# mahdi-slh/DeformContact

Measured on AMD Instinct MI355X. Metric: M edges/sec fwd+bwd, everyday-deform batch=32 per GPU (encoder hot path), higher is better.
Workload: dtype f32 (hops, storage, accumulate); wide dense blocks fp16x2-split operands (3 fp16 MFMA products, fp32 accumulate), narrow ones bf16x3-split (6 products); 1 GPU; everyday-deform synthetic, B=32 sample pairs per GPU: soft 32x(1024 v, 6132 e) + rigid 32x(762 v, 4560 e); TAGConv encoder 2 layers/branch, hidden 256, K=3 (configs[1]); edges_per_gpu_step=342144, global_batch=32, settle_steps=150, hipgraph=True, two_stream_branches=True, merged_branches=False, segmented_adjacency_build=True, parallelism=dp1

## Files before the change

deformcontact_amd/_lib.py:

```python
from __future__ import annotations

import ctypes
import os
from ctypes import POINTER, c_char_p, c_float, c_int, c_int32, c_int64, c_void_p

_HERE = os.path.dirname(os.path.abspath(__file__))
SO_PATH = os.path.join(_HERE, "libdeformcontact_hip.so")

_lib = None

_vp = c_void_p
_SIGNATURES = {
    "dc_version": (c_int, []),
    "dc_last_error": (c_char_p, []),
    "dc_stream_capture_id": (c_int64, [_vp]),
    "dc_csr_workspace_bytes": (c_int64, [c_int64, c_int64]),
    "dc_csr_build": (c_int, [_vp, c_int64, c_int64, c_int, c_int, _vp, _vp, _vp, _vp, _vp, _vp,
                             _vp, c_int64, _vp]),
    "dc_graph_workspace_bytes": (c_int64, [c_int64, c_int64]),
    "dc_graph_build": (c_int, [_vp, c_int64, c_int64, c_int, _vp, _vp, _vp, _vp, _vp, _vp, _vp, _vp,
                               _vp, _vp, c_int64, _vp]),
    "dc_graph_build_parts": (c_int, [POINTER(_vp), POINTER(c_int64), POINTER(c_int64), POINTER(c_int64), c_int,
                                     c_int64, c_int, _vp, _vp, _vp, _vp, _vp, _vp, _vp, _vp, _vp, _vp, c_int64,
                                     _vp]),
    "dc_graph_build_plan": (c_int, [c_int64, c_int64, c_int, POINTER(c_int), POINTER(c_int)]),
    "dc_graph_build_segmented": (c_int, [_vp, c_int64, c_int64, POINTER(c_int64), POINTER(c_int64), c_int,
                                         _vp, _vp, _vp, _vp, _vp, _vp, _vp, _vp, _vp, _vp]),
    "dc_attn_flash_prep": (c_int, [_vp, c_int64, c_int64, _vp, _vp, _vp]),
    "dc_attn_flash_ds": (c_int, [_vp, c_int64, _vp, _vp, c_int64, _vp, _vp, _vp, _vp, _vp, _vp, c_int64, c_int64,
                                 c_int64, c_int64, _vp, _vp, c_int64, _vp, _vp, _vp, _vp]),
    "dc_tag_linear_fwd_h2p_corr": (c_int, [_vp, c_int64, _vp, _vp, _vp, _vp, c_int64, c_int64, c_int64, c_int64, _vp, _vp,
                                           _vp]),
    "dc_tag_linear_bwd_dw_h2_corr": (c_int, [_vp, c_int64, _vp, _vp, POINTER(_vp), POINTER(c_int64), c_int, POINTER(_vp),
                                             c_int, c_int64, c_int, _vp, c_int64, c_int64, c_int64, c_int64, _vp, _vp,
                                             _vp]),
    "dc_attn_flash_fwd": (c_int, [_vp, c_int64, _vp, _vp, _vp, _vp, _vp, c_int64, c_int64, c_int64, c_int64, _vp,
                                  c_int64, _vp, _vp]),
    "dc_hop_chain_max_nodes": (c_int64, []),
    "dc_hop_chain_lds_request": (c_int64, []),
    "dc_hop_chain_f32": (c_int, [_vp, _vp, _vp, _vp, c_int64, POINTER(c_int64), c_int, _vp, c_int64, c_int64, c_int64,
                                 c_int, c_int, c_int, _vp, c_int, _vp]),
    "dc_spmm_f32_bias_act": (c_int, [_vp, _vp, _vp, _vp, c_int64, _vp, c_int, _vp, c_int64, c_int64, c_int64, _vp]),
    "dc_colsum_workspace_bytes": (c_int64, [c_int64, c_int64, c_int]),
    "dc_mask_colsum_f32": (c_int, [_vp, c_int64, _vp, c_int64, _vp, c_int64, c_int64, c_int64, _vp, c_int64, _vp, c_int,
                                   _vp]),
    "dc_gat_alpha_fwd": (c_int, [_vp, c_int64, _vp, _vp, _vp, _vp, c_int64, c_int64, _vp]),
    "dc_gat_alpha_bwd": (c_int, [_vp, c_int64, _vp, _vp, _vp, _vp, _vp, c_int64, c_int64, c_int64, _vp, c_int64, _vp, _vp,
                                 c_int, _vp]),
    "dc_spmm_f32_pack": (c_int, [_vp, _vp, _vp, _vp, c_int64, _vp, c_int64, c_int64, c_int64, c_int64, c_int64, _vp]),
    "dc_spmm_f32_window": (c_int, [_vp, _vp, _vp, _vp, c_int64, _vp, c_int64, _vp, c_int64, c_int64,
                                   c_int64, c_int64, _vp]),
    "dc_spmm_f32_rowmax_window": (c_int, [_vp, _vp, _vp, _vp, c_int64, _vp, c_int64, _vp, c_int64, c_int64,
                                          c_int64, _vp, c_int, c_int64, _vp]),
    "dc_tag_grouped_weight_prep": (c_int, [POINTER(_vp), c_int, c_int, c_int64, c_int64, POINTER(_vp),
                                           POINTER(_vp), POINTER(_vp), POINTER(_vp), _vp]),
    "dc_tag_grouped_fwd_h2p": (c_int, [_vp, c_int64, c_int, POINTER(c_int64), POINTER(c_int64), c_int64,
                                       POINTER(_vp), POINTER(_vp), c_int, _vp, c_int64, c_int64, c_int64, _vp,
                                       POINTER(_vp), _vp]),
    "dc_tag_grouped_mask_grad": (c_int, [POINTER(_vp), POINTER(c_int64), c_int, POINTER(c_int64),
                                         POINTER(c_int64), c_int64, _vp, c_int64, _vp, c_int64, c_int64, _vp,
                                         _vp, _vp]),
    "dc_tag_grouped_bwd_dw_workspace_bytes": (c_int64, [POINTER(c_int64), c_int, c_int64, c_int64, c_int]),
    "dc_tag_grouped_bwd_dw_h2": (c_int, [_vp, c_int64, POINTER(_vp), POINTER(c_int64), c_int, c_int,
                                         POINTER(c_int64), POINTER(c_int64), c_int64, POINTER(_vp),
                                         POINTER(_vp), c_int, _vp, c_int64, c_int64, c_int64, _vp, _vp, _vp]),
    "dc_generic_dense_launches": (c_int64, [c_int]),
    "dc_kernel_trace": (None, [c_int]),
    "dc_kernel_trace_dump": (c_int64, [c_char_p, c_int64]),
    "dc_hash_i64": (c_int, [_vp, c_int64, _vp, _vp]),
    "dc_morton_codes": (c_int, [_vp, c_int64, c_int64, POINTER(c_float), POINTER(c_float), _vp, _vp]),
    "dc_morton_order_workspace_bytes": (c_int64, [c_int64]),
    "dc_morton_order": (c_int, [_vp, c_int64, c_int64, _vp, _vp, _vp, c_int64, _vp]),
    "dc_relabel_edges": (c_int, [_vp, c_int64, _vp, c_int64, _vp, _vp]),
    "dc_gather_rows": (c_int, [_vp, c_int64, _vp, _vp, c_int64, c_int64, c_int64, _vp]),
    "dc_invert_perm": (c_int, [_vp, _vp, _vp, c_int64, _vp]),
    "dc_spmm_f32": (c_int, [_vp, _vp, _vp, _vp, c_int64, _vp, c_int64, _vp, c_int64, c_int64,
                            c_int64, _vp]),
    "dc_spmm_bf16": (c_int, [_vp, _vp, _vp, _vp, c_int64, _vp, c_int64, _vp, c_int64, c_int64,
                             c_int64, c_int, _vp]),
    "dc_tag_linear_fwd_bf16": (c_int, [_vp, c_int64, _vp, _vp, c_int, _vp, c_int64, c_int, c_int64, c_int64,
                                       c_int64, _vp]),
    "dc_tag_mask_grad_bf16": (c_int, [_vp, c_int64, c_int, _vp, c_int64, c_int, _vp, c_int64, c_int64, c_int64, _vp]),
    "dc_tag_linear_bwd_dw_bf16_workspace_bytes": (c_int64, [c_int64, c_int64, c_int64, c_int]),
    "dc_tag_linear_bwd_dw_bf16": (c_int, [_vp, c_int64, _vp, c_int64, c_int, POINTER(_vp), _vp, c_int, _vp, c_int64,
                                          c_int64, c_int64, c_int64, _vp]),
    "dc_to_bf16": (c_int, [POINTER(_vp), c_int, c_int64, c_int64, c_int64, _vp, c_int64, _vp]),
    "dc_contact_loss_workspace_bytes": (c_int64, [c_int64]),
    "dc_contact_loss": (c_int, [_vp, _vp, _vp, _vp, _vp, c_int64, _vp, c_int64, c_int64, c_int64, _vp, _vp,
                                _vp, _vp, c_int64, _vp]),
    "dc_tag_linear_fwd": (c_int, [POINTER(_vp), POINTER(c_int64), POINTER(_vp), c_int, _vp, c_int,
                                  _vp, c_int64, c_int64, c_int64, c_int64, _vp]),
    "dc_tag_linear_bwd_dx": (c_int, [_vp, c_int64, _vp, c_int64, POINTER(_vp), c_int,
                                     POINTER(_vp), POINTER(c_int64), c_int64, c_int64, c_int64,
                                     _vp]),
    "dc_tag_linear_fwd_split": (c_int, [POINTER(_vp), POINTER(c_int64), POINTER(_vp), c_int, _vp,
                                        c_int, _vp, c_int64, c_int64, c_int64, c_int64, c_int, _vp]),
    "dc_tag_linear_bwd_dx_split_workspace_bytes": (c_int64, [c_int64, c_int64, c_int]),
    "dc_tag_linear_bwd_dx_split": (c_int, [_vp, c_int64, _vp, c_int64, POINTER(_vp), c_int,
                                           POINTER(_vp), POINTER(c_int64), _vp, c_int64, c_int64,
                                           c_int64, c_int64, c_int, _vp]),
    "dc_tag_linear_bwd_dw_workspace_bytes": (c_int64, [c_int64, c_int64, c_int64, c_int]),
    "dc_tag_linear_bwd_dw": (c_int, [_vp, c_int64, _vp, c_int64, POINTER(_vp), POINTER(c_int64),
                                     c_int, POINTER(_vp), c_int, c_int64, _vp, c_int, _vp, c_int64,
                                     c_int64, c_int64, c_int64, _vp]),
    "dc_tag_linear_bwd_dw_split": (c_int, [_vp, c_int64, _vp, c_int64, POINTER(_vp),
                                           POINTER(c_int64), c_int, POINTER(_vp), c_int, c_int64,
                                           _vp, c_int, _vp, c_int64, c_int64, c_int64, c_int64,
                                           c_int, _vp]),
    "dc_tag_linear_fwd_h2": (c_int, [POINTER(_vp), POINTER(c_int64), POINTER(_vp), c_int, _vp,
                                     c_int, _vp, c_int64, c_int64, c_int64, c_int64, _vp, _vp, _vp]),
    "dc_tag_linear_bwd_dx_h2": (c_int, [_vp, c_int64, _vp, c_int64, POINTER(_vp), c_int,
                                        POINTER(_vp), POINTER(c_int64), _vp, c_int64, c_int64,
                                        c_int64, c_int64, _vp, _vp, _vp]),
    "dc_tag_linear_bwd_dw_h2": (c_int, [_vp, c_int64, _vp, c_int64, POINTER(_vp),
                                        POINTER(c_int64), c_int, POINTER(_vp), c_int, c_int64,
                                        _vp, c_int, _vp, c_int64, c_int64, c_int64, c_int64,
                                        _vp, _vp, _vp]),
    "dc_tag_mask_grad": (c_int, [_vp, c_int64, _vp, c_int64, _vp, c_int64, c_int64, c_int64, _vp, _vp, _vp]),
    "dc_tag_transpose_weights": (c_int, [POINTER(_vp), c_int, c_int64, c_int64, _vp, _vp]),
    "dc_tag_linear_fwd_h2p_workspace_bytes": (c_int64, [c_int64, c_int64, c_int64]),
    "dc_tag_linear_fwd_h2p": (c_int, [_vp, c_int64, _vp, _vp, c_int, _vp, c_int64, c_int64, c_int64, c_int64,
                                      _vp, _vp, _vp, c_int64, _vp]),
    "dc_tag_linear_fwd_h2p_exp": (c_int, [_vp, c_int64, _vp, _vp, c_int64, c_int64, c_int64, c_int64, _vp, _vp, _vp,
                                          c_int64, _vp]),
    "dc_tag_weight_prep": (c_int, [POINTER(_vp), c_int, c_int64, c_int64, _vp, _vp, _vp, _vp, _vp]),
    "dc_tag_weight_prep_zero": (c_int, [POINTER(_vp), c_int, c_int64, c_int64, _vp, _vp, _vp, _vp, _vp, c_int64, _vp]),
    "dc_rowabsmax_f32": (c_int, [_vp, c_int64, c_int64, c_int64, _vp, _vp]),
    "dc_tag_weight_rowmax": (c_int, [POINTER(_vp), c_int, c_int64, c_int64, _vp, _vp]),
    "dc_spmm_f32_rowmax": (c_int, [_vp, _vp, _vp, _vp, c_int64, _vp, c_int64, _vp, c_int64, c_int64,
                                   c_int64, _vp, c_int, _vp]),
    "dc_tag_pack_input": (c_int, [_vp, c_int64, _vp, c_int64, c_int64, c_int64, c_int64, c_int64, _vp]),
    "dc_tag_pack_weights": (c_int, [POINTER(_vp), c_int, _vp, c_int64, c_int64, c_int64, _vp]),
    "dc_tag_linear_fwd_narrow_ok": (c_int, [c_int64, c_int, c_int64, c_int64]),
    "dc_tag_linear_fwd_narrow": (c_int, [_vp, c_int64, POINTER(_vp), c_int, c_int64, _vp, c_int, _vp, c_int64, c_int64,
                                         c_int64, c_int64, _vp]),
    "dc_attn_softmax_rows": (c_int, [_vp, c_int64, c_int64, c_int64, c_int64, _vp, _vp]),
    "dc_attn_exp_rows": (c_int, [_vp, c_int64, c_int64, c_int64, c_int64, _vp, _vp]),
    "dc_attn_ds_rows": (c_int, [_vp, _vp, c_int64, c_int64, c_int64, _vp, _vp, _vp]),
    "dc_adam_flat": (c_int, [_vp, _vp, _vp, _vp, c_int64, _vp, c_float, c_float, c_float, c_float,
                             c_int, _vp]),
    "dc_compose_perm": (c_int, [_vp, _vp, _vp, _vp, c_int64, _vp]),
    "dc_gat_edge_softmax_fwd": (c_int, [_vp, _vp, _vp, _vp, c_float, _vp, c_int64, _vp]),
    "dc_gat_edge_softmax_bwd": (c_int, [_vp, _vp, _vp, _vp, c_float, _vp, _vp, _vp, _vp, c_int64,
                                        _vp]),
    "dc_sddmm_f32": (c_int, [_vp, _vp, _vp, c_int64, _vp, c_int64, _vp, c_int64, c_int64, _vp]),
    "dc_segment_sum_f32": (c_int, [_vp, _vp, _vp, _vp, c_int64, _vp]),
    "dc_gather_f32": (c_int, [_vp, _vp, _vp, _vp, c_int64, _vp]),
}


class DeformContactLibraryError(RuntimeError):
    pass


def lib():
    global _lib
    if _lib is None:
        if not os.path.exists(SO_PATH):
            raise DeformContactLibraryError(
                f"{SO_PATH} not found. Build it with `python -m deformcontact_amd.build` "
                "(hipcc --offload-arch=gfx950). deformcontact_amd has no CPU/PyTorch fallback.")
        try:
            handle = ctypes.CDLL(SO_PATH)
        except OSError as e:
            raise DeformContactLibraryError(f"cannot load {SO_PATH}: {e}") from e
        for name, (res, args) in _SIGNATURES.items():
            try:
                fn = getattr(handle, name)
            except AttributeError as e:
                raise DeformContactLibraryError(
                    f"{SO_PATH} does not export {name}; rebuild the library") from e
            fn.restype, fn.argtypes = res, args
        _lib = handle
    return _lib


def check(rc: int, what: str) -> None:
    if rc != 0:
        msg = lib().dc_last_error()
        raise DeformContactLibraryError(
            f"{what} failed (rc={rc}): {msg.decode() if msg else '?'}")


def kernel_trace(on: bool) -> None:
    lib().dc_kernel_trace(1 if on else 0)


def kernel_trace_counts() -> dict:
    n = int(lib().dc_kernel_trace_dump(None, 0))
    buf = ctypes.create_string_buffer(n + 1)
    lib().dc_kernel_trace_dump(buf, n + 1)
    out = {}
    for line in buf.value.decode().splitlines():
        name, _, cnt = line.rpartition(" ")
        out[name] = int(cnt)
    return out


def exported_names():
    return list(_SIGNATURES)
```

deformcontact_amd/csrc/dc_dense.h:

```cpp
#pragma once
#include "dc_common.h"

namespace dc {

constexpr int BK = 16;
constexpr int LDK = BK + 4;
constexpr int BN = 128;
constexpr int kMaxSeg = DC_MAX_SEG;

using f32x16 = __attribute__((ext_vector_type(16))) float;

struct Mat {
    const float *p;
    int64_t ld;
};

template <int MB>
struct Frag {
    float a[MB][4];
    float b[2][4];
};

template <int MB, bool A_KC, bool B_KC>
__device__ __forceinline__ void load_frag(Frag<MB> &f, const float *As, const float *Bs, int c,
                                          int wm, int wn) {
    constexpr int BM = 64 * MB;
    const int lane = threadIdx.x & 63, r = lane & 31, h = lane >> 5;
    const int kb = 8 * c + 4 * h;
#pragma unroll
    for (int mb = 0; mb < MB; ++mb) {
        const int row = wm * 32 * MB + mb * 32 + r;
        if (A_KC) {
            const float4 t = *reinterpret_cast<const float4 *>(As + row * LDK + kb);
            f.a[mb][0] = t.x, f.a[mb][1] = t.y, f.a[mb][2] = t.z, f.a[mb][3] = t.w;
        } else {
#pragma unroll
            for (int t = 0; t < 4; ++t) f.a[mb][t] = As[(kb + t) * BM + row];
        }
    }
#pragma unroll
    for (int nb = 0; nb < 2; ++nb) {
        if (B_KC) {
            const float4 t =
                *reinterpret_cast<const float4 *>(Bs + (wn * 64 + nb * 32 + r) * LDK + kb);
            f.b[nb][0] = t.x, f.b[nb][1] = t.y, f.b[nb][2] = t.z, f.b[nb][3] = t.w;
        } else {
#pragma unroll
            for (int t = 0; t < 4; ++t) f.b[nb][t] = Bs[(kb + t) * BN + wn * 64 + nb * 32 + r];
        }
    }
}

template <int MB>
__device__ __forceinline__ void mma_frag(const Frag<MB> &f, f32x16 (&acc)[MB][2]) {
#pragma unroll
    for (int t = 0; t < 4; ++t)
#pragma unroll
        for (int mb = 0; mb < MB; ++mb) {
            acc[mb][0] = __builtin_amdgcn_mfma_f32_32x32x2f32(f.a[mb][t], f.b[0][t], acc[mb][0], 0, 0, 0);
            acc[mb][1] = __builtin_amdgcn_mfma_f32_32x32x2f32(f.a[mb][t], f.b[1][t], acc[mb][1], 0, 0, 0);
        }
}

template <int MB>
__device__ __forceinline__ void zero_acc(f32x16 (&acc)[MB][2]) {
#pragma unroll
    for (int mb = 0; mb < MB; ++mb)
#pragma unroll
        for (int i = 0; i < 16; ++i) acc[mb][0][i] = 0.f, acc[mb][1][i] = 0.f;
}

template <int MB> struct Tile {
    static constexpr int BM = 64 * MB;
    static constexpr int A_KC = BM * LDK, B_KC = BN * LDK, A_RC = BK * BM, B_RC = BK * BN;
};

template <int MB, typename F>
__device__ __forceinline__ void for_each_acc(const f32x16 (&acc)[MB][2], int wm, int wn, F &&f) {
    const int lane = threadIdx.x & 63, c = lane & 31, h = lane >> 5;
#pragma unroll
    for (int mb = 0; mb < MB; ++mb)
#pragma unroll
        for (int nb = 0; nb < 2; ++nb)
#pragma unroll
            for (int reg = 0; reg < 16; ++reg) {
                const int row = wm * 32 * MB + mb * 32 + (reg & 3) + 8 * (reg >> 2) + 4 * h;
                const int col = wn * 64 + nb * 32 + c;
                f(row, col, acc[mb][nb][reg]);
            }
}

struct H2Scales {
    const float *a_rowmax;
    const float *b_rowmax;
    int b_presplit;
};

__device__ __forceinline__ unsigned h2_exp(float m) {
    unsigned e = (__float_as_uint(m) >> 23) & 0xffu;
    e = e < 15u ? 15u : e;
    return e > 254u ? 254u : e;
}
__device__ __forceinline__ float h2_scale(float m) { return __uint_as_float((268u - h2_exp(m)) << 23); }
__device__ __forceinline__ float h2_unscale(float m) { return __uint_as_float((h2_exp(m) - 14u) << 23); }

__device__ __forceinline__ float h2_block_max(const float *v, int64_t beg, int64_t end, float *red) {
    float m = 0.f;
    for (int64_t i = beg + threadIdx.x; i < end; i += 256) m = fmaxf(m, v[i]);
#pragma unroll
    for (int o = 32; o >= 1; o >>= 1) m = fmaxf(m, __shfl_xor(m, o));
    if ((threadIdx.x & 63) == 0) red[threadIdx.x >> 6] = m;
    __syncthreads();
    m = fmaxf(fmaxf(red[0], red[1]), fmaxf(red[2], red[3]));
    __syncthreads();
    return m;
}

constexpr int kMaxGroups = DC_MAX_GROUPS;
constexpr int kGroupAlign = DC_GROUP_ALIGN;
struct FwdGroups {
    int n;
    int64_t row_beg[kMaxGroups];
    int64_t row_end[kMaxGroups];
    const float *w[kMaxGroups];
    const float *bias[kMaxGroups];
    const float *b_rowmax[kMaxGroups];
};
__device__ __forceinline__ int group_of_row(const int64_t (&row_beg)[kMaxGroups], int n, int64_t row) {
    int g = 0;
#pragma unroll
    for (int q = 1; q < kMaxGroups; ++q)
        if (q < n && row >= row_beg[q]) g = q;
    return g;
}

struct FwdParams {
    Mat x[kMaxSeg];
    Mat w[kMaxSeg];
    const float *bias;
    float *out;
    int64_t ldo, N, Fi, Fo;
    int nseg, relu;
    H2Scales h2;
    int ksplit;
    float *kpartial;
    const float *exp_lse;
    int64_t exp_ncols;
    FwdGroups grp;
    const float *x2, *x2_coef;
};

struct DxParams {
    Mat g, mask;
    int has_mask;
    Mat w[kMaxSeg];
    float *gx[kMaxSeg];
    int64_t ldgx[kMaxSeg];
    int64_t N, Fi, Fo;
    int nseg;
    H2Scales h2;
};

struct DwGroups {
    int n;
    int chunk_beg[kMaxGroups + 1];
    int64_t row_beg[kMaxGroups], row_end[kMaxGroups], chunk_rows[kMaxGroups];
};

struct DwParams {
    Mat g, mask;
    int has_mask;
    Mat x[kMaxSeg];
    float *partial;
    float *bias_partial;
    int64_t N, Fi, Fo, chunk_rows;
    int nseg, nchunks;
    H2Scales h2;
    DwGroups grp;
    const float *g2, *g2_coef;
};


struct DwBf16Params {
    const uint16_t *g, *x;
    int64_t ldg, ldx;
    float *partial;
    float *bias_partial;
    int64_t N, Fi, Fo, chunk_rows;
    int nseg, nchunks;
};
bool dw_bf16_launch(const DwBf16Params &p, hipStream_t hs);

bool fwd_fast_launch(const FwdParams &p, int mb, hipStream_t hs);
bool dx_fast_launch(const DxParams &p, int mb, hipStream_t hs);
bool dw_fast_launch(const DwParams &p, int mb, hipStream_t hs);
bool fwd_split_launch(const FwdParams &p, int mb, int products, hipStream_t hs);
bool dx_split_launch(DxParams p, float *wt, int mb, int products, hipStream_t hs);
bool dw_split_launch(const DwParams &p, int mb, int products, hipStream_t hs);
bool dw_h2w_launch(const DwParams &p, hipStream_t hs);
bool fwd_h2_launch(const FwdParams &p, int mb, hipStream_t hs);
bool fwd_h2w_launch(const FwdParams &p, hipStream_t hs);
bool fwd_h2d_launch(const FwdParams &p, hipStream_t hs);
void transpose_weights_launch(const float *const *ws, int nseg, int64_t Fo, int64_t Fi, float *wt,
                              hipStream_t hs);

}
```

deformcontact_amd/csrc/dc_dense.hip:

```cpp
#include <stdlib.h>

#include "dc_dense.h"

#include <atomic>
static std::atomic<long long> g_generic_dense_launches{0};

namespace dc {

template <bool VEC>
__device__ __forceinline__ float4 ld4(const float *row_ptr, int64_t k, int64_t kmax) {
    if (VEC) {
        const int64_t kc = (k + 4 <= kmax) ? k : 0;
        return *reinterpret_cast<const float4 *>(row_ptr + kc);
    } else {
        const int64_t last = kmax - 1;
        return make_float4(row_ptr[k + 0 <= last ? k + 0 : last], row_ptr[k + 1 <= last ? k + 1 : last],
                           row_ptr[k + 2 <= last ? k + 2 : last], row_ptr[k + 3 <= last ? k + 3 : last]);
    }
}

__device__ __forceinline__ float4 zero_invalid(float4 v, bool row_ok, int64_t k, int64_t kmax) {
    return make_float4((row_ok && k + 0 < kmax) ? v.x : 0.f, (row_ok && k + 1 < kmax) ? v.y : 0.f,
                       (row_ok && k + 2 < kmax) ? v.z : 0.f, (row_ok && k + 3 < kmax) ? v.w : 0.f);
}
// ... 325 lines not shown
        *dst = p.accumulate ? *dst + t : t;
    }
}

__device__ __forceinline__ void dw_reduce_body1(const ReduceParams &p) {
    const int64_t per_out = p.Fo * p.cols, total = per_out * p.ngw;
    const int64_t seg_elems = p.Fo * p.Fi, slab = seg_elems * p.nseg;
    const int64_t i = (int64_t)blockIdx.x * blockDim.x + threadIdx.x;
    const float *src;
    float *dst;
    int64_t stride;
    if (i < total) {
        const int j = (int)(i / per_out);
        const int64_t rem = i % per_out, o = rem / p.cols, c = rem % p.cols;
        src = p.partial + (int64_t)(j / p.bps) * seg_elems + o * p.Fi + (int64_t)(j % p.bps) * p.cols + c;
        dst = p.gw[j] + rem;
        stride = slab;
    } else if (p.gbias && i < total + p.Fo) {
        src = p.bias_partial + (i - total);
        dst = p.gbias + (i - total);
        stride = p.Fo;
    } else {
        return;
    }
    float s = 0.f;
    int c = 0;
    for (; c + 8 <= p.nchunks; c += 8) {
        float v[8];
#pragma unroll
        for (int u = 0; u < 8; ++u) v[u] = src[(int64_t)(c + u) * stride];
#pragma unroll
        for (int u = 0; u < 8; ++u) s += v[u];
    }
    for (; c < p.nchunks; ++c) s += src[(int64_t)c * stride];
    *dst = p.accumulate ? *dst + s : s;
}

__global__ void __launch_bounds__(256)
k_dw_reduce(ReduceParams p) { dw_reduce_body1(p); }
__global__ void __launch_bounds__(256)
k_dw_reduce4(ReduceParams p) { dw_reduce_body(p); }
constexpr int kReduce4From = 64;
static inline void launch_reduce(const ReduceParams &r, int64_t total, hipStream_t hs) {
    if (r.nchunks >= kReduce4From)
        DC_LAUNCH(k_dw_reduce4, dim3((unsigned)((total + kReduceOutputs - 1) / kReduceOutputs)), dim3(256), 0, hs, r);
    else
        DC_LAUNCH(k_dw_reduce, dim3((unsigned)((total + 255) / 256)), dim3(256), 0, hs, r);
}

struct ReduceGroups {
    ReduceParams g[kMaxGroups];
};
__global__ void __launch_bounds__(256)
k_dw_reduce_grouped(ReduceGroups rg) { dw_reduce_body1(rg.g[blockIdx.y]); }

static inline Mat make_mat(const float *p, int64_t ld, bool *vec) {
    if (((uintptr_t)p & 15) != 0 || (ld % 4) != 0) *vec = false;
    return Mat{p, ld};
}

static inline int env_int(const char *name, int dflt) {
    const char *v = getenv(name);
    return v ? atoi(v) : dflt;
}

static inline int pick_mb(int64_t rows, int64_t col_tiles) {
    return (((rows + 127) / 128) * col_tiles >= 512) ? 2 : 1;
}

static inline int split_mb(int64_t rows, int64_t col_tiles) {
    const int64_t nb2 = ((rows + 127) / 128) * col_tiles, nb1 = ((rows + 63) / 64) * col_tiles;
    const double t2 = (double)((nb2 + 255) / 256);
    const double t1 = (double)((nb1 + 255) / 256) * 0.5 * 1.12;
    return t1 < t2 ? 1 : 2;
}

static inline int dw_mb(int64_t Fo) {
    return Fo >= 128 ? 2 : 1;
}

static void dw_plan(int64_t N, int64_t Fi, int64_t Fo, int nseg, int64_t *chunk_rows,
                    int *nchunks) {
    const int64_t BM = 64 * dw_mb(Fo);
    const int64_t tiles = ((Fo + BM - 1) / BM) * ((Fi + BN - 1) / BN) * nseg;
    constexpr int target = 512, maxchunks = 128;
    int64_t want = target / (tiles > 0 ? tiles : 1);
    if (want < 1) want = 1;
    if (want > maxchunks) want = maxchunks;
    if (want == 1 && N >= 8192) {
        const int64_t t2 = ((Fo + 127) / 128) * ((Fi + 255) / 256) * nseg;
        double best = 0.0;
        for (int64_t c = 1; c <= 8 && N / c >= 2048; ++c) {
            const int64_t w = (t2 * c + 255) / 256;
            const double eff = (double)(t2 * c) / (double)(w * 256);
            if (eff > best + 0.02) best = eff, want = c;
        }
    }
    int64_t rows = (N + want - 1) / want;
    if (rows < 256) rows = 256;
    rows = (rows + 2 * BK - 1) / (2 * BK) * (2 * BK);
    *chunk_rows = rows;
    *nchunks = (int)((N + rows - 1) / rows);
    if (*nchunks < 1) *nchunks = 1;
}

}

using namespace dc;

static int fwd_impl(const float *const *xs, const int64_t *ldxs, const float *const *ws, int nseg,
                    const float *bias, int relu, float *out, int64_t ldo, int64_t N, int64_t Fi,
                    int64_t Fo, dc_stream_t stream, int products, H2Scales h2 = H2Scales{},
                    float *ksplit_ws = nullptr, int64_t ksplit_ws_bytes = 0, const float *exp_lse = nullptr,
                    int64_t exp_ncols = 0) {
    DC_REQUIRE(nseg >= 1 && nseg <= kMaxSeg, "dc_tag_linear_fwd: nseg must be 1..%d", kMaxSeg);
    DC_REQUIRE(N >= 0 && Fi >= 1 && Fo >= 1, "dc_tag_linear_fwd: bad sizes");
    if (N == 0) return DC_OK;
    DC_REQUIRE(xs && ldxs && ws && out && ldo >= Fo, "dc_tag_linear_fwd: null pointer / ldo < Fo");
    FwdParams p{};
    bool vec = (Fi % 4 == 0);
    for (int s = 0; s < nseg; ++s) {
        DC_REQUIRE(xs[s] && ws[s] && ldxs[s] >= Fi, "dc_tag_linear_fwd: bad segment %d", s);
        p.x[s] = make_mat(xs[s], ldxs[s], &vec);
        p.w[s] = make_mat(ws[s], Fi, &vec);
    }
    p.bias = bias, p.out = out, p.ldo = ldo, p.N = N, p.Fi = Fi, p.Fo = Fo;
    p.nseg = nseg, p.relu = relu;
    p.h2 = h2;
    p.exp_lse = exp_lse, p.exp_ncols = exp_ncols;
    DC_REQUIRE(!exp_lse || h2.b_presplit, "dc_tag_linear_fwd: the exp epilogue exists on the pre-split h2 kernels only");
    const int64_t ntn = (Fo + BN - 1) / BN;
    const int mb = pick_mb(N, ntn);
    const int64_t grid = ((N + 64 * mb - 1) / (64 * mb)) * ntn;
    DC_REQUIRE(grid < (int64_t)INT32_MAX, "dc_tag_linear_fwd: grid too large");
    const dim3 gd((unsigned)grid), bd(256);
    hipStream_t hs = (hipStream_t)stream;
    if (products == 2 && vec) {
        int smb = split_mb(N, ntn);
        const int64_t nst = Fi / BK;
        if (ksplit_ws && !bias && !relu && ldo == Fo && nseg == 1) {
            smb = 2;
            int64_t tiles = ((N + 127) / 128) * ntn;
            if (tiles < 128) smb = 1, tiles = ((N + 63) / 64) * ntn;
            int64_t ks = tiles < 256 ? (512 + tiles - 1) / tiles : 1;
            if (ks > nst / 8) ks = nst / 8;
            if (ks > 32) ks = 32;
            while (ks > 1 && ks * N * Fo * (int64_t)sizeof(float) > ksplit_ws_bytes) --ks;
            if (ks > 1) p.ksplit = (int)ks, p.kpartial = ksplit_ws;
        }
        if (fwd_h2_launch(p, smb, hs)) {
            if (p.ksplit > 1) {
                ReduceParams r{};
                r.partial = p.kpartial, r.gw[0] = out, r.Fi = Fo, r.Fo = N, r.cols = Fo;
                r.nseg = 1, r.nchunks = p.ksplit, r.ngw = 1, r.bps = 1, r.accumulate = 0;
                const int64_t total = N * Fo;
                launch_reduce(r, total, hs);
            }
            return check_launch("dc_tag_linear_fwd_h2");
        }
        p.ksplit = 0, p.kpartial = nullptr;
    }
    DC_REQUIRE(!h2.b_presplit, "dc_tag_linear_fwd_h2p: shape not eligible for the pre-split kernel");
    if (products && vec && fwd_split_launch(p, split_mb(N, ntn), products, hs))
        return check_launch("dc_tag_linear_fwd_split");
    DC_REQUIRE(products != 2, "dc_tag_linear_fwd_h2: needs Fi %% 16 == 0, 16-byte aligned operands, "
                              "equal leading dimensions (Fi=%lld)", (long long)Fi);
    if (vec && fwd_fast_launch(p, mb, hs)) return check_launch("dc_tag_linear_fwd");
    static const int trace = env_int("DC_DENSE_TRACE", 0);
    ++g_generic_dense_launches;
    if (trace)
        fprintf(stderr, "[dc] generic fwd dense kernel: N=%lld Fi=%lld Fo=%lld nseg=%d vec=%d ldx=%lld ldo=%lld products=%d\n",
                (long long)N, (long long)Fi, (long long)Fo, nseg, (int)vec, (long long)ldxs[0], (long long)ldo, products);
    if (mb == 2 && vec)
        DC_LAUNCH((k_tag_linear_fwd<2, true>), gd, bd, 0, hs, p);
    else if (mb == 2)
        DC_LAUNCH((k_tag_linear_fwd<2, false>), gd, bd, 0, hs, p);
    else if (vec)
        DC_LAUNCH((k_tag_linear_fwd<1, true>), gd, bd, 0, hs, p);
    else
        DC_LAUNCH((k_tag_linear_fwd<1, false>), gd, bd, 0, hs, p);
    return check_launch("dc_tag_linear_fwd");
}

static int dx_impl(const float *g, int64_t ldg, const float *out_for_mask, int64_t ldo,
                   const float *const *ws, int nseg, float *const *gxs, const int64_t *ldgxs,
                   int64_t N, int64_t Fi, int64_t Fo, dc_stream_t stream, float *split_ws,
                   int products, H2Scales h2 = H2Scales{}) {
    DC_REQUIRE(nseg >= 1 && nseg <= kMaxSeg, "dc_tag_linear_bwd_dx: nseg must be 1..%d", kMaxSeg);
    DC_REQUIRE(N >= 0 && Fi >= 1 && Fo >= 1, "dc_tag_linear_bwd_dx: bad sizes");
    if (N == 0) return DC_OK;
    DC_REQUIRE(g && ws && gxs && ldgxs && ldg >= Fo, "dc_tag_linear_bwd_dx: null pointer / ldg < Fo");
    DC_REQUIRE(!out_for_mask || ldo >= Fo, "dc_tag_linear_bwd_dx: ldo < Fo");
    DxParams p{};
    bool vec = (Fi % 4 == 0) && (Fo % 4 == 0);
    p.g = make_mat(g, ldg, &vec);
    p.has_mask = out_for_mask != nullptr;
    if (out_for_mask) p.mask = make_mat(out_for_mask, ldo, &vec);
    for (int s = 0; s < nseg; ++s) {
        DC_REQUIRE(ws[s] && gxs[s] && ldgxs[s] >= Fi, "dc_tag_linear_bwd_dx: bad segment %d", s);
        p.w[s] = make_mat(ws[s], Fi, &vec);
        p.gx[s] = gxs[s];
        p.ldgx[s] = ldgxs[s];
    }
    p.N = N, p.Fi = Fi, p.Fo = Fo, p.nseg = nseg;
    p.h2 = h2;
    const int64_t ntn = ((Fi + BN - 1) / BN) * nseg;
    const int mb = pick_mb(N, ntn);
    const int64_t grid = ((N + 64 * mb - 1) / (64 * mb)) * ntn;
    DC_REQUIRE(grid < (int64_t)INT32_MAX, "dc_tag_linear_bwd_dx: grid too large");
    if (!p.has_mask) p.mask = p.g;
    const dim3 gd((unsigned)grid), bd(256);
    hipStream_t hs = (hipStream_t)stream;
    if (split_ws && vec && dx_split_launch(p, split_ws, split_mb(N, ntn), products, hs))
        return check_launch("dc_tag_linear_bwd_dx_split");
    DC_REQUIRE(products != 2, "dc_tag_linear_bwd_dx_h2: needs Fo %% 16 == 0, Fi %% 4 == 0 and 16-byte "
                              "aligned operands (Fi=%lld Fo=%lld)", (long long)Fi, (long long)Fo);
    if (vec && dx_fast_launch(p, mb, hs)) return check_launch("dc_tag_linear_bwd_dx");
    ++g_generic_dense_launches;
#define DC_DX(MB_, V_, M_) DC_LAUNCH((k_tag_linear_bwd_dx<MB_, V_, M_>), gd, bd, 0, hs, p)
    if (mb == 2) {
        if (vec && p.has_mask) DC_DX(2, true, true);
        else if (vec) DC_DX(2, true, false);
        else if (p.has_mask) DC_DX(2, false, true);
        else DC_DX(2, false, false);
    } else {
        if (vec && p.has_mask) DC_DX(1, true, true);
        else if (vec) DC_DX(1, true, false);
        else if (p.has_mask) DC_DX(1, false, true);
        else DC_DX(1, false, false);
    }
#undef DC_DX
    return check_launch("dc_tag_linear_bwd_dx");
}

extern "C" int dc_tag_linear_fwd(const float *const *xs, const int64_t *ldxs,
                                 const float *const *ws, int nseg, const float *bias, int relu,
                                 float *out, int64_t ldo, int64_t N, int64_t Fi, int64_t Fo,
                                 dc_stream_t stream) {
    return fwd_impl(xs, ldxs, ws, nseg, bias, relu, out, ldo, N, Fi, Fo, stream, 0);
}

extern "C" int dc_tag_linear_fwd_split(const float *const *xs, const int64_t *ldxs,
                                       const float *const *ws, int nseg, const float *bias,
                                       int relu, float *out, int64_t ldo, int64_t N, int64_t Fi,
                                       int64_t Fo, int products, dc_stream_t stream) {
    DC_REQUIRE(products == 6 || products == 3 || products == 1,
               "dc_tag_linear_fwd_split: products must be 6, 3 or 1");
    return fwd_impl(xs, ldxs, ws, nseg, bias, relu, out, ldo, N, Fi, Fo, stream, products);
}

extern "C" int dc_tag_linear_bwd_dx(const float *g, int64_t ldg, const float *out_for_mask,
                                    int64_t ldo, const float *const *ws, int nseg,
                                    float *const *gxs, const int64_t *ldgxs, int64_t N, int64_t Fi,
                                    int64_t Fo, dc_stream_t stream) {
    return dx_impl(g, ldg, out_for_mask, ldo, ws, nseg, gxs, ldgxs, N, Fi, Fo, stream, nullptr, 0);
}

extern "C" int dc_tag_linear_bwd_dw(const float *g, int64_t ldg, const float *out_for_mask,
                                    int64_t ldo, const float *const *xs, const int64_t *ldxs,
                                    int nseg, float *const *gws, int ngw, int64_t gw_cols,
                                    float *gbias, int accumulate, void *partials,
                                    int64_t partials_bytes, int64_t N, int64_t Fi, int64_t Fo,
                                    dc_stream_t stream);
extern "C" int dc_tag_linear_bwd_dw_split(const float *g, int64_t ldg, const float *out_for_mask,
                                          int64_t ldo, const float *const *xs, const int64_t *ldxs,
                                          int nseg, float *const *gws, int ngw, int64_t gw_cols,
                                          float *gbias, int accumulate, void *partials,
                                          int64_t partials_bytes, int64_t N, int64_t Fi, int64_t Fo,
                                          int products, dc_stream_t stream);

extern "C" int64_t dc_tag_linear_bwd_dx_split_workspace_bytes(int64_t Fi, int64_t Fo, int nseg) {
    if (Fi < 1 || Fo < 1 || nseg < 1 || nseg > kMaxSeg) return DC_EINVAL;
    return (int64_t)sizeof(float) * nseg * Fi * Fo + 16;
}

extern "C" int dc_tag_linear_bwd_dx_split(const float *g, int64_t ldg, const float *out_for_mask,
                                          int64_t ldo, const float *const *ws, int nseg,
                                          float *const *gxs, const int64_t *ldgxs, void *workspace,
                                          int64_t workspace_bytes, int64_t N, int64_t Fi,
                                          int64_t Fo, int products, dc_stream_t stream) {
    DC_REQUIRE(products == 6 || products == 3 || products == 1,
               "dc_tag_linear_bwd_dx_split: products must be 6, 3 or 1");
    DC_REQUIRE(workspace && ((uintptr_t)workspace & 15) == 0 &&
                   workspace_bytes >= dc_tag_linear_bwd_dx_split_workspace_bytes(Fi, Fo, nseg),
               "dc_tag_linear_bwd_dx_split: workspace missing, misaligned or too small");
    return dx_impl(g, ldg, out_for_mask, ldo, ws, nseg, gxs, ldgxs, N, Fi, Fo, stream,
                   (float *)workspace, products);
}

extern "C" int64_t dc_tag_linear_bwd_dw_workspace_bytes(int64_t N, int64_t Fi, int64_t Fo,
                                                        int nseg) {
    if (N < 0 || Fi < 1 || Fo < 1 || nseg < 1 || nseg > kMaxSeg) return DC_EINVAL;
    int64_t rows;
    int nchunks;
    dw_plan(N, Fi, Fo, nseg, &rows, &nchunks);
    return (int64_t)sizeof(float) * (nchunks + 1) * (nseg * Fo * Fi + Fo) + 16;
}

static int dw_impl(const float *g, int64_t ldg, const float *out_for_mask, int64_t ldo,
                   const float *const *xs, const int64_t *ldxs, int nseg, float *const *gws, int ngw,
                   int64_t gw_cols, float *gbias, int accumulate, void *partials,
                   int64_t partials_bytes, int64_t N, int64_t Fi, int64_t Fo, dc_stream_t stream,
                   int products, H2Scales h2 = H2Scales{}, const float *g2 = nullptr,
                   const float *g2_coef = nullptr) {
    DC_REQUIRE(nseg >= 1 && nseg <= kMaxSeg, "dc_tag_linear_bwd_dw: nseg must be 1..%d", kMaxSeg);
    DC_REQUIRE(N >= 0 && Fi >= 1 && Fo >= 1, "dc_tag_linear_bwd_dw: bad sizes");
    DC_REQUIRE(g && xs && ldxs && gws && partials && ldg >= Fo,
               "dc_tag_linear_bwd_dw: null pointer / ldg < Fo");
    DC_REQUIRE(!out_for_mask || ldo >= Fo, "dc_tag_linear_bwd_dw: ldo < Fo");
    DC_REQUIRE(partials_bytes >= dc_tag_linear_bwd_dw_workspace_bytes(N, Fi, Fo, nseg),
               "dc_tag_linear_bwd_dw: workspace too small");
    DC_REQUIRE(((uintptr_t)partials & 15) == 0, "dc_tag_linear_bwd_dw: workspace not 16-byte aligned");
    DwParams p{};
    bool vec = (Fi % 4 == 0) && (Fo % 4 == 0);
    p.g = make_mat(g, ldg, &vec);
    p.has_mask = out_for_mask != nullptr;
    if (out_for_mask) p.mask = make_mat(out_for_mask, ldo, &vec);
    ReduceParams r{};
    for (int s = 0; s < nseg; ++s) {
        DC_REQUIRE(xs[s] && ldxs[s] >= Fi, "dc_tag_linear_bwd_dw: bad segment %d", s);
        p.x[s] = make_mat(xs[s], ldxs[s], &vec);
    }
    DC_REQUIRE(ngw >= nseg && ngw <= 2 * kMaxSeg && ngw % nseg == 0 && gw_cols >= 1 &&
                   (ngw / nseg) * gw_cols <= Fi,
               "dc_tag_linear_bwd_dw: %d output blocks of %lld columns do not tile %d segments of %lld",
               ngw, (long long)gw_cols, nseg, (long long)Fi);
    for (int j = 0; j < ngw; ++j) {
        DC_REQUIRE(gws[j], "dc_tag_linear_bwd_dw: null output block %d", j);
        r.gw[j] = gws[j];
    }
    dw_plan(N, Fi, Fo, nseg, &p.chunk_rows, &p.nchunks);
    p.N = N, p.Fi = Fi, p.Fo = Fo, p.nseg = nseg;
    p.h2 = h2;
    p.partial = (float *)partials;
    const int64_t tail = vec ? N % BK : 0;
    const bool ragged = tail != 0 && N > tail;
    const int nslots = p.nchunks + (ragged ? 1 : 0);
    p.bias_partial = gbias ? p.partial + (int64_t)nslots * nseg * Fo * Fi : nullptr;
    const int mb = dw_mb(Fo);
    const int64_t tiles = ((Fo + 64 * mb - 1) / (64 * mb)) * ((Fi + BN - 1) / BN);
    const int64_t grid = tiles * nseg * p.nchunks;
    if (!p.has_mask) p.mask = p.g;
    const dim3 gd((unsigned)grid), bd(256);
    hipStream_t hs = (hipStream_t)stream;
    if (g2) {
        DC_REQUIRE(g2_coef && products == 2 && vec && !ragged && (((uintptr_t)g2) & 15) == 0,
                   "dc_tag_linear_bwd_dw_h2_corr: needs the coefficient vector, aligned operands and N %% 16 == 0");
        p.g2 = g2, p.g2_coef = g2_coef;
        DC_REQUIRE(dw_h2w_launch(p, hs), "dc_tag_linear_bwd_dw_h2_corr: shape not eligible for the 128 x 256 tile kernel "
                   "(needs Fo %% 128 == 0, Fi == 256, N %% 32 == 0; N=%lld Fi=%lld Fo=%lld)", (long long)N,
                   (long long)Fi, (long long)Fo);
        r.partial = p.partial, r.bias_partial = p.bias_partial, r.gbias = gbias;
        r.Fi = Fi, r.Fo = Fo, r.nseg = nseg, r.nchunks = nslots;
        r.cols = gw_cols, r.ngw = ngw, r.bps = ngw / nseg, r.accumulate = accumulate;
        const int64_t total_c = (int64_t)ngw * Fo * gw_cols + (gbias ? Fo : 0);
        launch_reduce(r, total_c, hs);
        return check_launch("dc_tag_linear_bwd_dw_h2_corr");
    }
    if (ragged) {
        DwParams t = p;
        const int64_t n0 = N - tail;
        t.g.p += n0 * t.g.ld;
        t.mask.p += n0 * t.mask.ld;
        for (int s = 0; s < nseg; ++s) t.x[s].p += n0 * t.x[s].ld;
        t.N = tail, t.chunk_rows = BK, t.nchunks = 1;
        t.partial = p.partial + (int64_t)p.nchunks * nseg * Fo * Fi;
        t.bias_partial = p.bias_partial ? p.bias_partial + (int64_t)p.nchunks * Fo : nullptr;
        t.h2 = H2Scales{};
        const dim3 gt((unsigned)(tiles * nseg));
        if (mb == 2) {
            if (p.has_mask) DC_LAUNCH((k_tag_linear_bwd_dw<2, true, true>), gt, bd, 0, hs, t);
            else DC_LAUNCH((k_tag_linear_bwd_dw<2, true, false>), gt, bd, 0, hs, t);
        } else {
            if (p.has_mask) DC_LAUNCH((k_tag_linear_bwd_dw<1, true, true>), gt, bd, 0, hs, t);
            else DC_LAUNCH((k_tag_linear_bwd_dw<1, true, false>), gt, bd, 0, hs, t);
        }
        p.N = n0;
    }
    bool fast_done = products && vec && dw_split_launch(p, mb, products, hs);
    DC_REQUIRE(fast_done || products != 2, "dc_tag_linear_bwd_dw_h2: needs N %% 16 == 0, Fi %% 4 == 0, "
               "Fo %% 4 == 0 and 16-byte aligned operands (N=%lld)", (long long)N);
    fast_done = fast_done || (vec && dw_fast_launch(p, mb, hs));
#define DC_DW(MB_, V_, M_) DC_LAUNCH((k_tag_linear_bwd_dw<MB_, V_, M_>), gd, bd, 0, hs, p)
    if (!fast_done) ++g_generic_dense_launches;
    if (fast_done) {
    } else
    if (mb == 2) {
        if (vec && p.has_mask) DC_DW(2, true, true);
        else if (vec) DC_DW(2, true, false);
        else if (p.has_mask) DC_DW(2, false, true);
        else DC_DW(2, false, false);
    } else {
        if (vec && p.has_mask) DC_DW(1, true, true);
        else if (vec) DC_DW(1, true, false);
        else if (p.has_mask) DC_DW(1, false, true);
        else DC_DW(1, false, false);
    }
#undef DC_DW
    r.partial = p.partial, r.bias_partial = p.bias_partial, r.gbias = gbias;
    r.Fi = Fi, r.Fo = Fo, r.nseg = nseg, r.nchunks = nslots;
    r.cols = gw_cols, r.ngw = ngw, r.bps = ngw / nseg, r.accumulate = accumulate;
    const int64_t total = (int64_t)ngw * Fo * gw_cols + (gbias ? Fo : 0);
    launch_reduce(r, total, (hipStream_t)stream);
    return check_launch("dc_tag_linear_bwd_dw");
}

extern "C" int dc_tag_linear_bwd_dw(const float *g, int64_t ldg, const float *out_for_mask,
                                    int64_t ldo, const float *const *xs, const int64_t *ldxs,
                                    int nseg, float *const *gws, int ngw, int64_t gw_cols,
                                    float *gbias, int accumulate, void *partials,
                                    int64_t partials_bytes, int64_t N, int64_t Fi, int64_t Fo,
                                    dc_stream_t stream) {
    return dw_impl(g, ldg, out_for_mask, ldo, xs, ldxs, nseg, gws, ngw, gw_cols, gbias, accumulate,
                   partials, partials_bytes, N, Fi, Fo, stream, 0);
}

extern "C" int dc_tag_linear_bwd_dw_split(const float *g, int64_t ldg, const float *out_for_mask,
                                          int64_t ldo, const float *const *xs, const int64_t *ldxs,
                                          int nseg, float *const *gws, int ngw, int64_t gw_cols,
                                          float *gbias, int accumulate, void *partials,
                                          int64_t partials_bytes, int64_t N, int64_t Fi, int64_t Fo,
                                          int products, dc_stream_t stream) {
    DC_REQUIRE(products == 6 || products == 3 || products == 1,
               "dc_tag_linear_bwd_dw_split: products must be 6, 3 or 1");
    return dw_impl(g, ldg, out_for_mask, ldo, xs, ldxs, nseg, gws, ngw, gw_cols, gbias, accumulate,
                   partials, partials_bytes, N, Fi, Fo, stream, products);
}


extern "C" int dc_tag_linear_fwd_h2(const float *const *xs, const int64_t *ldxs,
                                    const float *const *ws, int nseg, const float *bias, int relu,
                                    float *out, int64_t ldo, int64_t N, int64_t Fi, int64_t Fo,
                                    const float *x_rowmax, const float *w_rowmax,
                                    dc_stream_t stream) {
    DC_REQUIRE(x_rowmax && w_rowmax, "dc_tag_linear_fwd_h2: x_rowmax / w_rowmax missing");
    H2Scales h{};
    h.a_rowmax = x_rowmax, h.b_rowmax = w_rowmax;
    return fwd_impl(xs, ldxs, ws, nseg, bias, relu, out, ldo, N, Fi, Fo, stream, 2, h);
}

extern "C" int64_t dc_tag_linear_fwd_h2p_workspace_bytes(int64_t N, int64_t K, int64_t Fo) {
    if (N < 0 || K < 1 || Fo < 1) return DC_EINVAL;
    const int64_t tiles = ((N + 63) / 64) * ((Fo + BN - 1) / BN);
    if (tiles >= 256 || K / BK < 16) return 0;
    return 32 * N * Fo * (int64_t)sizeof(float);
}

extern "C" int dc_tag_linear_fwd_h2p(const float *x, int64_t ldx, const void *w_image,
                                     const float *bias, int relu, float *out, int64_t ldo, int64_t N,
                                     int64_t K, int64_t Fo, const float *x_rowmax,
                                     const float *w_rowmax, void *workspace,
                                     int64_t workspace_bytes, dc_stream_t stream) {
    DC_REQUIRE(x && w_image && x_rowmax && w_rowmax, "dc_tag_linear_fwd_h2p: null pointer");
    DC_REQUIRE(K >= 16 && K % 16 == 0 && ldx >= K && ldx % 4 == 0 && (((uintptr_t)x) & 15) == 0 &&
                   (((uintptr_t)w_image) & 15) == 0,
               "dc_tag_linear_fwd_h2p: K %% 16 == 0 and 16-byte aligned operands required (K=%lld)",
               (long long)K);
    H2Scales h{};
    h.a_rowmax = x_rowmax, h.b_rowmax = w_rowmax, h.b_presplit = 1;
    const float *xs[1] = {x};
    const float *ws[1] = {(const float *)w_image};
    const int64_t ld[1] = {ldx};
    DC_REQUIRE(!workspace || (((uintptr_t)workspace) & 15) == 0, "dc_tag_linear_fwd_h2p: workspace misaligned");
    return fwd_impl(xs, ld, ws, 1, bias, relu, out, ldo, N, K, Fo, stream, 2, h, (float *)workspace,
                    workspace ? workspace_bytes : 0);
}

extern "C" int dc_tag_linear_fwd_h2p_corr(const float *x, int64_t ldx, const float *x2, const float *x2_coef,
                                          const void *w_image, float *out, int64_t ldo, int64_t N, int64_t K,
                                          int64_t Fo, const float *x_rowmax, const float *w_rowmax,
                                          dc_stream_t stream) {
    DC_REQUIRE(N >= 0 && K >= 32 && K % 32 == 0 && Fo >= 1, "dc_tag_linear_fwd_h2p_corr: K must be a multiple of 32");
    if (N == 0) return DC_OK;
    DC_REQUIRE(x && x2 && x2_coef && w_image && out && x_rowmax && w_rowmax && ldx >= K && ldo >= Fo &&
                   (((uintptr_t)x2) & 15) == 0, "dc_tag_linear_fwd_h2p_corr: null / short / misaligned operand");
    FwdParams p{};
    bool vec = true;
    p.x[0] = make_mat(x, ldx, &vec);
    p.w[0] = make_mat((const float *)w_image, K, &vec);
    p.out = out, p.ldo = ldo, p.N = N, p.Fi = K, p.Fo = Fo, p.nseg = 1;
    p.h2.a_rowmax = x_rowmax, p.h2.b_rowmax = w_rowmax, p.h2.b_presplit = 1;
    p.x2 = x2, p.x2_coef = x2_coef;
    DC_REQUIRE(vec && fwd_h2w_launch(p, (hipStream_t)stream),
               "dc_tag_linear_fwd_h2p_corr: shape not eligible for the 128 x 256 tile kernel (N=%lld K=%lld Fo=%lld: "
               "needs 16-byte aligned rows)", (long long)N, (long long)K, (long long)Fo);
    return check_launch("dc_tag_linear_fwd_h2p_corr");
}

extern "C" int dc_tag_linear_fwd_h2p_exp(const float *x, int64_t ldx, const void *w_image, float *out,
                                         int64_t ldo, int64_t N, int64_t K, int64_t Fo, const float *x_rowmax,
                                         const float *w_rowmax, const float *row_lse, int64_t ncols_valid,
                                         dc_stream_t stream) {
    DC_REQUIRE(x && w_image && x_rowmax && w_rowmax && row_lse, "dc_tag_linear_fwd_h2p_exp: null pointer");
    DC_REQUIRE(K >= 16 && K % 16 == 0 && ldx >= K && ldx % 4 == 0 && (((uintptr_t)x) & 15) == 0 &&
                   (((uintptr_t)w_image) & 15) == 0 && ncols_valid >= 0 && ncols_valid <= Fo,
               "dc_tag_linear_fwd_h2p_exp: K %% 16 == 0, 16-byte aligned operands, 0 <= ncols_valid <= Fo required");
    H2Scales h{};
    h.a_rowmax = x_rowmax, h.b_rowmax = w_rowmax, h.b_presplit = 1;
    const float *xs[1] = {x};
    const float *ws[1] = {(const float *)w_image};
    const int64_t ld[1] = {ldx};
    return fwd_impl(xs, ld, ws, 1, nullptr, 0, out, ldo, N, K, Fo, stream, 2, h, nullptr, 0, row_lse, ncols_valid);
}

extern "C" int dc_tag_linear_bwd_dx_h2(const float *g, int64_t ldg, const float *out_for_mask,
                                       int64_t ldo, const float *const *ws, int nseg,
                                       float *const *gxs, const int64_t *ldgxs, void *workspace,
                                       int64_t workspace_bytes, int64_t N, int64_t Fi, int64_t Fo,
                                       const float *g_rowmax, const float *w_rowmax,
                                       dc_stream_t stream) {
    DC_REQUIRE(w_rowmax && g_rowmax, "dc_tag_linear_bwd_dx_h2: g_rowmax / w_rowmax missing");
    DC_REQUIRE(workspace && ((uintptr_t)workspace & 15) == 0 &&
                   workspace_bytes >= dc_tag_linear_bwd_dx_split_workspace_bytes(Fi, Fo, nseg),
               "dc_tag_linear_bwd_dx_h2: workspace missing, misaligned or too small");
    H2Scales h{};
    h.a_rowmax = g_rowmax, h.b_rowmax = w_rowmax;
    return dx_impl(g, ldg, out_for_mask, ldo, ws, nseg, gxs, ldgxs, N, Fi, Fo, stream,
                   (float *)workspace, 2, h);
}

extern "C" int dc_tag_linear_bwd_dw_h2(const float *g, int64_t ldg, const float *out_for_mask,
                                       int64_t ldo, const float *const *xs, const int64_t *ldxs,
                                       int nseg, float *const *gws, int ngw, int64_t gw_cols,
                                       float *gbias, int accumulate, void *partials,
                                       int64_t partials_bytes, int64_t N, int64_t Fi, int64_t Fo,
                                       const float *g_rowmax, const float *x_rowmax,
                                       dc_stream_t stream) {
    DC_REQUIRE(g_rowmax && x_rowmax, "dc_tag_linear_bwd_dw_h2: g_rowmax / x_rowmax missing");
    H2Scales h{};
    h.a_rowmax = g_rowmax, h.b_rowmax = x_rowmax;
    return dw_impl(g, ldg, out_for_mask, ldo, xs, ldxs, nseg, gws, ngw, gw_cols, gbias, accumulate,
                   partials, partials_bytes, N, Fi, Fo, stream, 2, h);
}

extern "C" int dc_tag_linear_bwd_dw_h2_corr(const float *g, int64_t ldg, const float *g2, const float *g2_coef,
                                            const float *const *xs, const int64_t *ldxs, int nseg,
                                            float *const *gws, int ngw, int64_t gw_cols, int accumulate,
                                            void *partials, int64_t partials_bytes, int64_t N, int64_t Fi,
                                            int64_t Fo, const float *g_rowmax, const float *x_rowmax,
                                            dc_stream_t stream) {
    DC_REQUIRE(g2 && g2_coef && g_rowmax && x_rowmax, "dc_tag_linear_bwd_dw_h2_corr: null g2 / coefficients / row maxima");
    H2Scales h2{};
    h2.a_rowmax = g_rowmax, h2.b_rowmax = x_rowmax;
    return dw_impl(g, ldg, nullptr, 0, xs, ldxs, nseg, gws, ngw, gw_cols, nullptr, accumulate, partials,
                   partials_bytes, N, Fi, Fo, stream, 2, h2, g2, g2_coef);
}

namespace dc {
__global__ void __launch_bounds__(256)
k_rowabsmax(const float *__restrict__ x, int64_t ld, int64_t N, int F, float *__restrict__ rowmax,
            bool vec4) {
    const int64_t row = (int64_t)blockIdx.x * 4 + (threadIdx.x >> 6);
    if (row >= N) return;
    const int lane = threadIdx.x & 63;
    const float *xr = x + row * ld;
    float m = 0.f;
    if (vec4) {
        for (int c = lane * 4; c < F; c += 256) {
            const float4 v = *reinterpret_cast<const float4 *>(xr + c);
            m = fmaxf(m, fmaxf(fmaxf(fabsf(v.x), fabsf(v.y)), fmaxf(fabsf(v.z), fabsf(v.w))));
        }
    } else {
        for (int c = lane; c < F; c += 64) m = fmaxf(m, fabsf(xr[c]));
    }
#pragma unroll
    for (int o = 32; o >= 1; o >>= 1) m = fmaxf(m, __shfl_xor(m, o));
    if (lane == 0) rowmax[row] = m;
}

struct WRowmaxParams {
    const float *w[kMaxSeg];
    int nseg;
    int64_t Fo, Fi;
    float *out;
};
__global__ void __launch_bounds__(256) k_w_rowmax(WRowmaxParams p) {
    const int64_t o = (int64_t)blockIdx.x * 4 + (threadIdx.x >> 6);
    if (o >= p.Fo) return;
    const int lane = threadIdx.x & 63;
    float m = 0.f;
    for (int s = 0; s < p.nseg; ++s) {
        const float *wr = p.w[s] + o * p.Fi;
        for (int64_t c = lane; c < p.Fi; c += 64) m = fmaxf(m, fabsf(wr[c]));
    }
#pragma unroll
    for (int q = 32; q >= 1; q >>= 1) m = fmaxf(m, __shfl_xor(m, q));
    if (lane == 0) p.out[o] = m;
}
}

namespace dc {
__global__ void __launch_bounds__(256)
k_mask_grad(const float *__restrict__ g, int64_t ldg, const float *__restrict__ mask, int64_t ldm,
            float *__restrict__ gm, int64_t ldgm, int64_t N, int F, float *__restrict__ rowmax_a,
            float *__restrict__ rowmax_b, bool vec4) {
    const int64_t row = (int64_t)blockIdx.x * 4 + (threadIdx.x >> 6);
    if (row >= N) return;
    const int lane = threadIdx.x & 63;
    const float *gr = g + row * ldg, *mr = mask ? mask + row * ldm : nullptr;
    float *o = gm + row * ldgm;
    float m = 0.f;
    if (vec4) {
        for (int c = lane * 4; c < F; c += 256) {
            float4 v = *reinterpret_cast<const float4 *>(gr + c);
            if (mr) {
                const float4 k = *reinterpret_cast<const float4 *>(mr + c);
                v = make_float4(k.x > 0.f ? v.x : 0.f, k.y > 0.f ? v.y : 0.f, k.z > 0.f ? v.z : 0.f,
                                k.w > 0.f ? v.w : 0.f);
            }
            *reinterpret_cast<float4 *>(o + c) = v;
            m = fmaxf(m, fmaxf(fmaxf(fabsf(v.x), fabsf(v.y)), fmaxf(fabsf(v.z), fabsf(v.w))));
        }
    } else {
        for (int c = lane; c < F; c += 64) {
            float v = gr[c];
            if (mr && !(mr[c] > 0.f)) v = 0.f;
            o[c] = v;
            m = fmaxf(m, fabsf(v));
        }
    }
#pragma unroll
    for (int q = 32; q >= 1; q >>= 1) m = fmaxf(m, __shfl_xor(m, q));
    if (lane == 0) {
        rowmax_a[row] = m;
        if (rowmax_b) rowmax_b[row] = m;
    }
}
}

extern "C" int dc_tag_mask_grad(const float *g, int64_t ldg, const float *out_for_mask, int64_t ldo,
                                float *gm, int64_t ldgm, int64_t N, int64_t F, float *rowmax_a,
                                float *rowmax_b, dc_stream_t stream) {
    DC_REQUIRE(N >= 0 && F >= 1 && F < (1 << 24) && ldg >= F && ldgm >= F && (!out_for_mask || ldo >= F),
               "dc_tag_mask_grad: bad sizes");
    if (N == 0) return DC_OK;
    DC_REQUIRE(g && gm && rowmax_a, "dc_tag_mask_grad: null pointer");
    const bool vec4 = (F % 4 == 0) && (ldg % 4 == 0) && (ldgm % 4 == 0) && (((uintptr_t)g) & 15) == 0 &&
                      (((uintptr_t)gm) & 15) == 0 &&
                      (!out_for_mask || ((ldo % 4 == 0) && (((uintptr_t)out_for_mask) & 15) == 0));
    DC_LAUNCH(k_mask_grad, dim3((unsigned)((N + 3) / 4)), dim3(256), 0, (hipStream_t)stream, g,
                       ldg, out_for_mask, ldo, gm, ldgm, N, (int)F, rowmax_a, rowmax_b, vec4);
    return check_launch("dc_tag_mask_grad");
}

namespace dc {
struct WPrepParams {
    const float *w[kMaxSeg];
    int nseg;
    int64_t Fo, Fi;
    float *w_rowmax, *wt_rowmax;
    _Float16 *wimg, *wtimg;
    float *zero;
    int64_t zero_n;
    int tall;
};
__device__ __forceinline__ void wprep_put(_Float16 *img_row, int64_t k, float v, float scale) {
    const float x = v * scale;
    const _Float16 h = (_Float16)x;
    _Float16 *rec = img_row + (k >> 4) * 32 + (k & 15);
    rec[0] = h;
    rec[16] = (_Float16)(x - (float)h);
}
__device__ __forceinline__ void weight_prep_body(const WPrepParams &p) {
    const int lane = threadIdx.x & 63;
    for (int64_t i = (int64_t)blockIdx.x * blockDim.x + threadIdx.x; i < p.zero_n; i += (int64_t)gridDim.x * blockDim.x)
        p.zero[i] = 0.f;
    if (p.tall)
        for (int64_t i = (int64_t)blockIdx.x * blockDim.x + threadIdx.x; i < p.Fi; i += (int64_t)gridDim.x * blockDim.x)
            p.wt_rowmax[i] = 0.f;
    const int64_t rb = (p.Fo + 3) / 4;
    float m = 0.f;
    const bool small = p.Fi <= 256 && p.Fo <= 256;
    if ((int64_t)blockIdx.x < rb) {
        const int64_t o = (int64_t)blockIdx.x * 4 + (threadIdx.x >> 6);
        if (o >= p.Fo) return;
        float v[kMaxSeg][4];
        if (small) {
#pragma unroll
            for (int s = 0; s < kMaxSeg; ++s)
#pragma unroll
                for (int j = 0; j < 4; ++j) {
                    const int64_t c = lane + 64 * j;
                    v[s][j] = (s < p.nseg && c < p.Fi) ? p.w[s][o * p.Fi + c] : 0.f;
                    m = fmaxf(m, fabsf(v[s][j]));
                }
        } else {
            for (int s = 0; s < p.nseg; ++s) {
                const float *wr = p.w[s] + o * p.Fi;
                for (int64_t c = lane; c < p.Fi; c += 64) m = fmaxf(m, fabsf(wr[c]));
            }
        }
#pragma unroll
        for (int q = 32; q >= 1; q >>= 1) m = fmaxf(m, __shfl_xor(m, q));
        if (lane == 0) p.w_rowmax[o] = m;
        if (p.wimg) {
            const float sc = h2_scale(m);
            _Float16 *row = p.wimg + o * (2 * p.nseg * p.Fi);
            if (small) {
#pragma unroll
                for (int s = 0; s < kMaxSeg; ++s)
#pragma unroll
                    for (int j = 0; j < 4; ++j) {
                        const int64_t c = lane + 64 * j;
                        if (s < p.nseg && c < p.Fi) wprep_put(row, s * p.Fi + c, v[s][j], sc);
                    }
            } else {
                for (int s = 0; s < p.nseg; ++s) {
                    const float *wr = p.w[s] + o * p.Fi;
                    for (int64_t c = lane; c < p.Fi; c += 64) wprep_put(row, s * p.Fi + c, wr[c], sc);
                }
            }
        }
    } else {
        const int64_t f = ((int64_t)blockIdx.x - rb) * 4 + (threadIdx.x >> 6);
        if (f >= p.Fi) return;
        float v[kMaxSeg][4];
        if (small) {
#pragma unroll
            for (int s = 0; s < kMaxSeg; ++s)
#pragma unroll
                for (int j = 0; j < 4; ++j) {
                    const int64_t o = lane + 64 * j;
                    v[s][j] = (s < p.nseg && o < p.Fo) ? p.w[s][o * p.Fi + f] : 0.f;
                    m = fmaxf(m, fabsf(v[s][j]));
                }
        } else {
            for (int s = 0; s < p.nseg; ++s) {
                const float *wc = p.w[s] + f;
                for (int64_t o = lane; o < p.Fo; o += 64) m = fmaxf(m, fabsf(wc[o * p.Fi]));
// ... 438 lines not shown
```

deformcontact_amd/csrc/dc_dense_narrow.hip:

```cpp
#include "dc_dense.h"

#ifndef DC_NARROW_ABL
#define DC_NARROW_ABL 0
#endif

namespace dc {

using nb_bf16x4 = __attribute__((ext_vector_type(4))) __bf16;
using nb_bf16x8 = __attribute__((ext_vector_type(8))) __bf16;
using nb_f32x4 = __attribute__((ext_vector_type(4))) float;

struct NarrowParams {
    const float *x;
    int64_t ld;
    const float *w[kMaxSeg];
    int nseg, fi;
    const float *bias;
    float *out;
    int64_t ldo, N;
    int relu, ntiles;
};

constexpr int kNarrowFo = 256;

__device__ __forceinline__ void nb_lds_barrier() {
    asm volatile("s_waitcnt lgkmcnt(0)\n\ts_barrier" ::: "memory");
}

__device__ __forceinline__ void nb_split1(float x, __bf16 &hi, __bf16 &mid, __bf16 &lo) {
    hi = (__bf16)x;
    const float r = x - (float)hi;
    mid = (__bf16)r;
    const float r2 = r - (float)mid;
    lo = (__bf16)r2;
}

template <int KS, int MB>
__global__ void __launch_bounds__(256)
k_fwd_narrow(NarrowParams p) {
    constexpr int TR = 32 * MB;
    constexpr int SROWA = KS * 96 + 16;
    constexpr int PPR = 4 * KS;
    constexpr int TP = TR * PPR, NV = (TP + 255) / 256;
    constexpr int KP = 16 * KS;
    constexpr int kOffStage = ((TR * SROWA + 1023) / 1024) * 1024;
    constexpr int kLdsTiles = kOffStage + TR * 1024, kLdsW = kNarrowFo * (KP + 4) * 4;
    __shared__ __attribute__((aligned(1024))) char lds[kLdsTiles > kLdsW ? kLdsTiles : kLdsW];
    char *const sA = lds;
    float *const so = reinterpret_cast<float *>(lds + kOffStage);
    const int wid = __builtin_amdgcn_readfirstlane((int)(threadIdx.x >> 6)), lane = threadIdx.x & 63;
    const int c = lane & 31, h = lane >> 5;

    nb_f32x4 xv[NV];
    auto load_tile = [&](int t) {
        const int64_t row0 = (int64_t)t * TR;
#pragma unroll
        for (int j = 0; j < NV; ++j) {
            const int q = (int)threadIdx.x + 256 * j;
            if (TP % 256 != 0 && q >= TP) continue;
            const int r = q / PPR, c4 = q - r * PPR;
            int64_t row = row0 + r;
            row = row < p.N ? row : p.N - 1;
            if (DC_NARROW_ABL & 8) xv[j] = nb_f32x4{(float)row, 1.f, 2.f, 3.f};
            else xv[j] = *reinterpret_cast<const nb_f32x4 *>(p.x + row * p.ld + 4 * c4);
        }
    };
    int t = blockIdx.x;
    if (t < p.ntiles) load_tile(t);

    constexpr int WROW = KP + 4;
    {
        float *wi = reinterpret_cast<float *>(lds);
        const int width = p.nseg * p.fi, per4 = kNarrowFo * p.fi / 4;
        constexpr int MAXQ = 8;
        nb_f32x4 wv[kMaxSeg][MAXQ];
#pragma unroll
        for (int s = 0; s < kMaxSeg; ++s)
#pragma unroll
            for (int j = 0; j < MAXQ; ++j) {
                const int q = (int)threadIdx.x + 256 * j;
                if (!(DC_NARROW_ABL & 2) && s < p.nseg && q < per4) wv[s][j] = *reinterpret_cast<const nb_f32x4 *>(p.w[s] + 4 * q);
            }
#pragma unroll
        for (int s = 0; s < kMaxSeg; ++s)
#pragma unroll
            for (int j = 0; j < MAXQ; ++j) {
                const int q = (int)threadIdx.x + 256 * j;
                if (!(DC_NARROW_ABL & 2) && s < p.nseg && q < per4) {
                    int o = (4 * q) / p.fi, f = 4 * q - o * p.fi;
#pragma unroll
                    for (int i = 0; i < 4; ++i) {
                        wi[o * WROW + s * p.fi + f] = wv[s][j][i];
                        if (++f == p.fi) f = 0, ++o;
                    }
                }
            }
        const int padw = KP - width;
        for (int e = threadIdx.x; e < kNarrowFo * padw; e += 256) {
            const int o = e / padw, f = e - o * padw;
            wi[o * WROW + width + f] = 0.f;
        }
    }
    __syncthreads();
    nb_bf16x8 fb[2][KS][3];
#pragma unroll
    for (int nb = 0; nb < 2; ++nb) {
        const float *wr = reinterpret_cast<const float *>(lds) + (64 * wid + 32 * nb + c) * WROW + 8 * h;
#pragma unroll
        for (int ks = 0; ks < KS; ++ks) {
            const nb_f32x4 v0 = *reinterpret_cast<const nb_f32x4 *>(wr + 16 * ks);
            const nb_f32x4 v1 = *reinterpret_cast<const nb_f32x4 *>(wr + 16 * ks + 4);
#pragma unroll
            for (int j = 0; j < 8; ++j) {
                __bf16 hi, mid, lo;
                nb_split1(j < 4 ? v0[j] : v1[j - 4], hi, mid, lo);
                fb[nb][ks][0][j] = hi, fb[nb][ks][1][j] = mid, fb[nb][ks][2][j] = lo;
            }
        }
    }
    __syncthreads();
    float bcol[2];
#pragma unroll
    for (int nb = 0; nb < 2; ++nb) bcol[nb] = p.bias ? p.bias[64 * wid + 32 * nb + c] : 0.f;
    const bool relu = p.relu != 0;

    auto store_tile = [&]() {
#pragma unroll
        for (int j = 0; j < NV; ++j) {
            const int q = (int)threadIdx.x + 256 * j;
            if (TP % 256 != 0 && q >= TP) continue;
            const int r = q / PPR, c4 = q - r * PPR;
            nb_bf16x4 hi, mid, lo;
#pragma unroll
            for (int i = 0; i < 4; ++i) {
                __bf16 a, b, d;
                nb_split1(xv[j][i], a, b, d);
                hi[i] = a, mid[i] = b, lo[i] = d;
            }
            char *dst = sA + r * SROWA + (c4 >> 2) * 96 + ((c4 >> 1) & 1) * 16 + (c4 & 1) * 8;
            *reinterpret_cast<nb_bf16x4 *>(dst) = hi;
            *reinterpret_cast<nb_bf16x4 *>(dst + 32) = mid;
            *reinterpret_cast<nb_bf16x4 *>(dst + 64) = lo;
        }
    };

    auto store_rows = [&](int64_t row0) {
#pragma unroll 4
        for (int r = wid; r < TR; r += 4) {
            const int64_t row = row0 + r;
            const nb_f32x4 v = *reinterpret_cast<const nb_f32x4 *>(so + r * 256 + 4 * lane);
            if (row < p.N && (!(DC_NARROW_ABL & 4) || v[0] == 12345.678f)) *reinterpret_cast<nb_f32x4 *>(p.out + row * p.ldo + 4 * lane) = v;
        }
    };
    int64_t prev_row0 = -1;
    for (; t < p.ntiles; t += gridDim.x) {
        const int64_t row0 = (int64_t)t * TR;
        if (!(DC_NARROW_ABL & 8)) store_tile();
        if (prev_row0 >= 0) store_rows(prev_row0);
        if (t + (int)gridDim.x < p.ntiles) load_tile(t + gridDim.x);
        nb_lds_barrier();
        f32x16 acc[MB][2];
#pragma unroll
        for (int mb = 0; mb < MB; ++mb)
#pragma unroll
            for (int nb = 0; nb < 2; ++nb)
#pragma unroll
                for (int i = 0; i < 16; ++i) acc[mb][nb][i] = 0.f;
        constexpr int HI = 0, MID = 1, LO = 2;
        constexpr int pa6[6] = {LO, HI, MID, MID, HI, HI}, pb6[6] = {HI, LO, MID, HI, MID, HI};
#pragma unroll
        for (int ks = 0; ks < KS; ++ks) {
            nb_bf16x8 fa[MB][3];
#pragma unroll
            for (int mb = 0; mb < MB; ++mb)
#pragma unroll
                for (int pl = 0; pl < 3; ++pl)
                    fa[mb][pl] = *reinterpret_cast<const nb_bf16x8 *>(sA + (mb * 32 + c) * SROWA + ks * 96 + pl * 32 + h * 16);
#pragma unroll
            for (int tt = 0; tt < 6; ++tt)
#pragma unroll
                for (int mb = 0; mb < MB; ++mb)
#pragma unroll
                    for (int nb = 0; nb < 2; ++nb)
                        if (!(DC_NARROW_ABL & 1))
                            acc[mb][nb] = __builtin_amdgcn_mfma_f32_32x32x16_bf16(fa[mb][pa6[tt]], fb[nb][ks][pb6[tt]], acc[mb][nb], 0, 0, 0);
                        else
                            acc[mb][nb][tt] += (float)fa[mb][pa6[tt]][0] * (float)fb[nb][ks][pb6[tt]][0];
        }
#pragma unroll
        for (int mb = 0; mb < MB; ++mb)
#pragma unroll
            for (int nb = 0; nb < 2; ++nb)
#pragma unroll
                for (int r = 0; r < 16; ++r) {
                    float v = acc[mb][nb][r] + bcol[nb];
                    if (relu) v = fmaxf(v, 0.f);
                    if (!(DC_NARROW_ABL & 16) || r == 0)
                        so[(mb * 32 + (r & 3) + 8 * (r >> 2) + 4 * h) * 256 + 64 * wid + 32 * nb + c] = v;
                }
        nb_lds_barrier();
        prev_row0 = row0;
    }
    if (prev_row0 >= 0) store_rows(prev_row0);
}

template <int KS>
static void narrow_launch(const NarrowParams &p0, hipStream_t hs) {
    NarrowParams p = p0;
    p.ntiles = (int)((p.N + 31) / 32);
    const unsigned grid = (unsigned)(p.ntiles < 256 ? p.ntiles : 256);
    DC_LAUNCH((k_fwd_narrow<KS, 1>), dim3(grid), dim3(256), 0, hs, p);
}

}

using namespace dc;

extern "C" int dc_tag_linear_fwd_narrow_ok(int64_t fi, int nseg, int64_t wpad, int64_t Fo) {
    return (Fo == kNarrowFo && nseg >= 1 && nseg <= kMaxSeg && fi >= 1 && fi <= 32 && nseg * fi <= wpad &&
            (wpad == 96 || wpad == 112 || wpad == 128)) ? 1 : 0;
}

extern "C" int dc_tag_linear_fwd_narrow(const float *slab, int64_t ld, const float *const *ws, int nseg, int64_t fi,
                                        const float *bias, int relu, float *out, int64_t ldo, int64_t N, int64_t wpad,
                                        int64_t Fo, dc_stream_t stream) {
    DC_REQUIRE(dc_tag_linear_fwd_narrow_ok(fi, nseg, wpad, Fo),
               "dc_tag_linear_fwd_narrow: needs Fo = 256, a padded reduction of 96 / 112 / 128 >= nseg * fi (got Fo=%lld wpad=%lld "
               "nseg=%d fi=%lld)", (long long)Fo, (long long)wpad, nseg, (long long)fi);
    DC_REQUIRE(N >= 0, "dc_tag_linear_fwd_narrow: negative N");
    if (N == 0) return DC_OK;
    DC_REQUIRE(slab && ws && out && ld >= wpad && ldo >= Fo, "dc_tag_linear_fwd_narrow: null pointer / short leading dimension");
    DC_REQUIRE(ld % 4 == 0 && ldo % 4 == 0 && ((uintptr_t)slab & 15) == 0 && ((uintptr_t)out & 15) == 0,
               "dc_tag_linear_fwd_narrow: rows of the slab and of the output must be 16-byte aligned");
    DC_REQUIRE(N < ((int64_t)1 << 31) - 64, "dc_tag_linear_fwd_narrow: too many rows");
    NarrowParams p{};
    p.x = slab, p.ld = ld, p.nseg = nseg, p.fi = (int)fi, p.bias = bias, p.out = out, p.ldo = ldo, p.N = N, p.relu = relu;
    for (int s = 0; s < nseg; ++s) {
        DC_REQUIRE(ws[s], "dc_tag_linear_fwd_narrow: null weight segment %d", s);
        p.w[s] = ws[s];
    }
    hipStream_t hs = (hipStream_t)stream;
    switch (wpad) {
    case 96: narrow_launch<6>(p, hs); break;
    case 112: narrow_launch<7>(p, hs); break;
    default: narrow_launch<8>(p, hs); break;
    }
    return check_launch("dc_tag_linear_fwd_narrow");
}
```

deformcontact_amd/csrc/dc_dense_split.hip:

```cpp
#include "dc_dense.h"

#ifndef DC_DWS_ABL
#define DC_DWS_ABL 0
#endif

namespace dc {

using bf16x4 = __attribute__((ext_vector_type(4))) __bf16;
using bf16x8 = __attribute__((ext_vector_type(8))) __bf16;

constexpr int kPlane = 32;

template <int NP> struct Planes {
    static_assert(NP == 6 || NP == 3 || NP == 1 || NP == 2, "products per tile: 6, 3, 1 or 2 (= fp16x2)");
    static constexpr bool F16 = NP == 2;
    static constexpr int P = NP == 6 ? 3 : ((NP == 3 || NP == 2) ? 2 : 1);
    static constexpr int NPROD = NP == 2 ? 3 : NP;
    static constexpr int SROW = P * kPlane + 16;
};

using f16x4 = __attribute__((ext_vector_type(4))) _Float16;
using f16x8 = __attribute__((ext_vector_type(8))) _Float16;

__device__ __forceinline__ void split4_h2(const float4 &v, f16x4 &h, f16x4 &l) {
    const float x[4] = {v.x, v.y, v.z, v.w};
#pragma unroll
    for (int i = 0; i < 4; ++i) {
        const _Float16 a = (_Float16)x[i];
        h[i] = a;
        l[i] = (_Float16)(x[i] - (float)a);
    }
}

__device__ __forceinline__ void split1(float x, __bf16 &hi, __bf16 &mid, __bf16 &lo) {
    hi = (__bf16)x;
    const float r = x - (float)hi;
    mid = (__bf16)r;
    const float r2 = r - (float)mid;
    lo = (__bf16)r2;
}

__device__ __forceinline__ void split4(const float4 &v, bf16x4 &hi, bf16x4 &mid, bf16x4 &lo) {
    __bf16 h, m, l;
    split1(v.x, h, m, l); hi[0] = h, mid[0] = m, lo[0] = l;
    split1(v.y, h, m, l); hi[1] = h, mid[1] = m, lo[1] = l;
    split1(v.z, h, m, l); hi[2] = h, mid[2] = m, lo[2] = l;
    split1(v.w, h, m, l); hi[3] = h, mid[3] = m, lo[3] = l;
}

template <int ROWS, bool MASK, int NP>
struct SplitOp {
    static constexpr int SROW = Planes<NP>::SROW, P = Planes<NP>::P;
    static constexpr int NV = ROWS / 64;
    const float *p[NV];
    const float *pm[MASK ? NV : 1];
    float4 v[NV];
    float4 m[MASK ? NV : 1];
    int off[NV];
    float sc[NV];

    __device__ __forceinline__ void init(const float *base, const float *mbase, int64_t ld,
                                         int64_t row0, int64_t nrows, int64_t mld = 0) {
        const int k4 = threadIdx.x & 3, r = threadIdx.x >> 2;
#pragma unroll
        for (int j = 0; j < NV; ++j) {
            int64_t row = row0 + r + 64 * j;
            row = row < nrows ? row : nrows - 1;
            p[j] = base + row * ld + 4 * k4;
            if (MASK) pm[j] = mbase + row * (mld ? mld : ld) + 4 * k4;
            off[j] = (r + 64 * j) * SROW + 8 * k4;
        }
    }
    __device__ __forceinline__ void rebase(int64_t delta) {
#pragma unroll
        for (int j = 0; j < NV; ++j) p[j] += delta;
    }
    __device__ __forceinline__ void load() {
#pragma unroll
        for (int j = 0; j < NV; ++j) {
            v[j] = *reinterpret_cast<const float4 *>(p[j]);
            p[j] += BK;
            if (MASK) {
                m[j] = *reinterpret_cast<const float4 *>(pm[j]);
                pm[j] += BK;
            }
        }
    }
    __device__ __forceinline__ void store(char *lds) const {
#pragma unroll
        for (int j = 0; j < NV; ++j) {
            float4 x = v[j];
            if (MASK)
                x = make_float4(m[j].x > 0.f ? x.x : 0.f, m[j].y > 0.f ? x.y : 0.f,
                                m[j].z > 0.f ? x.z : 0.f, m[j].w > 0.f ? x.w : 0.f);
            if (Planes<NP>::F16) {
                x = make_float4(x.x * sc[j], x.y * sc[j], x.z * sc[j], x.w * sc[j]);
                f16x4 h, l;
                split4_h2(x, h, l);
                *reinterpret_cast<f16x4 *>(lds + off[j]) = h;
                *reinterpret_cast<f16x4 *>(lds + off[j] + kPlane) = l;
                continue;
            }
            bf16x4 hi, mid, lo;
            split4(x, hi, mid, lo);
            *reinterpret_cast<bf16x4 *>(lds + off[j]) = hi;
            if (P > 1) *reinterpret_cast<bf16x4 *>(lds + off[j] + kPlane) = mid;
            if (P > 2) *reinterpret_cast<bf16x4 *>(lds + off[j] + 2 * kPlane) = lo;
        }
    }
    __device__ __forceinline__ void set_scale(float s) {
#pragma unroll
        for (int j = 0; j < NV; ++j) sc[j] = s;
    }
};

template <int MB, int NP>
struct SplitFrag {
    bf16x8 a[MB][Planes<NP>::P];
    bf16x8 b[2][Planes<NP>::P];
};

template <int MB, int NP>
__device__ __forceinline__ void load_split_frag(SplitFrag<MB, NP> &f, const char *As,
                                                const char *Bs, int wm, int wn) {
    constexpr int SROW = Planes<NP>::SROW, P = Planes<NP>::P;
    const int lane = threadIdx.x & 63, r = lane & 31, h = lane >> 5;
#pragma unroll
    for (int mb = 0; mb < MB; ++mb)
#pragma unroll
        for (int pl = 0; pl < P; ++pl)
            f.a[mb][pl] = *reinterpret_cast<const bf16x8 *>(
                As + (wm * 32 * MB + mb * 32 + r) * SROW + pl * kPlane + 16 * h);
#pragma unroll
    for (int nb = 0; nb < 2; ++nb)
#pragma unroll
        for (int pl = 0; pl < P; ++pl)
            f.b[nb][pl] = *reinterpret_cast<const bf16x8 *>(
                Bs + (wn * 64 + nb * 32 + r) * SROW + pl * kPlane + 16 * h);
}

template <int MB, int NP>
__device__ __forceinline__ void mma_split(const SplitFrag<MB, NP> &f, f32x16 (&acc)[MB][2]) {
    constexpr int HI = 0, MID = 1, LO = 2;
    constexpr int pa6[6] = {LO, HI, MID, MID, HI, HI}, pb6[6] = {HI, LO, MID, HI, MID, HI};
    constexpr int pa3[3] = {MID, HI, HI}, pb3[3] = {HI, MID, HI};
    constexpr int NPROD = Planes<NP>::NPROD;
#pragma unroll
    for (int t = 0; t < NPROD; ++t) {
        const int ia = NPROD == 6 ? pa6[t] : (NPROD == 3 ? pa3[t] : HI);
        const int ib = NPROD == 6 ? pb6[t] : (NPROD == 3 ? pb3[t] : HI);
#pragma unroll
        for (int mb = 0; mb < MB; ++mb)
#pragma unroll
            for (int nb = 0; nb < 2; ++nb) {
                if (Planes<NP>::F16)
                    acc[mb][nb] = __builtin_amdgcn_mfma_f32_32x32x16_f16(
                        __builtin_bit_cast(f16x8, f.a[mb][ia]), __builtin_bit_cast(f16x8, f.b[nb][ib]),
                        acc[mb][nb], 0, 0, 0);
                else
                    acc[mb][nb] = __builtin_amdgcn_mfma_f32_32x32x16_bf16(f.a[mb][ia], f.b[nb][ib],
                                                                          acc[mb][nb], 0, 0, 0);
            }
    }
}

template <int MB, int NP, typename OA, typename OB, typename Next>
__device__ __forceinline__ void split_loop(char *lds, int nst, OA &A, OB &B, Next &&next_stage,
                                           f32x16 (&acc)[MB][2], int wm, int wn) {
    constexpr int SROW = Planes<NP>::SROW;
    constexpr int BM = 64 * MB, kOffB = BM * SROW, kStage = (BM + BN) * SROW;
    if (nst <= 0) return;
    A.load();
    B.load();
    next_stage();
    A.store(lds);
    B.store(lds + kOffB);
    if (nst > 1) {
        A.load();
        B.load();
        next_stage();
    }
    __syncthreads();
    for (int it = 0; it < nst; ++it) {
        char *cur = lds + (it & 1) * kStage, *nxt = lds + ((it + 1) & 1) * kStage;
        SplitFrag<MB, NP> f;
        load_split_frag<MB, NP>(f, cur, cur + kOffB, wm, wn);
        if (it + 1 < nst) {
            A.store(nxt);
            B.store(nxt + kOffB);
        }
        if (it + 2 < nst) {
            A.load();
            B.load();
            next_stage();
        }
        mma_split<MB, NP>(f, acc);
        __syncthreads();
    }
}

template <int MB, int NP>
__global__ void __launch_bounds__(256)
k_fwd_split(FwdParams p) {
    constexpr int BM = 64 * MB, SROW = Planes<NP>::SROW;
    __shared__ __attribute__((aligned(16))) char lds[2 * (BM + BN) * SROW];
    const unsigned ntn = (unsigned)((p.Fo + BN - 1) / BN);
    const unsigned lb = xcd_remap(blockIdx.x, gridDim.x);
    const int64_t row0 = (int64_t)(lb / ntn) * BM, col0 = (int64_t)(lb % ntn) * BN;
    const int wid = threadIdx.x >> 6, wm = wid >> 1, wn = wid & 1;

    f32x16 acc[MB][2];
    zero_acc<MB>(acc);
    SplitOp<BM, false, NP> A;
    SplitOp<BN, false, NP> B;
    A.init(p.x[0].p, nullptr, p.x[0].ld, row0, p.N);
    B.init(p.w[0].p, nullptr, p.Fi, col0, p.Fo);
    constexpr bool F16 = Planes<NP>::F16;
    __shared__ float s_inv[F16 ? BM : 1];
    if (F16) {
        const int r = threadIdx.x >> 2;
#pragma unroll
        for (int j = 0; j < BM / 64; ++j) {
            int64_t row = row0 + r + 64 * j;
            row = row < p.N ? row : p.N - 1;
            const float m = p.h2.a_rowmax[row];
            A.sc[j] = h2_scale(m);
            if ((threadIdx.x & 3) == 0) s_inv[r + 64 * j] = h2_unscale(m);
        }
#pragma unroll
        for (int j = 0; j < BN / 64; ++j) {
            int64_t col = col0 + r + 64 * j;
            col = col < p.Fo ? col : p.Fo - 1;
            B.sc[j] = h2_scale(p.h2.b_rowmax[col]);
        }
    }
    const int kst = (int)(p.Fi / BK), nst = kst * p.nseg;
    int kk = 0, seg = 0;
    auto next_stage = [&]() {
        if (++kk == kst && seg + 1 < p.nseg) {
            kk = 0;
            A.rebase((p.x[seg + 1].p - p.x[seg].p) - p.Fi);
            B.rebase((p.w[seg + 1].p - p.w[seg].p) - p.Fi);
            ++seg;
        }
    };
    split_loop<MB, NP>(lds, nst, A, B, next_stage, acc, wm, wn);

    float bcol[2], icol[2] = {1.f, 1.f};
#pragma unroll
    for (int nb = 0; nb < 2; ++nb) {
        const int64_t col = col0 + wn * 64 + nb * 32 + (threadIdx.x & 31);
        bcol[nb] = (p.bias && col < p.Fo) ? p.bias[col] : 0.f;
        if (F16) icol[nb] = h2_unscale(p.h2.b_rowmax[col < p.Fo ? col : p.Fo - 1]);
    }
    const bool relu = p.relu != 0;
    for_each_acc<MB>(acc, wm, wn, [&](int r, int c, float v) {
        const int64_t row = row0 + r, col = col0 + c;
        if (row < p.N && col < p.Fo) {
            if (F16) v = (v * s_inv[r]) * icol[(c >> 5) & 1];
            v += bcol[(c >> 5) & 1];
            if (relu) v = fmaxf(v, 0.f);
            p.out[row * p.ldo + col] = v;
        }
    });
}

template <int MB, bool MASK, int NP>
__global__ void __launch_bounds__(256)
k_dx_split(DxParams p) {
    constexpr int BM = 64 * MB, SROW = Planes<NP>::SROW;
    __shared__ __attribute__((aligned(16))) char lds[2 * (BM + BN) * SROW];
    const unsigned ntn = (unsigned)((p.Fi + BN - 1) / BN), per_row = ntn * p.nseg;
    const unsigned lb = xcd_remap(blockIdx.x, gridDim.x);
    const int64_t row0 = (int64_t)(lb / per_row) * BM;
    const int s = (int)((lb % per_row) / ntn);
    const int64_t col0 = (int64_t)(lb % ntn) * BN;
    const int wid = threadIdx.x >> 6, wm = wid >> 1, wn = wid & 1;

    f32x16 acc[MB][2];
    zero_acc<MB>(acc);
    SplitOp<BM, MASK, NP> A;
    SplitOp<BN, false, NP> B;
    A.init(p.g.p, p.mask.p, p.g.ld, row0, p.N, p.mask.ld);
    B.init(p.w[s].p, nullptr, p.Fo, col0, p.Fi);
    constexpr bool F16 = Planes<NP>::F16;
    __shared__ float s_inv[F16 ? BM : 1];
    float invb = 1.f;
    if (F16) {
        const int r = threadIdx.x >> 2;
#pragma unroll
        for (int j = 0; j < BM / 64; ++j) {
            int64_t row = row0 + r + 64 * j;
            row = row < p.N ? row : p.N - 1;
            const float m = p.h2.a_rowmax[row];
            A.sc[j] = h2_scale(m);
            if ((threadIdx.x & 3) == 0) s_inv[r + 64 * j] = h2_unscale(m);
        }
        const float bm = h2_block_max(p.h2.b_rowmax, 0, p.Fo, reinterpret_cast<float *>(lds));
        B.set_scale(h2_scale(bm));
        invb = h2_unscale(bm);
    }
    split_loop<MB, NP>(lds, (int)(p.Fo / BK), A, B, []() {}, acc, wm, wn);
    float *out = p.gx[s];
    const int64_t ldo = p.ldgx[s];
    for_each_acc<MB>(acc, wm, wn, [&](int r, int c, float v) {
        const int64_t row = row0 + r, col = col0 + c;
        if (F16) v = (v * s_inv[r]) * invb;
        if (row < p.N && col < p.Fi) out[row * ldo + col] = v;
    });
}

template <int COLS, int NP> struct TrImage {
    static constexpr int ROWB = COLS * 2 + 64;
    static constexpr int PLANE = BK * ROWB;
    static constexpr int BYTES = Planes<NP>::P * PLANE;
};

template <int COLS, bool MASK, int NP>
struct SplitOpRC {
    static constexpr int P = Planes<NP>::P;
    static constexpr int NV = COLS / 64;
    static constexpr int PER = COLS / 4, KPER = 256 / PER;
    using Img = TrImage<COLS, NP>;
    const float *p[NV];
    const float *pm[MASK ? NV : 1];
    float4 v[NV];
    float4 m[MASK ? NV : 1];
    int off[NV];
    int64_t step, mstep;
    float sc;

    __device__ __forceinline__ void init(const float *base, const float *mbase, int64_t ld,
                                         int64_t k0, int64_t col0, int64_t ncols, int64_t mld = 0) {
        const int c4 = threadIdx.x % PER, kr = threadIdx.x / PER;
        int64_t col = col0 + 4 * c4;
        col = col + 4 <= ncols ? col : ncols - 4;
        mld = mld ? mld : ld;
#pragma unroll
        for (int j = 0; j < NV; ++j) {
            const int64_t k = k0 + kr + KPER * j;
            p[j] = base + k * ld + col;
            if (MASK) pm[j] = mbase + k * mld + col;
            off[j] = (kr + KPER * j) * Img::ROWB + 8 * c4;
        }
        step = BK * ld;
        mstep = BK * mld;
    }
    __device__ __forceinline__ void load() {
#pragma unroll
        for (int j = 0; j < NV; ++j) {
            if ((DC_DWS_ABL & 8) && MASK) v[j] = make_float4(1.f, 2.f, 3.f, (float)j);
            else if ((DC_DWS_ABL & 16) && !MASK) v[j] = make_float4(1.f, 2.f, 3.f, (float)j);
            else v[j] = *reinterpret_cast<const float4 *>(p[j]);
            p[j] += step;
            if (MASK) {
                if (DC_DWS_ABL & 2) m[j] = make_float4(1.f, -1.f, 1.f, 1.f);
                else m[j] = *reinterpret_cast<const float4 *>(pm[j]);
                pm[j] += mstep;
            }
        }
    }
    __device__ __forceinline__ float4 value(int j) const {
        if (!MASK) return v[j];
        return make_float4(m[j].x > 0.f ? v[j].x : 0.f, m[j].y > 0.f ? v[j].y : 0.f,
                           m[j].z > 0.f ? v[j].z : 0.f, m[j].w > 0.f ? v[j].w : 0.f);
    }
    __device__ __forceinline__ void store(char *lds) const {
#pragma unroll
        for (int j = 0; j < NV; ++j) {
            if (Planes<NP>::F16) {
                float4 x = value(j);
                x = make_float4(x.x * sc, x.y * sc, x.z * sc, x.w * sc);
                f16x4 h, l;
                split4_h2(x, h, l);
                *reinterpret_cast<f16x4 *>(lds + off[j]) = h;
                *reinterpret_cast<f16x4 *>(lds + off[j] + Img::PLANE) = l;
                continue;
            }
            bf16x4 hi, mid, lo;
            split4(value(j), hi, mid, lo);
            *reinterpret_cast<bf16x4 *>(lds + off[j]) = hi;
            if (P > 1) *reinterpret_cast<bf16x4 *>(lds + off[j] + Img::PLANE) = mid;
            if (P > 2) *reinterpret_cast<bf16x4 *>(lds + off[j] + 2 * Img::PLANE) = lo;
        }
    }
};

using s16x4 = __attribute__((ext_vector_type(4))) short;
typedef __attribute__((address_space(3))) s16x4 lds_s16x4;

template <int ROWB>
__device__ __forceinline__ bf16x8 tr_operand(const char *plane, int m0) {
    const int lane = threadIdx.x & 63, g = lane >> 4, q = (lane >> 2) & 3, pp = lane & 3;
    const int h = g >> 1;
    const char *a = plane + (8 * h + q) * ROWB + (m0 + 16 * (g & 1) + 4 * pp) * 2;
    const s16x4 lo4 = __builtin_amdgcn_ds_read_tr16_b64_v4i16((lds_s16x4 *)(uintptr_t)(a));
    const s16x4 hi4 = __builtin_amdgcn_ds_read_tr16_b64_v4i16(
        (lds_s16x4 *)(uintptr_t)(a + 4 * ROWB));
    union { s16x4 s[2]; bf16x8 b; } u;
    u.s[0] = lo4, u.s[1] = hi4;
    return u.b;
}

template <int MB, bool MASK, int NP>
__global__ void __launch_bounds__(256)
k_dw_split(DwParams p) {
    constexpr int BM = 64 * MB, P = Planes<NP>::P;
    using IA = TrImage<BM, NP>;
    using IB = TrImage<BN, NP>;
    constexpr int kStage = IA::BYTES + IB::BYTES, kOffB = IA::BYTES;
    __shared__ __attribute__((aligned(16))) char lds[2 * kStage];
    const unsigned ntm = (unsigned)((p.Fo + BM - 1) / BM), ntn = (unsigned)((p.Fi + BN - 1) / BN);
    const unsigned tiles = ntm * ntn, per_chunk = tiles * p.nseg;
    const unsigned lb = xcd_remap(blockIdx.x, gridDim.x);
    const unsigned chunk = lb / per_chunk, rem = lb % per_chunk;
    const int s = (int)(rem / tiles);
    const int64_t o0 = (int64_t)((rem % tiles) / ntn) * BM, f0 = (int64_t)((rem % tiles) % ntn) * BN;
    const int64_t n_beg = (int64_t)chunk * p.chunk_rows;
    const int64_t n_end = (n_beg + p.chunk_rows < p.N) ? n_beg + p.chunk_rows : p.N;
    const int wid = threadIdx.x >> 6, wm = wid >> 1, wn = wid & 1;
    const bool do_bias = p.bias_partial && s == 0 && f0 == 0;

    f32x16 acc[MB][2];
    zero_acc<MB>(acc);
    float4 bsum4 = make_float4(0.f, 0.f, 0.f, 0.f);
    using OA = SplitOpRC<BM, MASK, NP>;
    OA A;
    SplitOpRC<BN, false, NP> B;
    A.init(p.g.p, p.mask.p, p.g.ld, n_beg, o0, p.Fo, p.mask.ld);
    B.init(p.x[s].p, nullptr, p.x[s].ld, n_beg, f0, p.Fi);
    float inva = 1.f, invb = 1.f;
    if (Planes<NP>::F16) {
        const float am = h2_block_max(p.h2.a_rowmax, n_beg, n_end, reinterpret_cast<float *>(lds));
        const float bm = h2_block_max(p.h2.b_rowmax, n_beg, n_end, reinterpret_cast<float *>(lds));
        A.sc = h2_scale(am), B.sc = h2_scale(bm);
        inva = h2_unscale(am), invb = h2_unscale(bm);
    }
    auto bias_acc = [&]() {
        if (do_bias) {
#pragma unroll
            for (int j = 0; j < OA::NV; ++j) {
                const float4 x = A.value(j);
                bsum4.x += x.x, bsum4.y += x.y, bsum4.z += x.z, bsum4.w += x.w;
            }
        }
    };
    const int nst = (int)((n_end - n_beg) / BK);
    if (nst > 0) {
        A.load();
        B.load();
        A.store(lds);
        B.store(lds + kOffB);
        bias_acc();
        if (nst > 1) {
            A.load();
            B.load();
        }
    }
    __syncthreads();
    for (int it = 0; it < nst; ++it) {
        const char *cur = lds + (it & 1) * kStage;
        char *nxt = lds + ((it + 1) & 1) * kStage;
        SplitFrag<MB, NP> f;
#pragma unroll
        for (int pl = 0; pl < P; ++pl) {
#pragma unroll
            for (int mb = 0; mb < MB; ++mb)
                f.a[mb][pl] = tr_operand<IA::ROWB>(cur + pl * IA::PLANE, wm * 32 * MB + mb * 32);
#pragma unroll
            for (int nb = 0; nb < 2; ++nb)
                f.b[nb][pl] = tr_operand<IB::ROWB>(cur + kOffB + pl * IB::PLANE, wn * 64 + nb * 32);
        }
        if (it + 1 < nst) {
            A.store(nxt);
            B.store(nxt + kOffB);
            bias_acc();
        }
        if (it + 2 < nst) {
            A.load();
            B.load();
        }
        if (!(DC_DWS_ABL & 1)) mma_split<MB, NP>(f, acc);
        else acc[0][0][it & 15] += (float)f.a[0][0][0] * (float)f.b[0][0][0];
        __syncthreads();
    }
    float *out = p.partial + ((int64_t)chunk * p.nseg + s) * p.Fo * p.Fi;
    for_each_acc<MB>(acc, wm, wn, [&](int r, int c, float v) {
        const int64_t o = o0 + r, ff = f0 + c;
        if (Planes<NP>::F16) v = (v * inva) * invb;
        if (o < p.Fo && ff < p.Fi && (!(DC_DWS_ABL & 4) || v == 12345.678f)) out[o * p.Fi + ff] = v;
    });
    if (do_bias) {
        __syncthreads();
        float4 *red = reinterpret_cast<float4 *>(lds);
        red[threadIdx.x] = bsum4;
        __syncthreads();
        if (threadIdx.x < OA::PER) {
            float4 t = make_float4(0.f, 0.f, 0.f, 0.f);
            for (int g = 0; g < 256 / OA::PER; ++g) {
                const float4 v = red[g * OA::PER + threadIdx.x];
                t.x += v.x, t.y += v.y, t.z += v.z, t.w += v.w;
            }
            float *bp = p.bias_partial + (int64_t)chunk * p.Fo;
            const int64_t o = o0 + 4 * threadIdx.x;
            if (o + 4 <= p.Fo) bp[o + 0] = t.x, bp[o + 1] = t.y, bp[o + 2] = t.z, bp[o + 3] = t.w;
        }
    }
}

constexpr int kDwK = 32;
template <int COLS> struct TrImage32 {
    static constexpr int ROWB = COLS * 2 + 64;
    static constexpr int PLANE = kDwK * ROWB;
    static constexpr int BYTES = 2 * PLANE;
};

template <bool CORR = false>
__global__ void __launch_bounds__(512)
k_dw_h2w(DwParams p) {
    using IA = TrImage32<128>;
    using IB = TrImage32<256>;
    constexpr int kStage = IA::BYTES + IB::BYTES, kOffB = IA::BYTES;
    __shared__ __attribute__((aligned(16))) char lds[2 * kStage];
    const unsigned nto = (unsigned)(p.Fo / 128);
    const unsigned per_chunk = nto * (unsigned)p.nseg;
    const unsigned lb = xcd_remap(blockIdx.x, gridDim.x);
    const unsigned chunk = lb / per_chunk, rem = lb % per_chunk;
    const int s = (int)(rem / nto);
    const int64_t o0 = (int64_t)(rem % nto) * 128;
    int64_t n_beg = (int64_t)chunk * p.chunk_rows;
    int64_t n_end = (n_beg + p.chunk_rows < p.N) ? n_beg + p.chunk_rows : p.N;
    if (p.grp.n >= 1) {
        int g = 0;
#pragma unroll
        for (int q = 1; q < kMaxGroups; ++q)
            if (q < p.grp.n && (int)chunk >= p.grp.chunk_beg[q]) g = q;
        n_beg = p.grp.row_beg[g] + (int64_t)((int)chunk - p.grp.chunk_beg[g]) * p.grp.chunk_rows[g];
        n_end = n_beg + p.grp.chunk_rows[g] < p.grp.row_end[g] ? n_beg + p.grp.chunk_rows[g] : p.grp.row_end[g];
        if (n_end < n_beg) n_end = n_beg;
    }
    const int wid = threadIdx.x >> 6, wm = wid >> 2, wn = wid & 3;
    const bool do_bias = p.bias_partial && s == 0;

    float am = 0.f, bm = 0.f;
    for (int64_t i = n_beg + threadIdx.x; i < n_end; i += 512) {
        am = fmaxf(am, p.h2.a_rowmax[i]);
        bm = fmaxf(bm, p.h2.b_rowmax[i]);
    }
#pragma unroll
    for (int o = 32; o >= 1; o >>= 1) {
        am = fmaxf(am, __shfl_xor(am, o));
        bm = fmaxf(bm, __shfl_xor(bm, o));
    }
    {
        float *red = reinterpret_cast<float *>(lds);
        if ((threadIdx.x & 63) == 0) red[wid] = am, red[8 + wid] = bm;
        __syncthreads();
        am = bm = 0.f;
#pragma unroll
        for (int i = 0; i < 8; ++i) am = fmaxf(am, red[i]), bm = fmaxf(bm, red[8 + i]);
        __syncthreads();
    }
    const float sca = h2_scale(am), scb = h2_scale(bm), inva = h2_unscale(am), invb = h2_unscale(bm);

    const int c4g = threadIdx.x & 31, krg = threadIdx.x >> 5;
    const int c4x = threadIdx.x & 63, krx = threadIdx.x >> 6;
    const int64_t ldg = p.g.ld, ldx = p.x[s].ld;
    unsigned offg[2], offx[4];
    int ldsg[2], ldsx[4];
#pragma unroll
    for (int j = 0; j < 2; ++j) {
        offg[j] = (unsigned)((krg + 16 * j) * ldg + 4 * c4g);
        ldsg[j] = (krg + 16 * j) * IA::ROWB + 8 * c4g;
    }
#pragma unroll
    for (int j = 0; j < 4; ++j) {
        offx[j] = (unsigned)((krx + 8 * j) * ldx + 4 * c4x);
        ldsx[j] = kOffB + (krx + 8 * j) * IB::ROWB + 8 * c4x;
    }
    const float *baseg = p.g.p + n_beg * ldg + o0;
    const float *basex = p.x[s].p + n_beg * ldx;
    using f32x4 = __attribute__((ext_vector_type(4))) float;
    f32x4 vg0[2], vg1[2], vx0[4], vx1[4];
    f32x4 vc0[2], vc1[2];
    float cc0[2], cc1[2];
    f32x4 bsum = {0.f, 0.f, 0.f, 0.f};
    const float *baseg2 = CORR ? p.g2 + n_beg * ldg + o0 : nullptr;
    const float *basec = CORR ? p.g2_coef + n_beg + krg : nullptr;

    auto gload_c = [&](f32x4 (&vg)[2], f32x4 (&vx)[4], f32x4 (&vc)[2], float (&cc)[2]) {
#pragma unroll
        for (int j = 0; j < 2; ++j) vg[j] = *reinterpret_cast<const f32x4 *>(baseg + offg[j]);
        if (CORR) {
#pragma unroll
            for (int j = 0; j < 2; ++j) {
                vc[j] = *reinterpret_cast<const f32x4 *>(baseg2 + offg[j]);
                cc[j] = basec[16 * j];
            }
            baseg2 += kDwK * ldg;
            basec += kDwK;
        }
#pragma unroll
        for (int j = 0; j < 4; ++j) vx[j] = *reinterpret_cast<const f32x4 *>(basex + offx[j]);
        baseg += kDwK * ldg;
        basex += kDwK * ldx;
    };
    auto gload = [&](f32x4 (&vg)[2], f32x4 (&vx)[4]) {
        if (&vg == &vg0) gload_c(vg, vx, vc0, cc0); else gload_c(vg, vx, vc1, cc1);
    };
    auto split_store = [&](char *dst, int plane, f32x4 v, float sc) {
        v = v * sc;
        f16x4 h, l;
#pragma unroll
        for (int i = 0; i < 4; ++i) {
            const _Float16 a = (_Float16)v[i];
            h[i] = a;
            l[i] = (_Float16)(v[i] - (float)a);
        }
        *reinterpret_cast<f16x4 *>(dst) = h;
        *reinterpret_cast<f16x4 *>(dst + plane) = l;
    };
    auto lstore = [&](const f32x4 (&vg)[2], const f32x4 (&vx)[4], int b) {
        char *buf = lds + b * kStage;
        const bool set0 = &vg == &vg0;
#pragma unroll
        for (int j = 0; j < 2; ++j) {
            f32x4 gv = vg[j];
            if (CORR) gv = set0 ? gv - vc0[j] * cc0[j] : gv - vc1[j] * cc1[j];
            split_store(buf + ldsg[j], IA::PLANE, gv, sca);
            if (do_bias) bsum += vg[j];
        }
#pragma unroll
        for (int j = 0; j < 4; ++j) split_store(buf + ldsx[j], IB::PLANE, vx[j], scb);
    };
    f32x16 acc[2][2];
    zero_acc<2>(acc);
    auto compute = [&](int b) {
        const char *buf = lds + b * kStage;
#pragma unroll
        for (int ks = 0; ks < 2; ++ks) {
            SplitFrag<2, 2> f;
#pragma unroll
            for (int pl = 0; pl < 2; ++pl) {
#pragma unroll
                for (int mb = 0; mb < 2; ++mb)
                    f.a[mb][pl] = tr_operand<IA::ROWB>(buf + pl * IA::PLANE + ks * 16 * IA::ROWB, wm * 64 + mb * 32);
#pragma unroll
                for (int nb = 0; nb < 2; ++nb)
                    f.b[nb][pl] = tr_operand<IB::ROWB>(buf + kOffB + pl * IB::PLANE + ks * 16 * IB::ROWB,
                                                       wn * 64 + nb * 32);
            }
            mma_split<2, 2>(f, acc);
        }
    };

    const int nst = (int)((n_end - n_beg) / kDwK);
    if (nst > 0) {
        gload(vg0, vx0);
        if (nst > 1) gload(vg1, vx1);
        lstore(vg0, vx0, 0);
    }
    __syncthreads();
    int it = 0;
#define DC_DW_STAGE(CUR, VG_L, VX_L, VG_S, VX_S)                                                      \
    gload(VG_L, VX_L);                                                                \
    __builtin_amdgcn_sched_barrier(0);                    \
    compute(CUR);                                                                                     \
    lstore(VG_S, VX_S, CUR ^ 1);                                                      \
    __syncthreads();
    for (; it + 3 < nst; it += 2) {
        DC_DW_STAGE(0, vg0, vx0, vg1, vx1)
        DC_DW_STAGE(1, vg1, vx1, vg0, vx0)
    }
#undef DC_DW_STAGE
#define DC_DW_TAIL(K, CUR, VG_L, VX_L, VG_S, VX_S)                                                    \
    if (it + K < nst) {                                                                               \
        if (it + K + 2 < nst) gload(VG_L, VX_L);                                                      \
        compute(CUR);                                                                                 \
        if (it + K + 1 < nst) lstore(VG_S, VX_S, CUR ^ 1);                                            \
        __syncthreads();                                                                              \
    }
    for (; it < nst; it += 2) {
        DC_DW_TAIL(0, 0, vg0, vx0, vg1, vx1)
        DC_DW_TAIL(1, 1, vg1, vx1, vg0, vx0)
    }
#undef DC_DW_TAIL

    float *out = p.partial + ((int64_t)chunk * p.nseg + s) * p.Fo * p.Fi;
    for_each_acc<2>(acc, wm, wn, [&](int r, int c, float v) {
        out[(o0 + r) * p.Fi + c] = (v * inva) * invb;
    });
    if (do_bias) {
        f32x4 *red = reinterpret_cast<f32x4 *>(lds);
        red[threadIdx.x] = bsum;
        __syncthreads();
        if (threadIdx.x < 32) {
            f32x4 t = {0.f, 0.f, 0.f, 0.f};
            for (int g = 0; g < 16; ++g) t += red[g * 32 + threadIdx.x];
            float *bp = p.bias_partial + (int64_t)chunk * p.Fo + o0 + 4 * threadIdx.x;
            bp[0] = t[0], bp[1] = t[1], bp[2] = t[2], bp[3] = t[3];
        }
    }
}

bool dw_h2w_launch(const DwParams &p, hipStream_t hs) {
    static const int wide = getenv("DC_DW_WIDE") ? atoi(getenv("DC_DW_WIDE")) : 1;
    if ((!wide && p.grp.n < 1) || p.has_mask || p.Fo % 128 != 0 || p.Fo < 128 || p.Fi != 256 || p.N % kDwK != 0 ||
        p.chunk_rows % kDwK != 0)
        return false;
    if (p.g.ld * kDwK >= ((int64_t)1 << 30)) return false;
    for (int s = 0; s < p.nseg; ++s)
        if (p.x[s].ld * kDwK >= ((int64_t)1 << 30)) return false;
    const int64_t grid = (p.Fo / 128) * p.nseg * p.nchunks;
    if (grid >= (int64_t)INT32_MAX) return false;
    const dim3 gd((unsigned)grid), bd(512);
    if (p.g2) DC_LAUNCH((k_dw_h2w<true>), gd, bd, 0, hs, p);
    else DC_LAUNCH((k_dw_h2w<false>), gd, bd, 0, hs, p);
    return true;
}

struct TransposeParams {
    const float *w[kMaxSeg];
    float *wt;
    int64_t Fi, Fo;
    int nseg;
};

__global__ void __launch_bounds__(256)
k_transpose_w(TransposeParams p) {
    __shared__ float tile[32][33];
    const int64_t tf = (p.Fi + 31) / 32, to = (p.Fo + 31) / 32;
    const int64_t b = blockIdx.x;
    const int s = (int)(b / (tf * to));
    const int64_t o0 = ((b % (tf * to)) / tf) * 32, f0 = (b % tf) * 32;
    const int tx = threadIdx.x & 31, ty = threadIdx.x >> 5;
    for (int i = ty; i < 32; i += 8) {
        const int64_t o = o0 + i, f = f0 + tx;
        tile[i][tx] = (o < p.Fo && f < p.Fi) ? p.w[s][o * p.Fi + f] : 0.f;
    }
    __syncthreads();
    float *dst = p.wt + (int64_t)s * p.Fi * p.Fo;
    for (int i = ty; i < 32; i += 8) {
        const int64_t f = f0 + i, o = o0 + tx;
        if (f < p.Fi && o < p.Fo) dst[f * p.Fo + o] = tile[tx][i];
    }
}

void transpose_weights_launch(const float *const *ws, int nseg, int64_t Fo, int64_t Fi, float *wt,
                              hipStream_t hs) {
    TransposeParams t{};
    for (int s = 0; s < nseg; ++s) t.w[s] = ws[s];
    t.wt = wt, t.Fi = Fi, t.Fo = Fo, t.nseg = nseg;
    const int64_t tiles = ((Fi + 31) / 32) * ((Fo + 31) / 32) * nseg;
    DC_LAUNCH(k_transpose_w, dim3((unsigned)tiles), dim3(256), 0, hs, t);
}

static inline bool al16(const void *q) { return ((uintptr_t)q & 15) == 0; }

bool fwd_split_launch(const FwdParams &p, int mb, int np, hipStream_t hs) {
    if (np != 6 && np != 3 && np != 1 && np != 2) return false;
    if (np == 2 && (!p.h2.a_rowmax || !p.h2.b_rowmax)) return false;
    if (p.Fi % BK != 0 || p.Fi < BK) return false;
    for (int s = 0; s < p.nseg; ++s)
        if (!al16(p.x[s].p) || !al16(p.w[s].p) || p.x[s].ld % 4 != 0 || p.x[s].ld != p.x[0].ld)
            return false;
    const int64_t grid = ((p.N + 64 * mb - 1) / (64 * mb)) * ((p.Fo + BN - 1) / BN);
    const dim3 gd((unsigned)grid), bd(256);
#define DC_L(MB_, NP_) DC_LAUNCH((k_fwd_split<MB_, NP_>), gd, bd, 0, hs, p)
    if (mb == 2) { if (np == 6) DC_L(2, 6); else if (np == 3) DC_L(2, 3); else if (np == 2) DC_L(2, 2); else DC_L(2, 1); }
    else { if (np == 6) DC_L(1, 6); else if (np == 3) DC_L(1, 3); else if (np == 2) DC_L(1, 2); else DC_L(1, 1); }
#undef DC_L
    return true;
}

bool dx_split_eligible(const DxParams &p) {
    if (p.Fo % BK != 0 || p.Fo < BK || p.Fi % 4 != 0 || !al16(p.g.p) || p.g.ld % 4 != 0) return false;
    if (p.has_mask && (!al16(p.mask.p) || p.mask.ld % 4 != 0)) return false;
    return true;
}

bool dx_split_launch(DxParams p, float *wt, int mb, int np, hipStream_t hs) {
    if (!dx_split_eligible(p) || !al16(wt) || (np != 6 && np != 3 && np != 1 && np != 2)) return false;
    if (np == 2 && (!p.h2.b_rowmax || !p.h2.a_rowmax)) return false;
    TransposeParams t{};
    for (int s = 0; s < p.nseg; ++s) t.w[s] = p.w[s].p;
    t.wt = wt, t.Fi = p.Fi, t.Fo = p.Fo, t.nseg = p.nseg;
    const int64_t tiles = ((p.Fi + 31) / 32) * ((p.Fo + 31) / 32) * p.nseg;
    DC_LAUNCH(k_transpose_w, dim3((unsigned)tiles), dim3(256), 0, hs, t);
    for (int s = 0; s < p.nseg; ++s) p.w[s] = Mat{wt + (int64_t)s * p.Fi * p.Fo, p.Fo};
    const int64_t grid = ((p.N + 64 * mb - 1) / (64 * mb)) * ((p.Fi + BN - 1) / BN) * p.nseg;
    const dim3 gd((unsigned)grid), bd(256);
#define DC_L(MB_, M_)                                                                 \
    do {                                                                              \
        if (np == 6) DC_LAUNCH((k_dx_split<MB_, M_, 6>), gd, bd, 0, hs, p);       \
        else if (np == 3) DC_LAUNCH((k_dx_split<MB_, M_, 3>), gd, bd, 0, hs, p);  \
        else if (np == 2) DC_LAUNCH((k_dx_split<MB_, M_, 2>), gd, bd, 0, hs, p);  \
        else DC_LAUNCH((k_dx_split<MB_, M_, 1>), gd, bd, 0, hs, p);               \
    } while (0)
    if (mb == 2) { if (p.has_mask) DC_L(2, true); else DC_L(2, false); }
    else { if (p.has_mask) DC_L(1, true); else DC_L(1, false); }
#undef DC_L
    return true;
}

bool dw_split_launch(const DwParams &p, int mb, int np, hipStream_t hs) {
    if (np != 6 && np != 3 && np != 1 && np != 2) return false;
    if (np == 2 && (!p.h2.a_rowmax || !p.h2.b_rowmax)) return false;
    if (p.N % BK != 0 || p.chunk_rows % BK != 0 || p.Fi % 4 != 0 || p.Fo % 4 != 0 || p.Fi < 4 ||
        p.Fo < 4 || !al16(p.g.p) || p.g.ld % 4 != 0)
        return false;
    if (p.has_mask && (!al16(p.mask.p) || p.mask.ld % 4 != 0)) return false;
    for (int s = 0; s < p.nseg; ++s)
        if (!al16(p.x[s].p) || p.x[s].ld % 4 != 0) return false;
    if (np == 2 && dw_h2w_launch(p, hs)) return true;
    const int64_t tiles = ((p.Fo + 64 * mb - 1) / (64 * mb)) * ((p.Fi + BN - 1) / BN);
    const dim3 gd((unsigned)(tiles * p.nseg * p.nchunks)), bd(256);
#define DC_L(MB_, M_)                                                                 \
    do {                                                                              \
        if (np == 6) DC_LAUNCH((k_dw_split<MB_, M_, 6>), gd, bd, 0, hs, p);       \
        else if (np == 3) DC_LAUNCH((k_dw_split<MB_, M_, 3>), gd, bd, 0, hs, p);  \
        else if (np == 2) DC_LAUNCH((k_dw_split<MB_, M_, 2>), gd, bd, 0, hs, p);  \
        else DC_LAUNCH((k_dw_split<MB_, M_, 1>), gd, bd, 0, hs, p);               \
    } while (0)
    if (mb == 2) { if (p.has_mask) DC_L(2, true); else DC_L(2, false); }
    else { if (p.has_mask) DC_L(1, true); else DC_L(1, false); }
#undef DC_L
    return true;
}

}
```

deformcontact_amd/ops.py:

```python
from __future__ import annotations

import ctypes
import os
from typing import List, Optional

import torch

from . import _lib
from .deferred import resolve
from .graph import GraphIndex, SortedAdjacency, _require_cuda, current_stream_ptr


def _rowmajor(t: torch.Tensor, what: str) -> int:
    if t.dim() != 2 or t.dtype != torch.float32:
        raise ValueError(f"{what}: expected a 2-D float32 tensor, got {tuple(t.shape)} {t.dtype}")
    if t.size(1) > 1 and t.stride(1) != 1:
        raise ValueError(f"{what}: innermost dimension must be contiguous")
    return t.stride(0) if t.size(0) > 1 else max(t.stride(0), t.size(1))


def hop(adj: SortedAdjacency, x: torch.Tensor, out: Optional[torch.Tensor] = None,
        addend: Optional[torch.Tensor] = None, weighted: bool = True,
        rowmax: Optional[torch.Tensor] = None, rowmax_mode: int = 0) -> torch.Tensor:
    _require_cuda(x, "x")
    n, f = x.shape
    if adj.ptr.numel() != n + 1:
        raise ValueError(f"hop: x has {n} rows but the graph has {adj.ptr.numel() - 1} nodes")
    if out is None:
        out = torch.empty((n, f), dtype=torch.float32, device=x.device)
    ldx, ldy = _rowmajor(x, "x"), _rowmajor(out, "out")
    if out.shape != x.shape:
        raise ValueError("hop: out shape mismatch")
    lda = 0
    if addend is not None:
        if addend.shape != x.shape:
            raise ValueError("hop: addend shape mismatch")
        lda = _rowmajor(addend, "addend")
    w = adj.w if weighted else None
    if rowmax is not None and (rowmax.dtype != torch.float32 or rowmax.numel() != n or not rowmax.is_contiguous()):
        raise ValueError("hop: rowmax must be a contiguous float32 [N] tensor")
    if adj.row_offset:
        if rowmax is not None:
            rc = _lib.lib().dc_spmm_f32_rowmax_window(
                adj.ptr.data_ptr(), adj.other.data_ptr(), w.data_ptr() if w is not None else None,
                x.data_ptr(), ldx, addend.data_ptr() if addend is not None else None, lda,
                out.data_ptr(), ldy, n, f, rowmax.data_ptr(), int(rowmax_mode), int(adj.row_offset),
                current_stream_ptr(x.device))
            _lib.check(rc, "dc_spmm_f32_rowmax_window")
            return out
        rc = _lib.lib().dc_spmm_f32_window(
            adj.ptr.data_ptr(), adj.other.data_ptr(), w.data_ptr() if w is not None else None,
            x.data_ptr(), ldx, addend.data_ptr() if addend is not None else None, lda,
            out.data_ptr(), ldy, n, f, int(adj.row_offset), current_stream_ptr(x.device))
        _lib.check(rc, "dc_spmm_f32_window")
        return out
    if rowmax is not None:
        rc = _lib.lib().dc_spmm_f32_rowmax(
            adj.ptr.data_ptr(), adj.other.data_ptr(), w.data_ptr() if w is not None else None,
            x.data_ptr(), ldx, addend.data_ptr() if addend is not None else None, lda,
            out.data_ptr(), ldy, n, f, rowmax.data_ptr(), int(rowmax_mode),
            current_stream_ptr(x.device))
        _lib.check(rc, "dc_spmm_f32_rowmax")
        return out
    rc = _lib.lib().dc_spmm_f32(
        adj.ptr.data_ptr(), adj.other.data_ptr(), w.data_ptr() if w is not None else None,
        x.data_ptr(), ldx, addend.data_ptr() if addend is not None else None, lda,
        out.data_ptr(), ldy, n, f, current_stream_ptr(x.device))
    _lib.check(rc, "dc_spmm_f32")
    return out


def weight_rowmax(ws) -> torch.Tensor:
    fo, fi = ws[0].shape
    out = torch.empty(fo, dtype=torch.float32, device=ws[0].device)
    rc = _lib.lib().dc_tag_weight_rowmax(_ptr_array(ws), len(ws), fo, fi, out.data_ptr(),
                                         current_stream_ptr(out.device))
    _lib.check(rc, "dc_tag_weight_rowmax")
    return out


def rowabsmax(x: torch.Tensor) -> torch.Tensor:
    _require_cuda(x, "x")
    n, f = x.shape
    out = torch.empty(n, dtype=torch.float32, device=x.device)
    rc = _lib.lib().dc_rowabsmax_f32(x.data_ptr(), _rowmajor(x, "x"), n, f, out.data_ptr(),
                                     current_stream_ptr(x.device))
    _lib.check(rc, "dc_rowabsmax_f32")
    return out


def _rowmajor_any(t: torch.Tensor, what: str, dtypes) -> int:
    if t.dim() != 2 or t.dtype not in dtypes:
        raise ValueError(f"{what}: expected a 2-D tensor of {dtypes}, got {tuple(t.shape)} {t.dtype}")
    if t.size(1) > 1 and t.stride(1) != 1:
        raise ValueError(f"{what}: innermost dimension must be contiguous")
    return t.stride(0) if t.size(0) > 1 else max(t.stride(0), t.size(1))


def hop_bf16(adj: SortedAdjacency, x: torch.Tensor, out: Optional[torch.Tensor] = None,
             addend: Optional[torch.Tensor] = None, weighted: bool = True,
             out_dtype: torch.dtype = torch.bfloat16) -> torch.Tensor:
    _require_cuda(x, "x")
    if out_dtype not in (torch.bfloat16, torch.float32):
        raise ValueError("hop_bf16: out_dtype must be bfloat16 or float32")
    ldx = _rowmajor_any(x, "x", (torch.bfloat16,))
    n, f = x.shape
    if adj.ptr.numel() != n + 1:
        raise ValueError(f"hop_bf16: x has {n} rows but the graph has {adj.ptr.numel() - 1} nodes")
    if out is None:
        out = torch.empty((n, f), dtype=out_dtype, device=x.device)
    if out.shape != x.shape:
        raise ValueError("hop_bf16: out shape mismatch")
    ldy = _rowmajor_any(out, "out", (out_dtype,))
    lda = 0
    if addend is not None:
        if addend.shape != x.shape:
            raise ValueError("hop_bf16: addend shape mismatch")
        lda = _rowmajor_any(addend, "addend", (out_dtype,))
    w = adj.w if weighted else None
    rc = _lib.lib().dc_spmm_bf16(
        adj.ptr.data_ptr(), adj.other.data_ptr(), w.data_ptr() if w is not None else None,
        x.data_ptr(), ldx, addend.data_ptr() if addend is not None else None, lda,
        out.data_ptr(), ldy, n, f, 1 if out_dtype == torch.float32 else 0,
        current_stream_ptr(x.device))
    _lib.check(rc, "dc_spmm_bf16")
    return out


class _HopFn(torch.autograd.Function):

    @staticmethod
    def forward(ctx, g: GraphIndex, x: torch.Tensor, weighted: bool):
        ctx.g, ctx.weighted = g, weighted
        return hop(g.fwd, x.contiguous(), weighted=weighted)

    @staticmethod
    def backward(ctx, gy):
        return None, hop(ctx.g.bwd, gy.contiguous(), weighted=ctx.weighted), None


def propagate(g: GraphIndex, x: torch.Tensor, weighted: bool = True) -> torch.Tensor:
    return _HopFn.apply(g, resolve(x), weighted)


def _ptr_array(tensors):
    return (ctypes.c_void_p * len(tensors))(*[t.data_ptr() for t in tensors])


def _i64_array(vals):
    return (ctypes.c_int64 * len(vals))(*vals)


MAX_SEG = 4

DIRECT_PARAM_GRAD = True


DENSE_SPLIT_BF16 = os.environ.get("DC_DENSE_SPLIT", "1") != "0"

DENSE_PRODUCTS = 6


NARROW_FWD = os.environ.get("DC_NARROW_FWD", "1") != "0"

DENSE_F16X2 = os.environ.get("DC_DENSE_F16X2", "1") != "0"


HOP_CHAIN = os.environ.get("DC_HOP_CHAIN", "1") != "0"
_CHAIN_MAX_NODES = None


def hop_chain_eligible(g, adj: SortedAdjacency, slab: torch.Tensor, f: int, k: int) -> bool:
    global _CHAIN_MAX_NODES
    seg = getattr(g, "_layout", None)
    if not HOP_CHAIN or seg is None or k < 1 or f % 32 != 0 or adj.row_offset:
        return False
    if _CHAIN_MAX_NODES is None:
        _CHAIN_MAX_NODES = int(_lib.lib().dc_hop_chain_max_nodes())
    return (0 < g._seg_max_nodes <= _CHAIN_MAX_NODES and slab.dtype == torch.float32 and slab.dim() == 2
            and slab.stride(1) == 1 and slab.stride(0) % 4 == 0 and slab.data_ptr() % 16 == 0
            and adj.ptr.numel() == slab.size(0) + 1)


HOP_CHAIN_GCN = True


def hop_chain(g, adj: SortedAdjacency, slab: torch.Tensor, f: int, k: int, weighted: bool = True,
              rowmax: Optional[torch.Tensor] = None, rowmax_mode: int = 0, src_block: int = 0, direction: int = 1) -> None:
    nptr, nseg = g._layout
    w = adj.w if weighted else None
    deg = g.fwd.ptr if (HOP_CHAIN_GCN and w is not None and g.normalize and not g.self_loops) else None
    rc = _lib.lib().dc_hop_chain_f32(
        adj.ptr.data_ptr(), adj.other.data_ptr(), w.data_ptr() if w is not None else None,
        deg.data_ptr() if deg is not None else None, adj.other.numel(),
        nptr, nseg, slab.data_ptr(), slab.stride(0), slab.size(0), f, k, int(src_block), int(direction),
        rowmax.data_ptr() if rowmax is not None else None, int(rowmax_mode), current_stream_ptr(slab.device))
    _lib.check(rc, "dc_hop_chain_f32")


DEBUG_TAP = None
DEBUG_CHAIN = None
DEBUG_CHAIN_PRE = None


def chained_hops(g: GraphIndex, slab: torch.Tensor, f: int, k: int, backward: bool,
                 rowmax: Optional[torch.Tensor] = None, transposed: bool = False,
                 rowmax_has_block0: bool = False, rowmax_zeroed: bool = False) -> None:
    if k == 0:
        return
    adj = g.bwd if (backward or transposed) else g.fwd
    blocks = [slab[:, j * f:(j + 1) * f] for j in range(k + 1)]
    if backward:
        for j in range(k, 0, -1):
            hop(adj, blocks[j], out=blocks[j - 1], addend=blocks[j - 1], weighted=g.normalize)
    elif hop_chain_eligible(g, adj, slab, f, k):
        if DEBUG_CHAIN_PRE is not None:
            DEBUG_CHAIN_PRE(g, adj, slab, f, k, transposed)
        hop_chain(g, adj, slab, f, k, weighted=g.normalize, rowmax=rowmax,
                  rowmax_mode=2 if rowmax_has_block0 else (3 if rowmax_zeroed else 1))
        if DEBUG_CHAIN is not None:
            DEBUG_CHAIN(g, adj, slab, f, k, transposed)
    else:
        for j in range(k):
            hop(adj, blocks[j], out=blocks[j + 1], weighted=g.normalize, rowmax=rowmax,
                rowmax_mode=1 if (j == 0 and not rowmax_has_block0) else 2)


HOP_CACHE = os.environ.get("DC_HOP_CACHE", "1") != "0"
_HOP_CACHE_ENTRIES = 2


def _hop_cache_key(x: torch.Tensor, k: int, wpad: int, want_rowmax: bool):
    return (x.data_ptr(), tuple(x.shape), tuple(x.stride()), int(k), int(wpad), bool(want_rowmax))


def _hop_cache_get(g, key, x, dev):
    cache = getattr(g, "_hop_cache", None)
    if not cache or key not in cache:
        return None
    from .graph import capture_id
    cid = capture_id(dev)
    slab, rowmax, ecid, _ref, version = cache[key]
    if version == x._version and (ecid == cid or (cid != 0 and g._static_ok)):
        return slab, rowmax
    return None


def _hop_cache_put(g, key, x, slab, rowmax, dev):
    from .graph import capture_id
    cache = g.__dict__.setdefault("_hop_cache", {})
    if key not in cache:
        while len(cache) >= _HOP_CACHE_ENTRIES:
            cache.pop(next(iter(cache)))
    cache[key] = (slab, rowmax, capture_id(dev), x, x._version)


FUSED_PACK = os.environ.get("DC_FUSED_PACK", "1") != "0"


def _build_input_slab(g: GraphIndex, x: torch.Tensor, k: int, want_rowmax: bool, into=None):
    n, fi = x.shape
    concat, width, wpad = tag_slab_geometry(fi, k)
    dev = x.device
    slab = into[0] if into is not None else _alloc_slab(n, wpad, dev)
    xin = x if (x.dim() == 2 and x.stride(1) == 1) else x.contiguous()
    adj = g.fwd if (g is not None and k >= 1) else None
    if (FUSED_PACK and adj is not None and not want_rowmax and fi <= 32 and not adj.row_offset and g.normalize
            and adj.ptr.numel() == n + 1):
        _lib.check(_lib.lib().dc_spmm_f32_pack(adj.ptr.data_ptr(), adj.other.data_ptr(), adj.w.data_ptr(),
                                               xin.data_ptr(), xin.stride(0), slab.data_ptr(), slab.stride(0), n, fi,
                                               width, wpad, current_stream_ptr(dev)), "dc_spmm_f32_pack")
        for j in range(1, k):
            hop(adj, slab[:, j * fi:(j + 1) * fi], out=slab[:, (j + 1) * fi:(j + 2) * fi], weighted=True)
        return slab, None
    _lib.check(_lib.lib().dc_tag_pack_input(xin.data_ptr(), xin.stride(0), slab.data_ptr(), slab.stride(0), n,
                                            fi, width, wpad, current_stream_ptr(dev)),
               "dc_tag_pack_input")
    rowmax = None
    if want_rowmax:
        rowmax = into[1] if into is not None else torch.empty(n, dtype=torch.float32, device=dev)
    chained_hops(g, slab, fi, k, backward=False, rowmax=rowmax)
    return slab, rowmax




def _tag_uses_h2(fi: int, k: int, fo: Optional[int] = None) -> bool:
    concat, _, wpad = tag_slab_geometry(fi, k)
    ok = (DENSE_F16X2 and DENSE_SPLIT_BF16 and DENSE_PRODUCTS == 6 and not concat and fi % 16 == 0 and wpad % 4 == 0)
    if k >= 1:
        return ok
    return ok and fo is not None and fi >= 128 and fi % 32 == 0 and fo % 16 == 0 and fo >= 64


def precompute_input_hops(g: GraphIndex, x: torch.Tensor, k: int = 3) -> None:
    _require_cuda(x, "x")
    if not HOP_CACHE or k < 1 or x.dtype != torch.float32 or x.dim() != 2:
        return
    fi = x.size(1)
    want = _tag_uses_h2(fi, k)
    key = _hop_cache_key(x, k, tag_slab_geometry(fi, k)[2], want)
    if _hop_cache_get(g, key, x, x.device) is None:
        slab, rowmax = _build_input_slab(g, x, k, want)
        _hop_cache_put(g, key, x, slab, rowmax, x.device)


def _grad_sink(p):
    ref = getattr(p, "_dc_grad_sink", None)
    bucket = ref() if ref is not None else None
    if bucket is None or not p.requires_grad:
        return None
    g = p.grad
    if (g is None or g.dtype != torch.float32 or not g.is_contiguous() or g.device != p.device
            or g.shape != p.shape or not bucket.owns(p, g)):
        return None
    return bucket


def tag_slab_geometry(fi: int, k: int):
    concat = (fi * (k + 1) <= 128) or (fi % 16 != 0)
    width = (k + 1) * fi
    wpad = (width + 15) // 16 * 16 if concat else width
    return concat, width, wpad


_SLAB_TAG = "_dc_hop_slab"

SLAB_PAD = 64


def _alloc_slab(n: int, wpad: int, dev, tag=None) -> torch.Tensor:
    pad = SLAB_PAD if (SLAB_PAD > 0 and (wpad * 4) % 1024 == 0) else 0
    base = torch.empty((n, wpad + pad), dtype=torch.float32, device=dev)
    if tag is not None:
        setattr(base, _SLAB_TAG, tag)
    return base[:, :wpad] if pad else base


_SLAB_CLAIMED = "_dc_hop_slab_claimed"


def _as_slab_block0(x: torch.Tensor, n: int, fi: int, wpad: int):
    base = x._base
    if (base is not None and getattr(base, _SLAB_TAG, None) == (n, fi, wpad)
            and not getattr(base, _SLAB_CLAIMED, False)
            and base.dim() == 2 and base.size(0) == n and base.size(1) >= wpad
            and base.is_contiguous() and x.stride() == (base.size(1), 1) and x.shape == (n, fi)
            and x.data_ptr() == base.data_ptr() and base.dtype == torch.float32):
        setattr(base, _SLAB_CLAIMED, True)
        return base[:, :wpad] if base.size(1) > wpad else base
    return None


def _h2_weight_prep(L, ws, k: int, fo: int, fi: int, want_t: bool, dev, st, zero: Optional[torch.Tensor] = None):
    width = (k + 1) * fi
    wmax = torch.empty(fo, dtype=torch.float32, device=dev)
    wimg = torch.empty((fo, width), dtype=torch.float32, device=dev)
    wt = wt_rowmax = None
    if want_t:
        wt = torch.empty((fi, (k + 1) * fo), dtype=torch.float32, device=dev)
        wt_rowmax = torch.empty(fi, dtype=torch.float32, device=dev)
    _lib.check(L.dc_tag_weight_prep_zero(_ptr_array(ws), k + 1, fo, fi, wmax.data_ptr(), wimg.data_ptr(),
                                         wt.data_ptr() if wt is not None else None,
                                         wt_rowmax.data_ptr() if wt is not None else None,
                                         zero.data_ptr() if zero is not None else None,
                                         zero.numel() if zero is not None else 0, st), "dc_tag_weight_prep")
    return wmax, wimg, wt, wt_rowmax


DW_LAST_STREAMS: set = set()
DW_POSITION = {"unlisted": "mid", "listed": "last"}


def _dw_position(dev) -> str:
    return DW_POSITION["listed" if current_stream_ptr(dev) in DW_LAST_STREAMS else "unlisted"]


class _TagConvFn(torch.autograd.Function):

    @staticmethod
    def forward(ctx, g: GraphIndex, x: torch.Tensor, bias: Optional[torch.Tensor], relu: bool,
                next_geom, *weights):
        n, fi = x.shape
        k = len(weights) - 1
        fo = weights[0].size(0)
        if k + 1 > MAX_SEG:
            raise NotImplementedError(f"TAGConv K={k} > {MAX_SEG - 1} is not supported by the fused dense block")
        dev = x.device
        concat, width, wpad = tag_slab_geometry(fi, k)
        slab = _as_slab_block0(x, n, fi, wpad)
        if (slab is None and k == 0 and wpad == fi and x.is_contiguous() and x.data_ptr() % 16 == 0):
            slab = x
        L = _lib.lib()
        st = current_stream_ptr(dev)
        six = next_geom is SIX_PRODUCTS
        if six:
            next_geom = None
        h2 = _tag_uses_h2(fi, k, None if six else fo)
        rowmax = None
        prepped = None
        if slab is None:
            key = None
            if HOP_CACHE and g is not None and k >= 1 and not ctx.needs_input_grad[1]:
                key = _hop_cache_key(x, k, wpad, h2)
                hit = _hop_cache_get(g, key, x, dev)
                if hit is not None:
                    slab, rowmax = hit
            if slab is None:
                slab, rowmax = _build_input_slab(g, x, k, h2)
                if key is not None:
                    _hop_cache_put(g, key, x, slab, rowmax, dev)
        else:
            rowmax = torch.empty(n, dtype=torch.float32, device=dev) if h2 else None
            zeroed = False
            if h2 and g is not None and hop_chain_eligible(g, g.fwd, slab, fi, k):
                prepped = _h2_weight_prep(L, [w.contiguous() for w in weights], k, fo, fi,
                                          ctx.needs_input_grad[1] and fo % 16 == 0, dev, st, zero=rowmax)
                zeroed = True
            chained_hops(g, slab, fi, k, backward=False, rowmax=rowmax, rowmax_zeroed=zeroed)
        if h2 and k == 0:
            rowmax = torch.empty(n, dtype=torch.float32, device=dev)
            _lib.check(L.dc_rowabsmax_f32(slab.data_ptr(), slab.stride(0), n, fi, rowmax.data_ptr(), st), "dc_rowabsmax_f32")
        blocks = [slab[:, j * fi:(j + 1) * fi] for j in range(k + 1)]
        narrow = (concat and NARROW_FWD and DENSE_SPLIT_BF16 and DENSE_PRODUCTS == 6
                  and bool(L.dc_tag_linear_fwd_narrow_ok(fi, k + 1, wpad, fo)))
        if concat and narrow:
            ws = [w.contiguous() for w in weights]
            xs, ldxs, fi_eff = [slab], [slab.stride(0)], wpad
        elif concat:
            wc = [w.contiguous() for w in weights]
            wcat = torch.empty((fo, wpad), dtype=torch.float32, device=dev)
            _lib.check(L.dc_tag_pack_weights(_ptr_array(wc), k + 1, wcat.data_ptr(), fo, fi, wpad,
                                             st), "dc_tag_pack_weights")
            ws = [wcat]
            xs, ldxs, fi_eff = [slab], [slab.stride(0)], wpad
        else:
            ws = [w.contiguous() for w in weights]
            xs, ldxs, fi_eff = blocks, [slab.stride(0)] * (k + 1), fi
        if isinstance(next_geom, OutInto):
            out = next_geom.view
            if out.shape != (n, fo) or out.stride(1) != 1 or out.dtype != torch.float32 or out.device != dev:
                raise ValueError("tag_conv: out_into view has the wrong shape / layout")
        elif next_geom is not None:
            next_width, next_wpad = next_geom
            nxt = _alloc_slab(n, next_wpad, dev, tag=(n, fo, next_wpad))
            if next_wpad > next_width:
                nxt[:, next_width:].zero_()
            out = nxt[:, :fo]
        else:
            out = torch.empty((n, fo), dtype=torch.float32, device=dev)
        ldo = out.stride(0)
        b = bias.contiguous() if bias is not None else None
        args = (_ptr_array(xs), _i64_array(ldxs), _ptr_array(ws), len(xs),
                b.data_ptr() if b is not None else None, int(relu), out.data_ptr(), ldo, n, fi_eff, fo)
        wmax = wt = wt_rowmax = None
        if h2:
            if prepped is None:
                prepped = _h2_weight_prep(L, ws, k, fo, fi, ctx.needs_input_grad[1] and fo % 16 == 0, dev, st)
            wmax, wimg, wt, wt_rowmax = prepped
            rc = L.dc_tag_linear_fwd_h2p(slab.data_ptr(), slab.stride(0), wimg.data_ptr(),
                                         b.data_ptr() if b is not None else None, int(relu),
                                         out.data_ptr(), ldo, n, width, fo,
                                         rowmax.data_ptr(), wmax.data_ptr(), None, 0, st)
        elif narrow:
            rc = L.dc_tag_linear_fwd_narrow(slab.data_ptr(), slab.stride(0), _ptr_array(ws), k + 1, fi,
                                            b.data_ptr() if b is not None else None, int(relu), out.data_ptr(), ldo, n,
                                            wpad, fo, st)
        elif DENSE_SPLIT_BF16:
            rc = L.dc_tag_linear_fwd_split(*args, DENSE_PRODUCTS, st)
        else:
            rc = L.dc_tag_linear_fwd(*args, st)
        _lib.check(rc, "dc_tag_linear_fwd")
        ctx.g, ctx.k, ctx.fi, ctx.fo, ctx.has_bias, ctx.relu, ctx.concat = \
            g, k, fi, fo, bias is not None, relu, concat
        ctx.narrow = narrow
        ctx.params, ctx.bias_param = weights, bias
        ctx.h2 = h2
        ctx.save_for_backward(slab, out if relu else None, rowmax, wt, wt_rowmax, *ws)
        return out

    @staticmethod
    def backward(ctx, gout):
        slab, out, xrowmax, wt, wt_rowmax, *ws = ctx.saved_tensors
        g, k, fi, fo, concat = ctx.g, ctx.k, ctx.fi, ctx.fo, ctx.concat
        L = _lib.lib()
        if gout.stride(1) != 1 or gout.stride(0) % 4 != 0 or gout.data_ptr() % 16 != 0:
            gout = gout.contiguous()
        ldg = gout.stride(0)
        n = slab.size(0)
        dev = slab.device
        st = current_stream_ptr(dev)
        need_x, need_b = ctx.needs_input_grad[1], ctx.has_bias and ctx.needs_input_grad[2]
        need_w = any(ctx.needs_input_grad[5:])
        mask_ptr = out.data_ptr() if out is not None else None
        ldm = out.stride(0) if out is not None else fo
        wpad, lds = slab.size(1), slab.stride(0)
        if concat:
            xs, ldxs, fi_eff, nseg = [slab], [lds], wpad, 1
        else:
            xs = [slab[:, j * fi:(j + 1) * fi] for j in range(k + 1)]
            ldxs, fi_eff, nseg = [lds] * (k + 1), fi, k + 1

        h2 = ctx.h2
        gws: List[Optional[torch.Tensor]] = [None] * (k + 1)
        gb = gx = None
        g_ptr, g_ld, g_rowmax = gout.data_ptr(), ldg, None

        dw_done = not (need_w or need_b)

        def weight_gradients():
            nonlocal gws, gb
            if need_w or need_b:
                sinks = [_grad_sink(p) for p in ctx.params] + \
                    ([_grad_sink(ctx.bias_param)] if ctx.has_bias else [])
                direct = (DIRECT_PARAM_GRAD and not torch.is_grad_enabled()
                          and all(ctx.needs_input_grad[5:]) and (need_b or not ctx.has_bias)
                          and sinks[0] is not None and all(b is sinks[0] for b in sinks))
                if direct:
                    outs = [p.grad for p in ctx.params]
                    gb_out = ctx.bias_param.grad if ctx.has_bias else None
                else:
                    outs = [torch.empty((fo, fi), dtype=torch.float32, device=dev) for _ in range(k + 1)]
                    gb_out = torch.empty(fo, dtype=torch.float32, device=dev) if need_b else None
                nbytes = L.dc_tag_linear_bwd_dw_workspace_bytes(n, fi_eff, fo, nseg)
                scratch = torch.empty(nbytes, dtype=torch.uint8, device=dev)
                args = (g_ptr, g_ld, mask_ptr, ldm, _ptr_array(xs), _i64_array(ldxs), nseg,
                        _ptr_array(outs), k + 1, fi, gb_out.data_ptr() if gb_out is not None else None,
                        int(direct), scratch.data_ptr(), nbytes, n, fi_eff, fo)
                if g_rowmax is not None and n % 16 == 0:
                    rc = L.dc_tag_linear_bwd_dw_h2(*args, g_rowmax.data_ptr(), xrowmax.data_ptr(), st)
                elif DENSE_SPLIT_BF16:
                    rc = L.dc_tag_linear_bwd_dw_split(*args, DENSE_PRODUCTS, st)
                else:
                    rc = L.dc_tag_linear_bwd_dw(*args, st)
                _lib.check(rc, "dc_tag_linear_bwd_dw")
                if direct:
                    sinks[0].note_direct_write(torch.cuda.current_stream(dev))
                else:
                    gws = [outs[j] if ctx.needs_input_grad[5 + j] else None for j in range(k + 1)]
                    gb = gb_out

        if h2 and fo % 16 == 0 and fo % 4 == 0:
            gwid = (k + 1) * fo
            gslab = _alloc_slab(n, gwid, dev)
            gld = gslab.stride(0)
            g_rowmax = torch.empty(n, dtype=torch.float32, device=dev)
            hop_rowmax = torch.empty(n, dtype=torch.float32, device=dev) if need_x else None
            _lib.check(L.dc_tag_mask_grad(gout.data_ptr(), ldg, mask_ptr, ldm, gslab.data_ptr(), gld, n,
                                          fo, g_rowmax.data_ptr(),
                                          hop_rowmax.data_ptr() if need_x else None, st),
                       "dc_tag_mask_grad")
            g_ptr, g_ld, mask_ptr = gslab.data_ptr(), gld, None
            dw_pos = _dw_position(dev)
            if need_x and dw_pos == "first":
                weight_gradients()
                dw_done = True
            if need_x:
                chained_hops(g, gslab, fo, k, backward=False, rowmax=hop_rowmax, transposed=True,
                             rowmax_has_block0=True)
                if dw_pos == "mid" and not dw_done:
                    weight_gradients()
                    dw_done = True
                if wt is None:
                    wt = torch.empty((fi, gwid), dtype=torch.float32, device=dev)
                    wt_rowmax = torch.empty(fi, dtype=torch.float32, device=dev)
                    _lib.check(L.dc_tag_weight_prep(_ptr_array(ws), k + 1, fo, fi,
                                                    torch.empty(fo, device=dev).data_ptr(), None,
                                                    wt.data_ptr(), wt_rowmax.data_ptr(), st),
                               "dc_tag_weight_prep")
                gx = torch.empty((n, fi), dtype=torch.float32, device=dev)
                rc = L.dc_tag_linear_fwd_h2p(gslab.data_ptr(), gld, wt.data_ptr(), None, 0, gx.data_ptr(),
                                             fi, n, gwid, fi, hop_rowmax.data_ptr(), wt_rowmax.data_ptr(),
                                             None, 0, st)
                _lib.check(rc, "dc_tag_linear_fwd_h2 (dX)")
                if DEBUG_TAP is not None:
                    DEBUG_TAP(f"bwd{fi}x{fo}.hop_rowmax", hop_rowmax)
                    DEBUG_TAP(f"bwd{fi}x{fo}.g_rowmax", g_rowmax)
                    if os.environ.get("HUNT_TAP_ADJ") == "1":
                        for nm, t in (("bwd.ptr", g.bwd.ptr), ("bwd.other", g.bwd.other), ("bwd.w", g.bwd.w),
                                      ("fwd.ptr", g.fwd.ptr)):
                            DEBUG_TAP(f"bwd{fi}x{fo}.adj.{nm}", t)
                    if os.environ.get("HUNT_TAP_BIG") == "1":
                        DEBUG_TAP(f"bwd{fi}x{fo}.gx", gx)
                        DEBUG_TAP(f"bwd{fi}x{fo}.gslab", gslab)
                need_x = False

        if not dw_done:
            weight_gradients()

        if need_x:
            if concat and ctx.narrow:
                wcat = torch.empty((fo, wpad), dtype=torch.float32, device=dev)
                _lib.check(L.dc_tag_pack_weights(_ptr_array(ws), k + 1, wcat.data_ptr(), fo, fi, wpad, st),
                           "dc_tag_pack_weights")
                ws = [wcat]
            gslab = _alloc_slab(n, wpad, dev)
            gblocks = [gslab[:, j * fi:(j + 1) * fi] for j in range(k + 1)]
            gxs = [gslab] if concat else gblocks
            ldxs = [gslab.stride(0)] * len(ldxs)
            if DENSE_SPLIT_BF16:
                wsb = L.dc_tag_linear_bwd_dx_split_workspace_bytes(fi_eff, fo, nseg)
                wsx = torch.empty(wsb, dtype=torch.uint8, device=dev)
                rc = L.dc_tag_linear_bwd_dx_split(g_ptr, g_ld, mask_ptr, ldm, _ptr_array(ws), nseg,
                                                  _ptr_array(gxs), _i64_array(ldxs), wsx.data_ptr(), wsb,
                                                  n, fi_eff, fo, DENSE_PRODUCTS, st)
            else:
                rc = L.dc_tag_linear_bwd_dx(g_ptr, g_ld, mask_ptr, ldm, _ptr_array(ws), nseg,
                                            _ptr_array(gxs), _i64_array(ldxs), n, fi_eff, fo, st)
            _lib.check(rc, "dc_tag_linear_bwd_dx")
            chained_hops(g, gslab, fi, k, backward=True)
            gx = gblocks[0]
        return (None, gx, gb, None, None, *gws)


class OutInto:

    def __init__(self, view: torch.Tensor):
        self.view = view


_MERGED_TAG = "_dc_merged_slab"


def alloc_merged_slab(mg: GraphIndex, fi: int, k: int, dev) -> torch.Tensor:
    concat, width, wpad = tag_slab_geometry(fi, k)
    if concat:
        raise ValueError("alloc_merged_slab: wide layers only (Fi a multiple of 16, (K+1)*Fi > 128)")
    n = mg.num_nodes
    slab = _alloc_slab(n, wpad, dev, tag=("merged", n, fi, wpad, tuple(mg.row_beg), tuple(mg.rows)))
    base = slab._base if slab._base is not None else slab
    setattr(base, _SLAB_TAG, ("merged", n, fi, wpad, tuple(mg.row_beg), tuple(mg.rows)))
    ends = list(mg.row_beg[1:]) + [n]
    for r0, rows, r1 in zip(mg.row_beg, mg.rows, ends):
        if r0 + rows < r1:
            slab[r0 + rows:r1, :fi].zero_()
    return slab


def merged_slab_part(slab: torch.Tensor, mg: GraphIndex, g: int, fi: int) -> torch.Tensor:
    r0 = mg.row_beg[g]
    return slab[r0:r0 + mg.rows[g], :fi]


def _as_merged_slab(xs, mg: GraphIndex, fi: int, wpad: int):
    base = xs[0]._base
    tag = ("merged", mg.num_nodes, fi, wpad, tuple(mg.row_beg), tuple(mg.rows))
    if base is None or getattr(base, _SLAB_TAG, None) != tag or base.dim() != 2 or not base.is_contiguous():
        return None
    ld = base.size(1)
    for g, x in enumerate(xs):
        if (x._base is not base or x.shape != (mg.rows[g], fi) or x.stride() != (ld, 1)
                or x.data_ptr() != base.data_ptr() + 4 * ld * mg.row_beg[g]):
            return None
    return base[:, :wpad] if ld > wpad else base


def grouped_eligible(fi: int, fo: int, k: int) -> bool:
    return (_tag_uses_h2(fi, k) and fi == 256 and fo % 128 == 0 and fo % 16 == 0
            and ((k + 1) * fi) % 32 == 0 and ((k + 1) * fo) % 32 == 0)


def _vp_array(ptrs):
    return (ctypes.c_void_p * len(ptrs))(*ptrs)


class _TagConvGroupedFn(torch.autograd.Function):

    @staticmethod
    def forward(ctx, mg: GraphIndex, relu: bool, next_geom, ngroups: int, *args):
        xs = args[:ngroups]
        per = (len(args) - ngroups) // ngroups
        k = per - 2
        biases = [args[ngroups + g * per] for g in range(ngroups)]
        weights = [list(args[ngroups + g * per + 1: ngroups + (g + 1) * per]) for g in range(ngroups)]
        fo, fi = weights[0][0].shape
        dev = xs[0].device
        n = mg.num_nodes
        concat, width, wpad = tag_slab_geometry(fi, k)
        if not _tag_uses_h2(fi, k) or width % 32 != 0 or any(b is None for b in biases) != all(b is None for b in biases):
            raise NotImplementedError("tag_conv_grouped: wide fp16x2 layers only, bias on all groups or none")
        L = _lib.lib()
        st = current_stream_ptr(dev)
        slab = _as_merged_slab(xs, mg, fi, wpad)
        if slab is None:
            slab = alloc_merged_slab(mg, fi, k, dev)
            for g, x in enumerate(xs):
                merged_slab_part(slab, mg, g, fi).copy_(x)
        rowmax = torch.empty(n, dtype=torch.float32, device=dev)
        chained_hops(mg, slab, fi, k, backward=False, rowmax=rowmax)
        need_x = any(ctx.needs_input_grad[4:4 + ngroups])
        wmax = torch.empty((ngroups, fo), dtype=torch.float32, device=dev)
        wimg = torch.empty((ngroups, fo, width), dtype=torch.float32, device=dev)
        wt = wt_rowmax = None
        if need_x and fo % 16 == 0:
            wt = torch.empty((ngroups, fi, (k + 1) * fo), dtype=torch.float32, device=dev)
            wt_rowmax = torch.empty((ngroups, fi), dtype=torch.float32, device=dev)
        wcs = [[w.contiguous() for w in ws] for ws in weights]
        _lib.check(L.dc_tag_grouped_weight_prep(
            _vp_array([w.data_ptr() for ws in wcs for w in ws]), ngroups, k + 1, fo, fi,
            _vp_array([wmax[g].data_ptr() for g in range(ngroups)]),
            _vp_array([wimg[g].data_ptr() for g in range(ngroups)]),
            _vp_array([wt[g].data_ptr() for g in range(ngroups)]) if wt is not None else None,
            _vp_array([wt_rowmax[g].data_ptr() for g in range(ngroups)]) if wt is not None else None, st),
            "dc_tag_grouped_weight_prep")
        if isinstance(next_geom, tuple):
            nxt = alloc_merged_slab(mg, fo, next_geom[0], dev)
            out = nxt[:, :fo]
        else:
            out = torch.empty((n, fo), dtype=torch.float32, device=dev)
        bcs = [b.contiguous() if b is not None else None for b in biases]
        row_beg, rows = _i64_array(mg.row_beg), _i64_array(mg.rows)
        _lib.check(L.dc_tag_grouped_fwd_h2p(
            slab.data_ptr(), slab.stride(0), ngroups, row_beg, rows, n,
            _vp_array([wimg[g].data_ptr() for g in range(ngroups)]),
            _vp_array([b.data_ptr() if b is not None else None for b in bcs]), int(relu),
            out.data_ptr(), out.stride(0), width, fo, rowmax.data_ptr(),
            _vp_array([wmax[g].data_ptr() for g in range(ngroups)]), st), "dc_tag_grouped_fwd_h2p")
        ctx.mg, ctx.k, ctx.fi, ctx.fo, ctx.relu, ctx.ngroups = mg, k, fi, fo, relu, ngroups
        ctx.params, ctx.bias_params = weights, biases
        ctx.save_for_backward(slab, out if relu else None, rowmax, wt, wt_rowmax)
        outs = tuple(out[r0:r0 + r] for r0, r in zip(mg.row_beg, mg.rows))
        return outs

    @staticmethod
    def backward(ctx, *gouts):
        slab, out, xrowmax, wt, wt_rowmax = ctx.saved_tensors
        mg, k, fi, fo, ngroups = ctx.mg, ctx.k, ctx.fi, ctx.fo, ctx.ngroups
        L = _lib.lib()
        dev = slab.device
        st = current_stream_ptr(dev)
        n = mg.num_nodes
        per = k + 2
        need_x = any(ctx.needs_input_grad[4:4 + ngroups])
        need_p = any(ctx.needs_input_grad[4 + ngroups:])
        gs = []
        for g, go in enumerate(gouts):
            if go is None:
                go = torch.zeros((mg.rows[g], fo), dtype=torch.float32, device=dev)
            if go.stride(1) != 1 or go.stride(0) % 4 != 0 or go.data_ptr() % 16 != 0:
                go = go.contiguous()
            gs.append(go)
        row_beg, rows = _i64_array(mg.row_beg), _i64_array(mg.rows)
        gwid = (k + 1) * fo
        gslab = _alloc_slab(n, gwid, dev)
        g_rowmax = torch.empty(n, dtype=torch.float32, device=dev)
        hop_rowmax = torch.empty(n, dtype=torch.float32, device=dev) if need_x else None
        _lib.check(L.dc_tag_grouped_mask_grad(
            _vp_array([t.data_ptr() for t in gs]), _i64_array([t.stride(0) for t in gs]), ngroups, row_beg, rows, n,
            out.data_ptr() if out is not None else None, out.stride(0) if out is not None else fo,
            gslab.data_ptr(), gslab.stride(0), fo, g_rowmax.data_ptr(),
            hop_rowmax.data_ptr() if need_x else None, st), "dc_tag_grouped_mask_grad")
        gxs = [None] * ngroups
        if need_x:
            if wt is None:
                raise RuntimeError("tag_conv_grouped: input gradient requested but the forward ran without it")
            chained_hops(mg, gslab, fo, k, backward=False, rowmax=hop_rowmax, transposed=True,
                         rowmax_has_block0=True)
            gx = torch.empty((n, fi), dtype=torch.float32, device=dev)
            _lib.check(L.dc_tag_grouped_fwd_h2p(
                gslab.data_ptr(), gslab.stride(0), ngroups, row_beg, rows, n,
                _vp_array([wt[g].data_ptr() for g in range(ngroups)]), None, 0, gx.data_ptr(), fi, gwid, fi,
                hop_rowmax.data_ptr(), _vp_array([wt_rowmax[g].data_ptr() for g in range(ngroups)]), st),
                "dc_tag_grouped_fwd_h2p (dX)")
            gxs = [gx[r0:r0 + r] if ctx.needs_input_grad[4 + g] else None
                   for g, (r0, r) in enumerate(zip(mg.row_beg, mg.rows))]
        pgrads = [None] * (ngroups * per)
        if need_p:
            has_bias = ctx.bias_params[0] is not None
            flat_params = [p for g in range(ngroups) for p in ([ctx.bias_params[g]] if has_bias else []) + ctx.params[g]]
            sinks = [_grad_sink(p) for p in flat_params]
            all_needed = all(ctx.needs_input_grad[4 + ngroups + g * per + j] for g in range(ngroups)
                             for j in range(per) if (j > 0 or has_bias))
            direct = (DIRECT_PARAM_GRAD and not torch.is_grad_enabled() and all_needed
                      and sinks[0] is not None and all(b is sinks[0] for b in sinks))
            if direct:
                gw_out = [[p.grad for p in ctx.params[g]] for g in range(ngroups)]
                gb_out = [ctx.bias_params[g].grad if has_bias else None for g in range(ngroups)]
            else:
                gw_out = [[torch.empty((fo, fi), dtype=torch.float32, device=dev) for _ in range(k + 1)]
                          for _ in range(ngroups)]
                gb_out = [torch.empty(fo, dtype=torch.float32, device=dev) if has_bias else None
                          for _ in range(ngroups)]
            nbytes = L.dc_tag_grouped_bwd_dw_workspace_bytes(rows, ngroups, fi, fo, k + 1)
            scratch = torch.empty(nbytes, dtype=torch.uint8, device=dev)
            xblocks = [slab[:, j * fi:(j + 1) * fi] for j in range(k + 1)]
            _lib.check(L.dc_tag_grouped_bwd_dw_h2(
                gslab.data_ptr(), gslab.stride(0), _ptr_array(xblocks), _i64_array([slab.stride(0)] * (k + 1)),
                k + 1, ngroups, row_beg, rows, n,
                _vp_array([t.data_ptr() for ws in gw_out for t in ws]),
                _vp_array([t.data_ptr() if t is not None else None for t in gb_out]), int(direct),
                scratch.data_ptr(), nbytes, fi, fo, g_rowmax.data_ptr(), xrowmax.data_ptr(), st),
                "dc_tag_grouped_bwd_dw_h2")
            if direct:
                sinks[0].note_direct_write(torch.cuda.current_stream(dev))
            else:
                for g in range(ngroups):
                    base = g * per
                    if has_bias and ctx.needs_input_grad[4 + ngroups + base]:
                        pgrads[base] = gb_out[g]
                    for j in range(k + 1):
                        if ctx.needs_input_grad[4 + ngroups + base + 1 + j]:
                            pgrads[base + 1 + j] = gw_out[g][j]
        return (None, None, None, None, *gxs, *pgrads)


def tag_conv_grouped(mg: GraphIndex, xs, weights, biases, relu: bool = False, next_k=None):
    flat = []
    xs = [resolve(x) for x in xs]
    for b, ws in zip(biases, weights):
        flat += [b] + list(ws)
    return _TagConvGroupedFn.apply(mg, bool(relu), (int(next_k),) if next_k is not None else None, len(xs),
                                   *xs, *flat)


class _SixProducts:
    """``next_geom`` marker of ``dense_linear(..., six_products=True)``."""


SIX_PRODUCTS = _SixProducts()


def dense_linear(x: torch.Tensor, weight: torch.Tensor, bias: Optional[torch.Tensor] = None,
                 relu: bool = False, six_products: bool = False) -> torch.Tensor:
    return _TagConvFn.apply(None, resolve(x), bias, bool(relu), SIX_PRODUCTS if six_products else None, weight)


def tag_conv(g: GraphIndex, x: torch.Tensor, weights, bias, relu: bool = False,
             next_geom=None) -> torch.Tensor:
    return _TagConvFn.apply(g, resolve(x), bias, bool(relu), next_geom, *weights)


_SLAB_TAG_BF16 = "_dc_hop_slab_bf16"

# ... 372 lines not shown
```

include/deformcontact.h:

```cpp
#ifndef DEFORMCONTACT_H
#define DEFORMCONTACT_H

#include <stdint.h>

#ifdef __cplusplus
extern "C" {
#endif

#define DC_OK 0
#define DC_EINVAL (-1)
#define DC_ELAUNCH (-2)
#define DC_EWORKSPACE (-3)

typedef void *dc_stream_t;

#define DC_MAX_PARTS 4
#define DC_MAX_GROUPS 4
#define DC_GROUP_ALIGN 256

int dc_version(void);
const char *dc_last_error(void);
int64_t dc_stream_capture_id(dc_stream_t stream);

int64_t dc_csr_workspace_bytes(int64_t E, int64_t N);
int dc_csr_build(const int64_t *edge_index, int64_t E, int64_t N, int key_row,
                 int self_loops, int32_t *ptr, int32_t *other, int32_t *perm,
                 const int32_t *deg_ptr, float *w, int32_t *status, void *workspace,
                 int64_t workspace_bytes, dc_stream_t stream);

int64_t dc_graph_workspace_bytes(int64_t E, int64_t N);
int dc_graph_build(const int64_t *edge_index, int64_t E, int64_t N, int self_loops,
                   int32_t *ptr_f, int32_t *other_f, int32_t *perm_f, float *w_f,
                   int32_t *ptr_b, int32_t *other_b, int32_t *perm_b, float *w_b,
                   int32_t *status, void *workspace, int64_t workspace_bytes, dc_stream_t stream);

int dc_graph_build_parts(const int64_t *const *edge_index_parts, const int64_t *E_parts,
                         const int64_t *node_offset_parts, const int64_t *nodes_parts, int nparts,
                         int64_t N, int self_loops,
                         int32_t *ptr_f, int32_t *other_f, int32_t *perm_f, float *w_f,
                         int32_t *ptr_b, int32_t *other_b, int32_t *perm_b, float *w_b,
                         int32_t *status, void *workspace, int64_t workspace_bytes, dc_stream_t stream);

int dc_graph_build_plan(int64_t E, int64_t N, int self_loops, int *bucket_shift, int *buckets);

#define DC_SEG_MAX_NODES 4096
#define DC_SEG_MAX_EDGES 16384
int dc_graph_build_segmented(const int64_t *edge_index, int64_t E, int64_t N,
                             const int64_t *node_ptr_host, const int64_t *edge_ptr_host, int nseg,
                             int32_t *ptr_f, int32_t *other_f, int32_t *perm_f, float *w_f,
                             int32_t *ptr_b, int32_t *other_b, int32_t *perm_b, float *w_b,
                             int32_t *status, dc_stream_t stream);

int dc_morton_codes(const float *pos, int64_t ld, int64_t n, const float *lo_host,
                    const float *inv_extent_host, int64_t *codes, dc_stream_t stream);

int64_t dc_morton_order_workspace_bytes(int64_t n);
int dc_morton_order(const float *pos, int64_t ld, int64_t n, int32_t *perm, int32_t *inv, void *workspace,
                    int64_t workspace_bytes, dc_stream_t stream);
int dc_relabel_edges(const int64_t *ei, int64_t count, const int32_t *inv, int64_t n, int64_t *out,
                     dc_stream_t stream);
int dc_gather_rows(const void *x, int64_t ldx_bytes, const int32_t *idx, void *out, int64_t ldo_bytes, int64_t n,
                   int64_t row_bytes, dc_stream_t stream);

int dc_hash_i64(const int64_t *v, int64_t n, uint64_t *out, dc_stream_t stream);

int dc_spmm_f32(const int32_t *ptr, const int32_t *other, const float *w, const float *x,
                int64_t ldx, const float *addend, int64_t ldadd, float *y, int64_t ldy,
                int64_t N, int64_t F, dc_stream_t stream);

int dc_spmm_f32_pack(const int32_t *ptr, const int32_t *other, const float *w, const float *x, int64_t ldx,
                     float *slab, int64_t lds, int64_t N, int64_t F, int64_t width, int64_t wpad,
                     dc_stream_t stream);

int dc_spmm_f32_window(const int32_t *ptr, const int32_t *other, const float *w, const float *x,
                       int64_t ldx, const float *addend, int64_t ldadd, float *y, int64_t ldy,
                       int64_t N, int64_t F, int64_t row_offset, dc_stream_t stream);
int dc_spmm_f32_rowmax_window(const int32_t *ptr, const int32_t *other, const float *w, const float *x,
                              int64_t ldx, const float *addend, int64_t ldadd, float *y, int64_t ldy,
                              int64_t N, int64_t F, float *rowmax, int mode, int64_t row_offset,
                              dc_stream_t stream);

int dc_spmm_bf16(const int32_t *ptr, const int32_t *other, const float *w, const uint16_t *x,
                 int64_t ldx, const void *addend, int64_t ldadd, void *y, int64_t ldy, int64_t N,
                 int64_t F, int y_is_f32, dc_stream_t stream);

int dc_spmm_f32_rowmax(const int32_t *ptr, const int32_t *other, const float *w, const float *x,
                       int64_t ldx, const float *addend, int64_t ldadd, float *y, int64_t ldy,
                       int64_t N, int64_t F, float *rowmax, int mode, dc_stream_t stream);

int64_t dc_hop_chain_max_nodes(void);
int64_t dc_hop_chain_lds_request(void);
int dc_hop_chain_f32(const int32_t *ptr, const int32_t *other, const float *w, const int32_t *deg_ptr,
                     int64_t cap, const int64_t *node_ptr_host, int nseg, float *slab, int64_t ld, int64_t N,
                     int64_t F, int K, int src_block, int dir, float *rowmax, int mode,
                     dc_stream_t stream);

int dc_tag_linear_fwd_bf16(const uint16_t *a, int64_t lda, const uint16_t *w, const float *bias,
                           int relu, void *out, int64_t ldo, int out_is_bf16, int64_t N, int64_t K,
                           int64_t Fo, dc_stream_t stream);
int dc_tag_mask_grad_bf16(const void *g, int64_t ldg, int g_is_bf16, const void *out_for_mask, int64_t ldo,
                          int mask_is_bf16, uint16_t *gm, int64_t ldgm, int64_t N, int64_t F,
                          dc_stream_t stream);
int64_t dc_tag_linear_bwd_dw_bf16_workspace_bytes(int64_t N, int64_t Fi, int64_t Fo, int nseg);
int dc_tag_linear_bwd_dw_bf16(const uint16_t *g, int64_t ldg, const uint16_t *x, int64_t ldx, int nseg,
                              float *const *gws, float *gbias, int accumulate, void *partials,
                              int64_t partials_bytes, int64_t N, int64_t Fi, int64_t Fo, dc_stream_t stream);
int dc_to_bf16(const float *const *srcs, int nseg, int64_t rows, int64_t cols, int64_t ld_src,
               uint16_t *dst, int64_t ld_dst, dc_stream_t stream);

int64_t dc_contact_loss_workspace_bytes(int64_t N);
int dc_contact_loss(const int32_t *ptr_f, const int32_t *other_f, const int32_t *ptr_b,
                    const int32_t *other_b, const float *pred, int64_t ld_pred, const float *target,
                    int64_t ld_target, int64_t N, int64_t E, float *grad_l1, float *grad_gcl,
                    float *losses , void *workspace, int64_t workspace_bytes,
                    dc_stream_t stream);

#define DC_MAX_SEG 4
int dc_tag_linear_fwd(const float *const *xs, const int64_t *ldxs, const float *const *ws,
                      int nseg, const float *bias, int relu, float *out, int64_t ldo,
                      int64_t N, int64_t Fi, int64_t Fo, dc_stream_t stream);

int dc_tag_linear_bwd_dx(const float *g, int64_t ldg, const float *out_for_mask, int64_t ldo,
                         const float *const *ws, int nseg, float *const *gxs,
                         const int64_t *ldgxs, int64_t N, int64_t Fi, int64_t Fo,
                         dc_stream_t stream);

int dc_tag_linear_fwd_split(const float *const *xs, const int64_t *ldxs, const float *const *ws,
                            int nseg, const float *bias, int relu, float *out, int64_t ldo,
                            int64_t N, int64_t Fi, int64_t Fo, int products, dc_stream_t stream);
int dc_tag_linear_fwd_narrow_ok(int64_t fi, int nseg, int64_t wpad, int64_t Fo);
int dc_tag_linear_fwd_narrow(const float *slab, int64_t ld, const float *const *ws, int nseg, int64_t fi,
                             const float *bias, int relu, float *out, int64_t ldo, int64_t N, int64_t wpad,
                             int64_t Fo, dc_stream_t stream);
int64_t dc_tag_linear_bwd_dx_split_workspace_bytes(int64_t Fi, int64_t Fo, int nseg);
int dc_tag_linear_bwd_dx_split(const float *g, int64_t ldg, const float *out_for_mask,
                               int64_t ldo, const float *const *ws, int nseg, float *const *gxs,
                               const int64_t *ldgxs, void *workspace, int64_t workspace_bytes,
                               int64_t N, int64_t Fi, int64_t Fo, int products, dc_stream_t stream);

int64_t dc_tag_linear_bwd_dw_workspace_bytes(int64_t N, int64_t Fi, int64_t Fo, int nseg);
int dc_tag_linear_bwd_dw(const float *g, int64_t ldg, const float *out_for_mask, int64_t ldo,
                         const float *const *xs, const int64_t *ldxs, int nseg,
                         float *const *gws, int ngw, int64_t gw_cols, float *gbias,
                         int accumulate, void *partials, int64_t partials_bytes, int64_t N,
                         int64_t Fi, int64_t Fo, dc_stream_t stream);
int dc_tag_linear_bwd_dw_split(const float *g, int64_t ldg, const float *out_for_mask,
                               int64_t ldo, const float *const *xs, const int64_t *ldxs, int nseg,
                               float *const *gws, int ngw, int64_t gw_cols, float *gbias,
                               int accumulate, void *partials, int64_t partials_bytes, int64_t N,
                               int64_t Fi, int64_t Fo, int products, dc_stream_t stream);

int dc_tag_linear_fwd_h2(const float *const *xs, const int64_t *ldxs, const float *const *ws,
                         int nseg, const float *bias, int relu, float *out, int64_t ldo, int64_t N,
                         int64_t Fi, int64_t Fo, const float *x_rowmax, const float *w_rowmax,
                         dc_stream_t stream);
int dc_tag_linear_bwd_dx_h2(const float *g, int64_t ldg, const float *out_for_mask, int64_t ldo,
                            const float *const *ws, int nseg, float *const *gxs,
                            const int64_t *ldgxs, void *workspace, int64_t workspace_bytes,
                            int64_t N, int64_t Fi, int64_t Fo, const float *g_rowmax,
                            const float *w_rowmax, dc_stream_t stream);
int dc_tag_linear_bwd_dw_h2(const float *g, int64_t ldg, const float *out_for_mask, int64_t ldo,
                            const float *const *xs, const int64_t *ldxs, int nseg,
                            float *const *gws, int ngw, int64_t gw_cols, float *gbias,
                            int accumulate, void *partials, int64_t partials_bytes, int64_t N,
                            int64_t Fi, int64_t Fo, const float *g_rowmax, const float *x_rowmax,
                            dc_stream_t stream);
int dc_tag_linear_bwd_dw_h2_corr(const float *g, int64_t ldg, const float *g2, const float *g2_coef,
                                 const float *const *xs, const int64_t *ldxs, int nseg, float *const *gws, int ngw,
                                 int64_t gw_cols, int accumulate, void *partials, int64_t partials_bytes, int64_t N,
                                 int64_t Fi, int64_t Fo, const float *g_rowmax, const float *x_rowmax,
                                 dc_stream_t stream);
int dc_tag_mask_grad(const float *g, int64_t ldg, const float *out_for_mask, int64_t ldo, float *gm,
                     int64_t ldgm, int64_t N, int64_t F, float *rowmax_a, float *rowmax_b,
                     dc_stream_t stream);
int dc_tag_transpose_weights(const float *const *ws, int nseg, int64_t Fo, int64_t Fi, float *wt,
                             dc_stream_t stream);
int dc_tag_weight_prep(const float *const *ws, int nseg, int64_t Fo, int64_t Fi, float *w_rowmax,
                       void *w_image, void *wt_image, float *wt_rowmax, dc_stream_t stream);
int dc_tag_weight_prep_zero(const float *const *ws, int nseg, int64_t Fo, int64_t Fi, float *w_rowmax,
                            void *w_image, void *wt_image, float *wt_rowmax, float *zero, int64_t zero_n,
                            dc_stream_t stream);
int64_t dc_tag_linear_fwd_h2p_workspace_bytes(int64_t N, int64_t K, int64_t Fo);
int dc_tag_linear_fwd_h2p(const float *x, int64_t ldx, const void *w_image, const float *bias, int relu,
                          float *out, int64_t ldo, int64_t N, int64_t K, int64_t Fo,
                          const float *x_rowmax, const float *w_rowmax, void *workspace,
                          int64_t workspace_bytes, dc_stream_t stream);
int dc_tag_linear_fwd_h2p_exp(const float *x, int64_t ldx, const void *w_image, float *out, int64_t ldo,
                              int64_t N, int64_t K, int64_t Fo, const float *x_rowmax, const float *w_rowmax,
                              const float *row_lse, int64_t ncols_valid, dc_stream_t stream);
int dc_tag_linear_fwd_h2p_corr(const float *x, int64_t ldx, const float *x2, const float *x2_coef, const void *w_image,
                               float *out, int64_t ldo, int64_t N, int64_t K, int64_t Fo, const float *x_rowmax,
                               const float *w_rowmax, dc_stream_t stream);
int dc_tag_grouped_weight_prep(const float *const *ws, int ngroups, int nseg, int64_t Fo, int64_t Fi,
                               float *const *w_rowmax, void *const *w_image, void *const *wt_image,
                               float *const *wt_rowmax, dc_stream_t stream);
int dc_tag_grouped_fwd_h2p(const float *x, int64_t ldx, int ngroups, const int64_t *row_beg,
                           const int64_t *rows, int64_t N_total, const void *const *w_images,
                           const float *const *biases, int relu, float *out, int64_t ldo, int64_t K,
                           int64_t Fo, const float *x_rowmax, const float *const *w_rowmaxes,
                           dc_stream_t stream);
int dc_tag_grouped_mask_grad(const float *const *g, const int64_t *ldg, int ngroups, const int64_t *row_beg,
                             const int64_t *rows, int64_t N_total, const float *out_for_mask, int64_t ldo,
                             float *gm, int64_t ldgm, int64_t F, float *rowmax_a, float *rowmax_b,
                             dc_stream_t stream);
int64_t dc_tag_grouped_bwd_dw_workspace_bytes(const int64_t *rows, int ngroups, int64_t Fi, int64_t Fo,
                                              int nseg);
int dc_tag_grouped_bwd_dw_h2(const float *g, int64_t ldg, const float *const *xs, const int64_t *ldxs,
                             int nseg, int ngroups, const int64_t *row_beg, const int64_t *rows,
                             int64_t N_total, float *const *gws, float *const *gbias, int accumulate,
                             void *partials, int64_t partials_bytes, int64_t Fi, int64_t Fo,
                             const float *g_rowmax, const float *x_rowmax, dc_stream_t stream);

int64_t dc_generic_dense_launches(int reset);

void dc_kernel_trace(int on);
int64_t dc_kernel_trace_dump(char *buf, int64_t cap);

int dc_rowabsmax_f32(const float *x, int64_t ld, int64_t N, int64_t F, float *rowmax,
                     dc_stream_t stream);
int dc_tag_weight_rowmax(const float *const *ws, int nseg, int64_t Fo, int64_t Fi, float *w_rowmax,
                         dc_stream_t stream);

int dc_invert_perm(const int32_t *perm, const int32_t *ptr_last , int32_t *pos_of,
                   int64_t max_edges, dc_stream_t stream);
int dc_compose_perm(const int32_t *a, const int32_t *b, int32_t *out, const int32_t *count_ptr,
                    int64_t cap, dc_stream_t stream);

int dc_spmm_f32_bias_act(const int32_t *ptr, const int32_t *other, const float *w, const float *x,
                         int64_t ldx, const float *bias, int relu, float *y, int64_t ldy, int64_t N,
                         int64_t F, dc_stream_t stream);
int64_t dc_colsum_workspace_bytes(int64_t N, int64_t F, int nvec);
int dc_mask_colsum_f32(const float *g, int64_t ldg, const float *y_mask, int64_t ldy, float *gm,
                       int64_t ldgm, int64_t N, int64_t F, void *workspace, int64_t workspace_bytes,
                       float *colsum, int accumulate, dc_stream_t stream);
int dc_gat_alpha_fwd(const float *h, int64_t ldh, const float *att_src, const float *att_dst, float *a_src,
                     float *a_dst, int64_t N, int64_t F, dc_stream_t stream);
int dc_gat_alpha_bwd(const float *h, int64_t ldh, const float *ga_src, const float *ga_dst,
                     const float *att_src, const float *att_dst, float *gh, int64_t ldgh, int64_t N,
                     int64_t F, void *workspace, int64_t workspace_bytes, float *g_att_src,
                     float *g_att_dst, int accumulate, dc_stream_t stream);

int dc_gat_edge_softmax_fwd(const int32_t *ptr, const int32_t *other, const float *a_src,
                            const float *a_dst, float slope, float *alpha, int64_t N,
                            dc_stream_t stream);
int dc_gat_edge_softmax_bwd(const int32_t *ptr, const int32_t *other, const float *a_src,
                            const float *a_dst, float slope, const float *alpha,
                            const float *galpha, float *ge, float *g_a_dst, int64_t N,
                            dc_stream_t stream);
int dc_sddmm_f32(const int32_t *ptr, const int32_t *other, const float *g, int64_t ldg,
                 const float *h, int64_t ldh, float *d, int64_t N, int64_t F,
                 dc_stream_t stream);
int dc_segment_sum_f32(const int32_t *ptr, const int32_t *map, const float *v, float *out,
                       int64_t N, dc_stream_t stream);
int dc_gather_f32(const float *v, const int32_t *idx, float *out, const int32_t *count_ptr,
                  int64_t cap, dc_stream_t stream);

int dc_tag_pack_input(const float *x, int64_t ldx, float *slab, int64_t ld_slab, int64_t N,
                      int64_t F, int64_t width, int64_t wpad, dc_stream_t stream);
int dc_tag_pack_weights(const float *const *ws, int nw, float *wcat, int64_t Fo, int64_t fi,
                        int64_t wpad, dc_stream_t stream);

#define DC_ATTN_FLASH_D 256
int dc_attn_flash_prep(void *vt_image, int64_t dv, int64_t nr_padded, const float *k_rowmax, float *k_unscale,
                       dc_stream_t stream);
int dc_attn_flash_fwd(const float *q, int64_t ldq, const float *q_rowmax, const void *k_image,
                      const float *k_unscale, const void *vt_image, const float *vt_rowmax, int64_t ns,
                      int64_t nr, int64_t nr_padded, int64_t d, float *o, int64_t ldo, float *lse,
                      dc_stream_t stream);
int dc_attn_flash_ds(const float *q, int64_t ldq, const float *q_rowmax, const float *go, int64_t ldgo,
                     const float *go_rowmax, const void *k_image, const float *k_unscale, const void *v_image,
                     const float *v_unscale, const float *lse, int64_t ns, int64_t nr, int64_t nr_padded, int64_t d,
                     float *p_out, float *ds_out, int64_t ldp, float *ds_rowmax, const float *delta_in,
                     float *eps_out, dc_stream_t stream);
int dc_attn_softmax_rows(float *s, int64_t ld, int64_t rows, int64_t n, int64_t npad, float *lse,
                         dc_stream_t stream);
int dc_attn_exp_rows(float *s, int64_t ld, int64_t rows, int64_t n, int64_t npad, const float *lse,
                     dc_stream_t stream);
int dc_attn_ds_rows(const float *p, float *dp, int64_t ld, int64_t rows, int64_t npad,
                    const float *delta, float *rowmax, dc_stream_t stream);

#define DC_ADAM_STEP_WORDS 34
int dc_adam_flat(float *p, float *g, float *m, float *v, int64_t n, float *step, float lr,
                 float beta1, float beta2, float eps, int zero_grad, dc_stream_t stream);

#ifdef __cplusplus
}
#endif
#endif
```

Measured before the change: 538.1 M edges/s.

## Prep narrow bf16x3 weight image once and emit ReLU bitmask for dW backward

Adds a small pre-pass kernel that splits the narrow TAGConv weights into bf16 hi/mid/lo planes, already laid out as MFMA fragments, so the narrow forward kernel loads fragments directly. This removes the per-block LDS transpose, the split and two barriers. The forward kernel now also writes a packed ReLU sign bitmask via ballot, and the dW backward reads this bit image instead of the fp32 output to build its mask, cutting mask traffic. The costs are an extra kernel launch and weight-image allocation per call, an extra bit-image write, and disabling the h2w dW path whenever bits are used.

```diff
diff --git a/deformcontact_amd/_lib.py b/deformcontact_amd/_lib.py
--- a/deformcontact_amd/_lib.py
+++ b/deformcontact_amd/_lib.py
@@ -134,6 +134,14 @@
     "dc_tag_linear_fwd_narrow_ok": (c_int, [c_int64, c_int, c_int64, c_int64]),
     "dc_tag_linear_fwd_narrow": (c_int, [_vp, c_int64, POINTER(_vp), c_int, c_int64, _vp, c_int, _vp, c_int64, c_int64,
                                          c_int64, c_int64, _vp]),
+    "dc_tag_narrow_weight_image_bytes": (c_int64, [c_int64]),
+    "dc_tag_narrow_weight_prep": (c_int, [POINTER(_vp), c_int, c_int64, c_int64, c_int64, _vp, c_int64, _vp]),
+    "dc_tag_linear_fwd_narrow_prepped": (c_int, [_vp, c_int64, _vp, _vp, c_int, _vp, c_int64, c_int64, c_int64, c_int64,
+                                                 _vp, _vp]),
+    "dc_tag_linear_bwd_dw_split_bits": (c_int, [_vp, c_int64, _vp, c_int64, _vp, c_int64, POINTER(_vp),
+                                                POINTER(c_int64), c_int, POINTER(_vp), c_int, c_int64,
+                                                _vp, c_int, _vp, c_int64, c_int64, c_int64, c_int64,
+                                                c_int, _vp]),
     "dc_attn_softmax_rows": (c_int, [_vp, c_int64, c_int64, c_int64, c_int64, _vp, _vp]),
     "dc_attn_exp_rows": (c_int, [_vp, c_int64, c_int64, c_int64, c_int64, _vp, _vp]),
     "dc_attn_ds_rows": (c_int, [_vp, _vp, c_int64, c_int64, c_int64, _vp, _vp, _vp]),
diff --git a/deformcontact_amd/csrc/dc_dense.h b/deformcontact_amd/csrc/dc_dense.h
--- a/deformcontact_amd/csrc/dc_dense.h
+++ b/deformcontact_amd/csrc/dc_dense.h
@@ -178,6 +178,8 @@
     H2Scales h2;
     DwGroups grp;
     const float *g2, *g2_coef;
+    const uint32_t *mask_bits;
+    int64_t mask_bits_ld;
 };
 
 
diff --git a/deformcontact_amd/csrc/dc_dense.hip b/deformcontact_amd/csrc/dc_dense.hip
--- a/deformcontact_amd/csrc/dc_dense.hip
+++ b/deformcontact_amd/csrc/dc_dense.hip
@@ -651,8 +651,11 @@
                    int64_t gw_cols, float *gbias, int accumulate, void *partials,
                    int64_t partials_bytes, int64_t N, int64_t Fi, int64_t Fo, dc_stream_t stream,
                    int products, H2Scales h2 = H2Scales{}, const float *g2 = nullptr,
-                   const float *g2_coef = nullptr) {
+                   const float *g2_coef = nullptr, const uint32_t *mask_bits = nullptr, int64_t ldb = 0) {
     DC_REQUIRE(nseg >= 1 && nseg <= kMaxSeg, "dc_tag_linear_bwd_dw: nseg must be 1..%d", kMaxSeg);
+    DC_REQUIRE(!mask_bits || (out_for_mask && ldb >= (Fo + 31) / 32 && ((uintptr_t)mask_bits & 3) == 0),
+               "dc_tag_linear_bwd_dw_split_bits: the bit image needs the fp32 mask beside it, ldb >= Fo / 32 words and "
+               "4-byte alignment");
     DC_REQUIRE(N >= 0 && Fi >= 1 && Fo >= 1, "dc_tag_linear_bwd_dw: bad sizes");
     DC_REQUIRE(g && xs && ldxs && gws && partials && ldg >= Fo,
                "dc_tag_linear_bwd_dw: null pointer / ldg < Fo");
@@ -681,6 +684,7 @@
     dw_plan(N, Fi, Fo, nseg, &p.chunk_rows, &p.nchunks);
     p.N = N, p.Fi = Fi, p.Fo = Fo, p.nseg = nseg;
     p.h2 = h2;
+    p.mask_bits = mask_bits, p.mask_bits_ld = ldb;
     p.partial = (float *)partials;
     const int64_t tail = vec ? N % BK : 0;
     const bool ragged = tail != 0 && N > tail;
@@ -774,6 +778,19 @@
                "dc_tag_linear_bwd_dw_split: products must be 6, 3 or 1");
     return dw_impl(g, ldg, out_for_mask, ldo, xs, ldxs, nseg, gws, ngw, gw_cols, gbias, accumulate,
                    partials, partials_bytes, N, Fi, Fo, stream, products);
+}
+
+extern "C" int dc_tag_linear_bwd_dw_split_bits(const float *g, int64_t ldg, const float *out_for_mask, int64_t ldo,
+                                               const uint32_t *mask_bits, int64_t ldb, const float *const *xs,
+                                               const int64_t *ldxs, int nseg, float *const *gws, int ngw,
+                                               int64_t gw_cols, float *gbias, int accumulate, void *partials,
+                                               int64_t partials_bytes, int64_t N, int64_t Fi, int64_t Fo,
+                                               int products, dc_stream_t stream) {
+    DC_REQUIRE(products == 6 || products == 3 || products == 1,
+               "dc_tag_linear_bwd_dw_split_bits: products must be 6, 3 or 1");
+    DC_REQUIRE(mask_bits, "dc_tag_linear_bwd_dw_split_bits: null bit image");
+    return dw_impl(g, ldg, out_for_mask, ldo, xs, ldxs, nseg, gws, ngw, gw_cols, gbias, accumulate,
+                   partials, partials_bytes, N, Fi, Fo, stream, products, H2Scales{}, nullptr, nullptr, mask_bits, ldb);
 }
 
 
diff --git a/deformcontact_amd/csrc/dc_dense_narrow.hip b/deformcontact_amd/csrc/dc_dense_narrow.hip
--- a/deformcontact_amd/csrc/dc_dense_narrow.hip
+++ b/deformcontact_amd/csrc/dc_dense_narrow.hip
@@ -10,22 +10,27 @@
 using nb_bf16x8 = __attribute__((ext_vector_type(8))) __bf16;
 using nb_f32x4 = __attribute__((ext_vector_type(4))) float;
 
+constexpr int kNarrowFo = 256;
+constexpr int kNarrowTR = 32;
+
+constexpr int64_t narrow_image_bytes(int ks) { return (int64_t)4 * 2 * ks * 3 * 64 * 16; }
+
+struct NarrowPrepParams {
+    const float *w[kMaxSeg];
+    int nseg, fi;
+    nb_bf16x8 *img;
+};
+
 struct NarrowParams {
     const float *x;
     int64_t ld;
-    const float *w[kMaxSeg];
-    int nseg, fi;
+    const nb_bf16x8 *img;
     const float *bias;
     float *out;
+    uint32_t *bits;
     int64_t ldo, N;
     int relu, ntiles;
 };
-
-constexpr int kNarrowFo = 256;
-
-__device__ __forceinline__ void nb_lds_barrier() {
-    asm volatile("s_waitcnt lgkmcnt(0)\n\ts_barrier" ::: "memory");
-}
 
 __device__ __forceinline__ void nb_split1(float x, __bf16 &hi, __bf16 &mid, __bf16 &lo) {
     hi = (__bf16)x;
@@ -35,19 +40,43 @@
     lo = (__bf16)r2;
 }
 
-template <int KS, int MB>
+template <int KS>
+__global__ void __launch_bounds__(256)
+k_narrow_wprep(NarrowPrepParams p) {
+    const int t = blockIdx.x * 256 + threadIdx.x;
+    const int j = t & 7, lane = (t >> 3) & 63, ks = (t >> 9) % KS, wb = (t >> 9) / KS;
+    if (wb >= 8) return;
+    const int o = 32 * wb + (lane & 31), k = 16 * ks + 8 * (lane >> 5) + j;
+    float v = 0.f;
+    if (k < p.nseg * p.fi) {
+        const int s = k / p.fi;
+        v = p.w[s][o * p.fi + (k - s * p.fi)];
+    }
+    __bf16 hi, mid, lo;
+    nb_split1(v, hi, mid, lo);
+    __bf16 *dst = reinterpret_cast<__bf16 *>(p.img + ((wb * KS + ks) * 3) * 64 + lane) + j;
+    dst[0] = hi;
+    dst[64 * 8] = mid;
+    dst[128 * 8] = lo;
+}
+
+__device__ __forceinline__ void nb_lds_barrier() {
+    asm volatile("s_waitcnt lgkmcnt(0)\n\ts_barrier" ::: "memory");
+}
+
+template <int KS>
 __global__ void __launch_bounds__(256)
 k_fwd_narrow(NarrowParams p) {
-    constexpr int TR = 32 * MB;
+    constexpr int TR = kNarrowTR;
     constexpr int SROWA = KS * 96 + 16;
     constexpr int PPR = 4 * KS;
     constexpr int TP = TR * PPR, NV = (TP + 255) / 256;
-    constexpr int KP = 16 * KS;
     constexpr int kOffStage = ((TR * SROWA + 1023) / 1024) * 1024;
-    constexpr int kLdsTiles = kOffStage + TR * 1024, kLdsW = kNarrowFo * (KP + 4) * 4;
-    __shared__ __attribute__((aligned(1024))) char lds[kLdsTiles > kLdsW ? kLdsTiles : kLdsW];
+    constexpr int kOffBits = kOffStage + TR * 1024;
+    __shared__ __attribute__((aligned(1024))) char lds[kOffBits + TR * (kNarrowFo / 32) * 4];
     char *const sA = lds;
     float *const so = reinterpret_cast<float *>(lds + kOffStage);
+    uint32_t *const sbits = reinterpret_cast<uint32_t *>(lds + kOffBits);
     const int wid = __builtin_amdgcn_readfirstlane((int)(threadIdx.x >> 6)), lane = threadIdx.x & 63;
     const int c = lane & 31, h = lane >> 5;
 
@@ -68,61 +97,28 @@
     int t = blockIdx.x;
     if (t < p.ntiles) load_tile(t);
 
-    constexpr int WROW = KP + 4;
+    nb_bf16x8 fb[2][KS][3];
     {
-        float *wi = reinterpret_cast<float *>(lds);
-        const int width = p.nseg * p.fi, per4 = kNarrowFo * p.fi / 4;
-        constexpr int MAXQ = 8;
-        nb_f32x4 wv[kMaxSeg][MAXQ];
-#pragma unroll
-        for (int s = 0; s < kMaxSeg; ++s)
-#pragma unroll
-            for (int j = 0; j < MAXQ; ++j) {
-                const int q = (int)threadIdx.x + 256 * j;
-                if (!(DC_NARROW_ABL & 2) && s < p.nseg && q < per4) wv[s][j] = *reinterpret_cast<const nb_f32x4 *>(p.w[s] + 4 * q);
-            }
-#pragma unroll
-        for (int s = 0; s < kMaxSeg; ++s)
-#pragma unroll
-            for (int j = 0; j < MAXQ; ++j) {
-                const int q = (int)threadIdx.x + 256 * j;
-                if (!(DC_NARROW_ABL & 2) && s < p.nseg && q < per4) {
-                    int o = (4 * q) / p.fi, f = 4 * q - o * p.fi;
-#pragma unroll
-                    for (int i = 0; i < 4; ++i) {
-                        wi[o * WROW + s * p.fi + f] = wv[s][j][i];
-                        if (++f == p.fi) f = 0, ++o;
+        const nb_bf16x8 *wf = p.img + (int64_t)wid * (2 * KS * 3 * 64) + lane;
+#pragma unroll
+        for (int nb = 0; nb < 2; ++nb)
+#pragma unroll
+            for (int ks = 0; ks < KS; ++ks)
+#pragma unroll
+                for (int pl = 0; pl < 3; ++pl) {
+                    if (DC_NARROW_ABL & 2) {
+                        const __bf16 v = (__bf16)(float)(nb + ks + pl);
+                        fb[nb][ks][pl] = nb_bf16x8{v, v, v, v, v, v, v, v};
+                    } else {
+                        fb[nb][ks][pl] = wf[((nb * KS + ks) * 3 + pl) * 64];
                     }
                 }
-            }
-        const int padw = KP - width;
-        for (int e = threadIdx.x; e < kNarrowFo * padw; e += 256) {
-            const int o = e / padw, f = e - o * padw;
-            wi[o * WROW + width + f] = 0.f;
-        }
-    }
-    __syncthreads();
-    nb_bf16x8 fb[2][KS][3];
-#pragma unroll
-    for (int nb = 0; nb < 2; ++nb) {
-        const float *wr = reinterpret_cast<const float *>(lds) + (64 * wid + 32 * nb + c) * WROW + 8 * h;
-#pragma unroll
-        for (int ks = 0; ks < KS; ++ks) {
-            const nb_f32x4 v0 = *reinterpret_cast<const nb_f32x4 *>(wr + 16 * ks);
-            const nb_f32x4 v1 = *reinterpret_cast<const nb_f32x4 *>(wr + 16 * ks + 4);
-#pragma unroll
-            for (int j = 0; j < 8; ++j) {
-                __bf16 hi, mid, lo;
-                nb_split1(j < 4 ? v0[j] : v1[j - 4], hi, mid, lo);
-                fb[nb][ks][0][j] = hi, fb[nb][ks][1][j] = mid, fb[nb][ks][2][j] = lo;
-            }
-        }
-    }
-    __syncthreads();
+    }
     float bcol[2];
 #pragma unroll
     for (int nb = 0; nb < 2; ++nb) bcol[nb] = p.bias ? p.bias[64 * wid + 32 * nb + c] : 0.f;
     const bool relu = p.relu != 0;
+    const bool bits = p.bits != nullptr;
 
     auto store_tile = [&]() {
 #pragma unroll
@@ -151,6 +147,10 @@
             const nb_f32x4 v = *reinterpret_cast<const nb_f32x4 *>(so + r * 256 + 4 * lane);
             if (row < p.N && (!(DC_NARROW_ABL & 4) || v[0] == 12345.678f)) *reinterpret_cast<nb_f32x4 *>(p.out + row * p.ldo + 4 * lane) = v;
         }
+        if (bits) {
+            const int64_t row = row0 + (threadIdx.x >> 3);
+            if (row < p.N) p.bits[row0 * (kNarrowFo / 32) + threadIdx.x] = sbits[threadIdx.x];
+        }
     };
     int64_t prev_row0 = -1;
     for (; t < p.ntiles; t += gridDim.x) {
@@ -159,57 +159,97 @@
         if (prev_row0 >= 0) store_rows(prev_row0);
         if (t + (int)gridDim.x < p.ntiles) load_tile(t + gridDim.x);
         nb_lds_barrier();
-        f32x16 acc[MB][2];
-#pragma unroll
-        for (int mb = 0; mb < MB; ++mb)
-#pragma unroll
-            for (int nb = 0; nb < 2; ++nb)
-#pragma unroll
-                for (int i = 0; i < 16; ++i) acc[mb][nb][i] = 0.f;
+        f32x16 acc[2];
+#pragma unroll
+        for (int nb = 0; nb < 2; ++nb)
+#pragma unroll
+            for (int i = 0; i < 16; ++i) acc[nb][i] = 0.f;
         constexpr int HI = 0, MID = 1, LO = 2;
         constexpr int pa6[6] = {LO, HI, MID, MID, HI, HI}, pb6[6] = {HI, LO, MID, HI, MID, HI};
 #pragma unroll
         for (int ks = 0; ks < KS; ++ks) {
-            nb_bf16x8 fa[MB][3];
-#pragma unroll
-            for (int mb = 0; mb < MB; ++mb)
-#pragma unroll
-                for (int pl = 0; pl < 3; ++pl)
-                    fa[mb][pl] = *reinterpret_cast<const nb_bf16x8 *>(sA + (mb * 32 + c) * SROWA + ks * 96 + pl * 32 + h * 16);
+            nb_bf16x8 fa[3];
+#pragma unroll
+            for (int pl = 0; pl < 3; ++pl)
+                fa[pl] = *reinterpret_cast<const nb_bf16x8 *>(sA + c * SROWA + ks * 96 + pl * 32 + h * 16);
 #pragma unroll
             for (int tt = 0; tt < 6; ++tt)
 #pragma unroll
-                for (int mb = 0; mb < MB; ++mb)
-#pragma unroll
-                    for (int nb = 0; nb < 2; ++nb)
-                        if (!(DC_NARROW_ABL & 1))
-                            acc[mb][nb] = __builtin_amdgcn_mfma_f32_32x32x16_bf16(fa[mb][pa6[tt]], fb[nb][ks][pb6[tt]], acc[mb][nb], 0, 0, 0);
-                        else
-                            acc[mb][nb][tt] += (float)fa[mb][pa6[tt]][0] * (float)fb[nb][ks][pb6[tt]][0];
-        }
-#pragma unroll
-        for (int mb = 0; mb < MB; ++mb)
-#pragma unroll
-            for (int nb = 0; nb < 2; ++nb)
-#pragma unroll
-                for (int r = 0; r < 16; ++r) {
-                    float v = acc[mb][nb][r] + bcol[nb];
-                    if (relu) v = fmaxf(v, 0.f);
-                    if (!(DC_NARROW_ABL & 16) || r == 0)
-                        so[(mb * 32 + (r & 3) + 8 * (r >> 2) + 4 * h) * 256 + 64 * wid + 32 * nb + c] = v;
+                for (int nb = 0; nb < 2; ++nb)
+                    if (!(DC_NARROW_ABL & 1))
+                        acc[nb] = __builtin_amdgcn_mfma_f32_32x32x16_bf16(fa[pa6[tt]], fb[nb][ks][pb6[tt]], acc[nb], 0, 0, 0);
+                    else
+                        acc[nb][tt] += (float)fa[pa6[tt]][0] * (float)fb[nb][ks][pb6[tt]][0];
+        }
+        uint32_t myw = 0;
+#pragma unroll
+        for (int nb = 0; nb < 2; ++nb)
+#pragma unroll
+            for (int r = 0; r < 16; ++r) {
+                float v = acc[nb][r] + bcol[nb];
+                if (relu) v = fmaxf(v, 0.f);
+                if (!(DC_NARROW_ABL & 16) || r == 0)
+                    so[((r & 3) + 8 * (r >> 2) + 4 * h) * 256 + 64 * wid + 32 * nb + c] = v;
+                if (bits) {
+                    const uint64_t b = __ballot(v > 0.f);
+                    if (c == 16 * nb + r) myw = (uint32_t)(h ? (b >> 32) : b);
                 }
+            }
+        if (bits) {
+            const int r = c & 15;
+            sbits[((r & 3) + 8 * (r >> 2) + 4 * h) * (kNarrowFo / 32) + 2 * wid + (c >> 4)] = myw;
+        }
         nb_lds_barrier();
         prev_row0 = row0;
     }
     if (prev_row0 >= 0) store_rows(prev_row0);
+}
+
+template <int KS>
+static void narrow_prep_launch(const NarrowPrepParams &p, hipStream_t hs) {
+    DC_LAUNCH((k_narrow_wprep<KS>), dim3(16 * KS), dim3(256), 0, hs, p);
 }
 
 template <int KS>
 static void narrow_launch(const NarrowParams &p0, hipStream_t hs) {
     NarrowParams p = p0;
-    p.ntiles = (int)((p.N + 31) / 32);
+    p.ntiles = (int)((p.N + kNarrowTR - 1) / kNarrowTR);
     const unsigned grid = (unsigned)(p.ntiles < 256 ? p.ntiles : 256);
-    DC_LAUNCH((k_fwd_narrow<KS, 1>), dim3(grid), dim3(256), 0, hs, p);
+    DC_LAUNCH((k_fwd_narrow<KS>), dim3(grid), dim3(256), 0, hs, p);
+}
+
+static int narrow_prep(const float *const *ws, int nseg, int64_t fi, int64_t wpad, void *img, hipStream_t hs) {
+    NarrowPrepParams q{};
+    for (int s = 0; s < nseg; ++s) {
+        DC_REQUIRE(ws[s], "dc_tag_narrow_weight_prep: null weight segment %d", s);
+        q.w[s] = ws[s];
+    }
+    q.nseg = nseg, q.fi = (int)fi, q.img = reinterpret_cast<nb_bf16x8 *>(img);
+    switch (wpad) {
+    case 96: narrow_prep_launch<6>(q, hs); break;
+    case 112: narrow_prep_launch<7>(q, hs); break;
+    default: narrow_prep_launch<8>(q, hs); break;
+    }
+    return DC_OK;
+}
+
+static int narrow_fwd(const float *slab, int64_t ld, const void *img, const float *bias, int relu, float *out, int64_t ldo,
+                      int64_t N, int64_t wpad, uint32_t *bits, hipStream_t hs) {
+    DC_REQUIRE(slab && img && out && ld >= wpad && ldo >= kNarrowFo, "dc_tag_linear_fwd_narrow: null pointer / short leading "
+               "dimension");
+    DC_REQUIRE(ld % 4 == 0 && ldo % 4 == 0 && ((uintptr_t)slab & 15) == 0 && ((uintptr_t)out & 15) == 0 &&
+                   ((uintptr_t)img & 15) == 0 && ((uintptr_t)bits & 3) == 0,
+               "dc_tag_linear_fwd_narrow: rows of the slab and of the output and the weight image must be 16-byte aligned");
+    DC_REQUIRE(N < ((int64_t)1 << 31) - 64, "dc_tag_linear_fwd_narrow: too many rows");
+    NarrowParams p{};
+    p.x = slab, p.ld = ld, p.img = reinterpret_cast<const nb_bf16x8 *>(img), p.bias = bias, p.out = out, p.bits = bits;
+    p.ldo = ldo, p.N = N, p.relu = relu;
+    switch (wpad) {
+    case 96: narrow_launch<6>(p, hs); break;
+    case 112: narrow_launch<7>(p, hs); break;
+    default: narrow_launch<8>(p, hs); break;
+    }
+    return DC_OK;
 }
 
 }
@@ -219,6 +259,36 @@
 extern "C" int dc_tag_linear_fwd_narrow_ok(int64_t fi, int nseg, int64_t wpad, int64_t Fo) {
     return (Fo == kNarrowFo && nseg >= 1 && nseg <= kMaxSeg && fi >= 1 && fi <= 32 && nseg * fi <= wpad &&
             (wpad == 96 || wpad == 112 || wpad == 128)) ? 1 : 0;
+}
+
+extern "C" int64_t dc_tag_narrow_weight_image_bytes(int64_t wpad) {
+    if (wpad != 96 && wpad != 112 && wpad != 128) return DC_EINVAL;
+    return narrow_image_bytes((int)(wpad / 16));
+}
+
+extern "C" int dc_tag_narrow_weight_prep(const float *const *ws, int nseg, int64_t fi, int64_t wpad, int64_t Fo, void *img,
+                                         int64_t img_bytes, dc_stream_t stream) {
+    DC_REQUIRE(dc_tag_linear_fwd_narrow_ok(fi, nseg, wpad, Fo),
+               "dc_tag_narrow_weight_prep: needs Fo = 256, a padded reduction of 96 / 112 / 128 >= nseg * fi (got Fo=%lld "
+               "wpad=%lld nseg=%d fi=%lld)", (long long)Fo, (long long)wpad, nseg, (long long)fi);
+    DC_REQUIRE(ws && img && ((uintptr_t)img & 15) == 0 && img_bytes >= dc_tag_narrow_weight_image_bytes(wpad),
+               "dc_tag_narrow_weight_prep: image missing, misaligned or too small");
+    const int rc = narrow_prep(ws, nseg, fi, wpad, img, (hipStream_t)stream);
+    if (rc != DC_OK) return rc;
+    return check_launch("dc_tag_narrow_weight_prep");
+}
+
+extern "C" int dc_tag_linear_fwd_narrow_prepped(const float *slab, int64_t ld, const void *img, const float *bias, int relu,
+                                                float *out, int64_t ldo, int64_t N, int64_t wpad, int64_t Fo,
+                                                uint32_t *relu_bits, dc_stream_t stream) {
+    DC_REQUIRE(Fo == kNarrowFo && (wpad == 96 || wpad == 112 || wpad == 128),
+               "dc_tag_linear_fwd_narrow_prepped: needs Fo = 256 and wpad = 96 / 112 / 128 (got Fo=%lld wpad=%lld)",
+               (long long)Fo, (long long)wpad);
+    DC_REQUIRE(N >= 0, "dc_tag_linear_fwd_narrow_prepped: negative N");
+    if (N == 0) return DC_OK;
+    const int rc = narrow_fwd(slab, ld, img, bias, relu, out, ldo, N, wpad, relu_bits, (hipStream_t)stream);
+    if (rc != DC_OK) return rc;
+    return check_launch("dc_tag_linear_fwd_narrow_prepped");
 }
 
 extern "C" int dc_tag_linear_fwd_narrow(const float *slab, int64_t ld, const float *const *ws, int nseg, int64_t fi,
@@ -229,21 +299,15 @@
                "nseg=%d fi=%lld)", (long long)Fo, (long long)wpad, nseg, (long long)fi);
     DC_REQUIRE(N >= 0, "dc_tag_linear_fwd_narrow: negative N");
     if (N == 0) return DC_OK;
-    DC_REQUIRE(slab && ws && out && ld >= wpad && ldo >= Fo, "dc_tag_linear_fwd_narrow: null pointer / short leading dimension");
-    DC_REQUIRE(ld % 4 == 0 && ldo % 4 == 0 && ((uintptr_t)slab & 15) == 0 && ((uintptr_t)out & 15) == 0,
-               "dc_tag_linear_fwd_narrow: rows of the slab and of the output must be 16-byte aligned");
-    DC_REQUIRE(N < ((int64_t)1 << 31) - 64, "dc_tag_linear_fwd_narrow: too many rows");
-    NarrowParams p{};
-    p.x = slab, p.ld = ld, p.nseg = nseg, p.fi = (int)fi, p.bias = bias, p.out = out, p.ldo = ldo, p.N = N, p.relu = relu;
-    for (int s = 0; s < nseg; ++s) {
-        DC_REQUIRE(ws[s], "dc_tag_linear_fwd_narrow: null weight segment %d", s);
-        p.w[s] = ws[s];
-    }
+    DC_REQUIRE(ws, "dc_tag_linear_fwd_narrow: null weight array");
     hipStream_t hs = (hipStream_t)stream;
-    switch (wpad) {
-    case 96: narrow_launch<6>(p, hs); break;
-    case 112: narrow_launch<7>(p, hs); break;
-    default: narrow_launch<8>(p, hs); break;
-    }
+    void *img = nullptr;
+    DC_REQUIRE(hipMallocAsync(&img, (size_t)dc_tag_narrow_weight_image_bytes(wpad), hs) == hipSuccess && img,
+               "dc_tag_linear_fwd_narrow: could not allocate the weight image");
+    int rc = narrow_prep(ws, nseg, fi, wpad, img, hs);
+    if (rc == DC_OK) rc = narrow_fwd(slab, ld, img, bias, relu, out, ldo, N, wpad, nullptr, hs);
+    const bool freed = hipFreeAsync(img, hs) == hipSuccess;
+    if (rc != DC_OK) return rc;
+    DC_REQUIRE(freed, "dc_tag_linear_fwd_narrow: could not release the weight image");
     return check_launch("dc_tag_linear_fwd_narrow");
 }
diff --git a/deformcontact_amd/csrc/dc_dense_split.hip b/deformcontact_amd/csrc/dc_dense_split.hip
--- a/deformcontact_amd/csrc/dc_dense_split.hip
+++ b/deformcontact_amd/csrc/dc_dense_split.hip
@@ -316,31 +316,38 @@
     static constexpr int BYTES = Planes<NP>::P * PLANE;
 };
 
-template <int COLS, bool MASK, int NP>
+constexpr int kMaskF32 = 1, kMaskBits = 2;
+template <int COLS, int MASK, int NP>
 struct SplitOpRC {
     static constexpr int P = Planes<NP>::P;
     static constexpr int NV = COLS / 64;
     static constexpr int PER = COLS / 4, KPER = 256 / PER;
+    static constexpr bool MF = MASK == kMaskF32, MB = MASK == kMaskBits;
     using Img = TrImage<COLS, NP>;
     const float *p[NV];
-    const float *pm[MASK ? NV : 1];
+    const float *pm[MF ? NV : 1];
+    const uint32_t *pb[MB ? NV : 1];
     float4 v[NV];
-    float4 m[MASK ? NV : 1];
+    float4 m[MF ? NV : 1];
+    uint32_t mb[MB ? NV : 1];
     int off[NV];
     int64_t step, mstep;
+    int bshift;
     float sc;
 
-    __device__ __forceinline__ void init(const float *base, const float *mbase, int64_t ld,
+    __device__ __forceinline__ void init(const float *base, const void *mbase, int64_t ld,
                                          int64_t k0, int64_t col0, int64_t ncols, int64_t mld = 0) {
         const int c4 = threadIdx.x % PER, kr = threadIdx.x / PER;
         int64_t col = col0 + 4 * c4;
         col = col + 4 <= ncols ? col : ncols - 4;
-        mld = mld ? mld : ld;
+        if (!MB) mld = mld ? mld : ld;
+        bshift = (int)(col & 31);
 #pragma unroll
         for (int j = 0; j < NV; ++j) {
             const int64_t k = k0 + kr + KPER * j;
             p[j] = base + k * ld + col;
-            if (MASK) pm[j] = mbase + k * mld + col;
+            if (MF) pm[j] = reinterpret_cast<const float *>(mbase) + k * mld + col;
+            if (MB) pb[j] = reinterpret_cast<const uint32_t *>(mbase) + k * mld + (col >> 5);
             off[j] = (kr + KPER * j) * Img::ROWB + 8 * c4;
         }
         step = BK * ld;
@@ -353,15 +360,24 @@
             else if ((DC_DWS_ABL & 16) && !MASK) v[j] = make_float4(1.f, 2.f, 3.f, (float)j);
             else v[j] = *reinterpret_cast<const float4 *>(p[j]);
             p[j] += step;
-            if (MASK) {
+            if (MF) {
                 if (DC_DWS_ABL & 2) m[j] = make_float4(1.f, -1.f, 1.f, 1.f);
                 else m[j] = *reinterpret_cast<const float4 *>(pm[j]);
                 pm[j] += mstep;
             }
+            if (MB) {
+                mb[j] = *pb[j];
+                pb[j] += mstep;
+            }
         }
     }
     __device__ __forceinline__ float4 value(int j) const {
-        if (!MASK) return v[j];
+        if (MB) {
+            const uint32_t b = mb[j] >> bshift;
+            return make_float4((b & 1u) ? v[j].x : 0.f, (b & 2u) ? v[j].y : 0.f,
+                               (b & 4u) ? v[j].z : 0.f, (b & 8u) ? v[j].w : 0.f);
+        }
+        if (!MF) return v[j];
         return make_float4(m[j].x > 0.f ? v[j].x : 0.f, m[j].y > 0.f ? v[j].y : 0.f,
                            m[j].z > 0.f ? v[j].z : 0.f, m[j].w > 0.f ? v[j].w : 0.f);
     }
@@ -402,7 +418,7 @@
     return u.b;
 }
 
-template <int MB, bool MASK, int NP>
+template <int MB, int MASK, int NP>
 __global__ void __launch_bounds__(256)
 k_dw_split(DwParams p) {
     constexpr int BM = 64 * MB, P = Planes<NP>::P;
@@ -427,7 +443,8 @@
     using OA = SplitOpRC<BM, MASK, NP>;
     OA A;
     SplitOpRC<BN, false, NP> B;
-    A.init(p.g.p, p.mask.p, p.g.ld, n_beg, o0, p.Fo, p.mask.ld);
+    if (MASK == kMaskBits) A.init(p.g.p, p.mask_bits, p.g.ld, n_beg, o0, p.Fo, p.mask_bits_ld);
+    else A.init(p.g.p, p.mask.p, p.g.ld, n_beg, o0, p.Fo, p.mask.ld);
     B.init(p.x[s].p, nullptr, p.x[s].ld, n_beg, f0, p.Fi);
     float inva = 1.f, invb = 1.f;
     if (Planes<NP>::F16) {
@@ -812,7 +829,8 @@
     if (p.has_mask && (!al16(p.mask.p) || p.mask.ld % 4 != 0)) return false;
     for (int s = 0; s < p.nseg; ++s)
         if (!al16(p.x[s].p) || p.x[s].ld % 4 != 0) return false;
-    if (np == 2 && dw_h2w_launch(p, hs)) return true;
+    const bool bits = p.has_mask && p.mask_bits;
+    if (np == 2 && !bits && dw_h2w_launch(p, hs)) return true;
     const int64_t tiles = ((p.Fo + 64 * mb - 1) / (64 * mb)) * ((p.Fi + BN - 1) / BN);
     const dim3 gd((unsigned)(tiles * p.nseg * p.nchunks)), bd(256);
 #define DC_L(MB_, M_)                                                                 \
@@ -822,8 +840,8 @@
         else if (np == 2) DC_LAUNCH((k_dw_split<MB_, M_, 2>), gd, bd, 0, hs, p);  \
         else DC_LAUNCH((k_dw_split<MB_, M_, 1>), gd, bd, 0, hs, p);               \
     } while (0)
-    if (mb == 2) { if (p.has_mask) DC_L(2, true); else DC_L(2, false); }
-    else { if (p.has_mask) DC_L(1, true); else DC_L(1, false); }
+    if (mb == 2) { if (bits) DC_L(2, kMaskBits); else if (p.has_mask) DC_L(2, kMaskF32); else DC_L(2, 0); }
+    else { if (bits) DC_L(1, kMaskBits); else if (p.has_mask) DC_L(1, kMaskF32); else DC_L(1, 0); }
 #undef DC_L
     return true;
 }
diff --git a/deformcontact_amd/ops.py b/deformcontact_amd/ops.py
--- a/deformcontact_amd/ops.py
+++ b/deformcontact_amd/ops.py
@@ -162,6 +162,7 @@
 
 
 NARROW_FWD = os.environ.get("DC_NARROW_FWD", "1") != "0"
+NARROW_PREPPED = True
 
 DENSE_F16X2 = os.environ.get("DC_DENSE_F16X2", "1") != "0"
 
@@ -399,6 +400,14 @@
         h2 = _tag_uses_h2(fi, k, None if six else fo)
         rowmax = None
         prepped = None
+        narrow = (concat and NARROW_FWD and DENSE_SPLIT_BF16 and DENSE_PRODUCTS == 6
+                  and bool(L.dc_tag_linear_fwd_narrow_ok(fi, k + 1, wpad, fo)))
+        nimg = None
+        if narrow and NARROW_PREPPED and not h2:
+            nbytes = L.dc_tag_narrow_weight_image_bytes(wpad)
+            nimg = torch.empty(nbytes, dtype=torch.uint8, device=dev)
+            _lib.check(L.dc_tag_narrow_weight_prep(_ptr_array([w.contiguous() for w in weights]), k + 1, fi, wpad, fo,
+                                                   nimg.data_ptr(), nbytes, st), "dc_tag_narrow_weight_prep")
         if slab is None:
             key = None
             if HOP_CACHE and g is not None and k >= 1 and not ctx.needs_input_grad[1]:
@@ -422,8 +431,6 @@
             rowmax = torch.empty(n, dtype=torch.float32, device=dev)
             _lib.check(L.dc_rowabsmax_f32(slab.data_ptr(), slab.stride(0), n, fi, rowmax.data_ptr(), st), "dc_rowabsmax_f32")
         blocks = [slab[:, j * fi:(j + 1) * fi] for j in range(k + 1)]
-        narrow = (concat and NARROW_FWD and DENSE_SPLIT_BF16 and DENSE_PRODUCTS == 6
-                  and bool(L.dc_tag_linear_fwd_narrow_ok(fi, k + 1, wpad, fo)))
         if concat and narrow:
             ws = [w.contiguous() for w in weights]
             xs, ldxs, fi_eff = [slab], [slab.stride(0)], wpad
@@ -453,7 +460,7 @@
         b = bias.contiguous() if bias is not None else None
         args = (_ptr_array(xs), _i64_array(ldxs), _ptr_array(ws), len(xs),
                 b.data_ptr() if b is not None else None, int(relu), out.data_ptr(), ldo, n, fi_eff, fo)
-        wmax = wt = wt_rowmax = None
+        wmax = wt = wt_rowmax = relu_bits = None
         if h2:
             if prepped is None:
                 prepped = _h2_weight_prep(L, ws, k, fo, fi, ctx.needs_input_grad[1] and fo % 16 == 0, dev, st)
@@ -462,6 +469,13 @@
                                          b.data_ptr() if b is not None else None, int(relu),
                                          out.data_ptr(), ldo, n, width, fo,
                                          rowmax.data_ptr(), wmax.data_ptr(), None, 0, st)
+        elif narrow and nimg is not None:
+            if relu and (any(ctx.needs_input_grad[5:]) or ctx.needs_input_grad[2]):
+                relu_bits = torch.empty((n, fo // 32), dtype=torch.int32, device=dev)
+            rc = L.dc_tag_linear_fwd_narrow_prepped(slab.data_ptr(), slab.stride(0), nimg.data_ptr(),
+                                                    b.data_ptr() if b is not None else None, int(relu), out.data_ptr(),
+                                                    ldo, n, wpad, fo,
+                                                    relu_bits.data_ptr() if relu_bits is not None else None, st)
         elif narrow:
             rc = L.dc_tag_linear_fwd_narrow(slab.data_ptr(), slab.stride(0), _ptr_array(ws), k + 1, fi,
                                             b.data_ptr() if b is not None else None, int(relu), out.data_ptr(), ldo, n,
@@ -476,12 +490,12 @@
         ctx.narrow = narrow
         ctx.params, ctx.bias_param = weights, bias
         ctx.h2 = h2
-        ctx.save_for_backward(slab, out if relu else None, rowmax, wt, wt_rowmax, *ws)
+        ctx.save_for_backward(slab, out if relu else None, rowmax, wt, wt_rowmax, relu_bits, *ws)
         return out
 
     @staticmethod
     def backward(ctx, gout):
-        slab, out, xrowmax, wt, wt_rowmax, *ws = ctx.saved_tensors
+        slab, out, xrowmax, wt, wt_rowmax, relu_bits, *ws = ctx.saved_tensors
         g, k, fi, fo, concat = ctx.g, ctx.k, ctx.fi, ctx.fo, ctx.concat
         L = _lib.lib()
         if gout.stride(1) != 1 or gout.stride(0) % 4 != 0 or gout.data_ptr() % 16 != 0:
@@ -529,6 +543,9 @@
                         int(direct), scratch.data_ptr(), nbytes, n, fi_eff, fo)
                 if g_rowmax is not None and n % 16 == 0:
                     rc = L.dc_tag_linear_bwd_dw_h2(*args, g_rowmax.data_ptr(), xrowmax.data_ptr(), st)
+                elif DENSE_SPLIT_BF16 and relu_bits is not None and mask_ptr is not None:
+                    rc = L.dc_tag_linear_bwd_dw_split_bits(*args[:4], relu_bits.data_ptr(), relu_bits.stride(0),
+                                                           *args[4:], DENSE_PRODUCTS, st)
                 elif DENSE_SPLIT_BF16:
                     rc = L.dc_tag_linear_bwd_dw_split(*args, DENSE_PRODUCTS, st)
                 else:
diff --git a/include/deformcontact.h b/include/deformcontact.h
--- a/include/deformcontact.h
+++ b/include/deformcontact.h
@@ -132,6 +132,12 @@
 int dc_tag_linear_fwd_narrow(const float *slab, int64_t ld, const float *const *ws, int nseg, int64_t fi,
                              const float *bias, int relu, float *out, int64_t ldo, int64_t N, int64_t wpad,
                              int64_t Fo, dc_stream_t stream);
+int64_t dc_tag_narrow_weight_image_bytes(int64_t wpad);
+int dc_tag_narrow_weight_prep(const float *const *ws, int nseg, int64_t fi, int64_t wpad, int64_t Fo, void *img,
+                              int64_t img_bytes, dc_stream_t stream);
+int dc_tag_linear_fwd_narrow_prepped(const float *slab, int64_t ld, const void *img, const float *bias, int relu,
+                                     float *out, int64_t ldo, int64_t N, int64_t wpad, int64_t Fo, uint32_t *relu_bits,
+                                     dc_stream_t stream);
 int64_t dc_tag_linear_bwd_dx_split_workspace_bytes(int64_t Fi, int64_t Fo, int nseg);
 int dc_tag_linear_bwd_dx_split(const float *g, int64_t ldg, const float *out_for_mask,
                                int64_t ldo, const float *const *ws, int nseg, float *const *gxs,
@@ -149,6 +155,11 @@
                                float *const *gws, int ngw, int64_t gw_cols, float *gbias,
                                int accumulate, void *partials, int64_t partials_bytes, int64_t N,
                                int64_t Fi, int64_t Fo, int products, dc_stream_t stream);
+int dc_tag_linear_bwd_dw_split_bits(const float *g, int64_t ldg, const float *out_for_mask, int64_t ldo,
+                                    const uint32_t *mask_bits, int64_t ldb, const float *const *xs, const int64_t *ldxs,
+                                    int nseg, float *const *gws, int ngw, int64_t gw_cols, float *gbias, int accumulate,
+                                    void *partials, int64_t partials_bytes, int64_t N, int64_t Fi, int64_t Fo,
+                                    int products, dc_stream_t stream);
 
 int dc_tag_linear_fwd_h2(const float *const *xs, const int64_t *ldxs, const float *const *ws,
                          int nseg, const float *bias, int relu, float *out, int64_t ldo, int64_t N,
```

Measured after the change: 546.0 M edges/s, median of 6. 1.01x the previous value.
